# lisvulaczo/lodestar

Measured on AMD Instinct MI355X. Metric: BLS signature sets verified/sec (whole node) at 1/2/4/8 MI355X; p50 batch latency, higher is better.
Workload: dtype u32

## Files before the change

include/lodestar_bls.h:

```cpp
#ifndef LODESTAR_BLS_H
#define LODESTAR_BLS_H

#include <stddef.h>
#include <stdint.h>

#ifdef __cplusplus
extern "C" {
#endif

#define LSG_OK 0
#define LSG_ERR_INVALID_ARG 1
#define LSG_ERR_NO_DEVICE 2
#define LSG_ERR_DEVICE 3
#define LSG_ERR_NOMEM 4
#define LSG_ERR_CLOSED 5
#define LSG_ERR_BUSY 6
#define LSG_ERR_ENTROPY 7

#define LSG_BLST_SUCCESS 0
#define LSG_BLST_BAD_ENCODING 1
#define LSG_BLST_POINT_NOT_ON_CURVE 2
#define LSG_BLST_POINT_NOT_IN_GROUP 3
#define LSG_BLST_AGGR_TYPE_MISMATCH 4
#define LSG_BLST_VERIFY_FAIL 5
#define LSG_BLST_PK_IS_INFINITY 6
#define LSG_BLST_BAD_SCALAR 7
#define LSG_BLST_INVALID_SIZE 10
#define LSG_ERR_EMPTY_SET 100
#define LSG_ERR_EMPTY_AGGREGATE 101
#define LSG_ERR_BAD_INDEX 102
#define LSG_ERR_BAD_COMMITTEE 103

#define LSG_PK_INDEX 4u
#define LSG_PK_BITS 8u

#define LSG_MSG_OBJECT 0x80000000u

#define LSG_INVALID 0
#define LSG_VALID 1
#define LSG_ERROR 2

#define LSG_JOB_BATCHABLE 1u
#define LSG_JOB_PRIORITY 2u
#define LSG_JOB_VALIDATE_KEYS 4u

typedef struct lsg_ctx lsg_ctx;
typedef uint64_t lsg_ticket;

typedef struct {
  const uint8_t* pks;
  uint32_t pk_len;
  uint32_t n_pks;
  const uint8_t* msg;
  uint32_t msg_len;
  const uint8_t* sig;
  uint32_t sig_len;
} lsg_set;

typedef struct {
  const lsg_set* sets;
  uint32_t n_sets;
  uint32_t flags;
} lsg_job;

typedef struct {
  int32_t status;
  int32_t err_code;
} lsg_job_result;

typedef struct {
  uint32_t batch_retries;
  uint32_t batch_sigs_success;
  uint64_t start_ns;
  uint64_t end_ns;
  uint32_t n_final_exps;
  uint32_t submit_us;
  int32_t key_error;
  uint32_t key_error_job;
} lsg_stats;

int lsg_init(int device_ordinal, lsg_ctx** out);
int lsg_init_devices(const int* device_ids, int n_devices, lsg_ctx** out);
int lsg_destroy(lsg_ctx* ctx);
int lsg_device_count(lsg_ctx* ctx, int32_t* n);
const char* lsg_last_error(lsg_ctx* ctx);
int lsg_device_name(lsg_ctx* ctx, char* buf, size_t len);
int lsg_reserve(lsg_ctx* ctx, size_t max_sets, size_t max_pks, size_t max_msg_bytes, int32_t n_slots);
int lsg_allocation_count(lsg_ctx* ctx, uint64_t* n);

int lsg_submit_jobs(lsg_ctx* ctx, const lsg_job* jobs, size_t n_jobs, uint64_t seed, lsg_ticket* ticket);
int lsg_wait_jobs(lsg_ctx* ctx, lsg_ticket ticket, lsg_job_result* results , lsg_stats* stats);
int lsg_jobs_partial(lsg_ctx* ctx, lsg_ticket ticket, uint8_t* out576, int32_t* has_batch);
int lsg_jobs_partial_device(lsg_ctx* ctx, lsg_ticket ticket, void* dev_out576, int32_t* has_batch);
int lsg_wait_jobs_node(lsg_ctx* ctx, lsg_ticket ticket, int32_t node_valid, lsg_job_result* results,
                       lsg_stats* stats);
int lsg_set_coalesce(lsg_ctx* ctx, uint32_t max_sets, int32_t max_inflight);
int lsg_assign_jobs(const uint32_t* job_sets, size_t n_jobs, int32_t n_devices, int32_t* owner);
int lsg_pipeline_slots(lsg_ctx* ctx, int32_t* n);
int lsg_poll(lsg_ctx* ctx, lsg_ticket ticket, int32_t* done);
int lsg_verify_jobs(lsg_ctx* ctx, const lsg_job* jobs, size_t n_jobs, uint64_t seed, lsg_job_result* results,
                    lsg_stats* stats);

int lsg_verify_sets(lsg_ctx* ctx, const lsg_set* sets, size_t n_sets, uint64_t seed, lsg_job_result* result);

int lsg_aggregate_pubkeys(lsg_ctx* ctx, const uint8_t* pks, uint32_t pk_len, size_t n, uint8_t* out96,
                          int32_t* err_code);
int lsg_aggregate_pubkeys_multi(lsg_ctx* ctx, const lsg_set* sets, size_t n_sets, uint8_t* out96, int32_t* err);

int lsg_hash_to_g2(lsg_ctx* ctx, const uint8_t* msgs, uint32_t msg_len, size_t n, const uint8_t* dst,
                   uint32_t dst_len, uint8_t* out192);

int lsg_sig_decode(lsg_ctx* ctx, const uint8_t* sigs, uint32_t sig_len, size_t n, uint8_t* out192, int32_t* err);

int lsg_batch_partial(lsg_ctx* ctx, const lsg_set* sets, size_t n_sets, uint64_t seed, uint8_t* out576,
                      int32_t* set_err, int32_t* any_error);
int lsg_final_verify(lsg_ctx* ctx, const uint8_t* partials576, size_t n_partials, int32_t* valid);
int lsg_final_submit(lsg_ctx* ctx, const uint8_t* partials576, size_t n_partials, lsg_ticket* ticket);
int lsg_final_submit_device(lsg_ctx* ctx, const void* dev_partials576, size_t n_partials, lsg_ticket* ticket);
int lsg_final_wait(lsg_ctx* ctx, lsg_ticket ticket, int32_t* valid);
int lsg_final_submit_groups(lsg_ctx* ctx, const uint8_t* partials576, size_t n_groups, size_t per_group,
                            lsg_ticket* ticket);
int lsg_final_wait_groups(lsg_ctx* ctx, lsg_ticket ticket, int32_t* valid );

int lsg_pubkey_table_set(lsg_ctx* ctx, size_t first_index, const uint8_t* pks, uint32_t pk_len, size_t n,
                         int32_t* err);
int lsg_pubkey_table_size(lsg_ctx* ctx, size_t* n);

int lsg_committees_set(lsg_ctx* ctx, uint32_t first_id, const uint32_t* indices,
                       const uint32_t* offsets , size_t n_committees,
                       int32_t* err );
int lsg_committees_clear(lsg_ctx* ctx, uint32_t first_id, size_t n);
int lsg_committee_count(lsg_ctx* ctx, size_t* n);

int lsg_pubkey_validate(lsg_ctx* ctx, const uint8_t* pks, uint32_t pk_len, size_t n, uint8_t* out96, int32_t* err);

int lsg_aggregate_signatures(lsg_ctx* ctx, const uint8_t* sigs, uint32_t sig_len, const uint32_t* offsets,
                             size_t n_groups, uint8_t* out96, int32_t* err);

int lsg_signing_roots(lsg_ctx* ctx, const uint8_t* roots32, size_t n, const uint8_t* domain32, uint32_t domain_stride,
                      uint8_t* out32);
int lsg_attestation_signing_roots(lsg_ctx* ctx, const uint8_t* data128, size_t n, const uint8_t* domain32,
                                  uint32_t domain_stride, uint8_t* out32);
int lsg_deposit_signing_roots(lsg_ctx* ctx, const uint8_t* msgs88, size_t n, const uint8_t* domain32,
                              uint32_t domain_stride, uint8_t* out32);
int lsg_object_signing_roots(lsg_ctx* ctx, const uint8_t* objs, uint32_t obj_len, size_t n, const uint8_t* domain32,
                             uint32_t domain_stride, uint8_t* out32);

int lsg_verify_deposits(lsg_ctx* ctx, const uint8_t* data184, size_t n, const uint8_t* domain32, uint64_t seed,
                        uint8_t* valid, int32_t* err);

int lsg_sign(lsg_ctx* ctx, const uint8_t* sks32, const uint8_t* msgs, uint32_t msg_len, size_t n, uint8_t* out96);
int lsg_sk_to_pk(lsg_ctx* ctx, const uint8_t* sks32, size_t n, uint8_t* out96);

int lsg_check_fp2_mul(lsg_ctx* ctx, const uint32_t* in, size_t n, uint32_t* out);
int lsg_check_fp_sqr(lsg_ctx* ctx, const uint32_t* in, size_t n, uint32_t* out);
int lsg_check_fp2_sqr(lsg_ctx* ctx, const uint32_t* in, size_t n, uint32_t* out);
int lsg_check_sums(lsg_ctx* ctx, const uint32_t* in, size_t n, uint32_t* out);
int lsg_probe_fp_mul_rate(lsg_ctx* ctx, double* fp_mul_per_s, double* mad_per_s);

int lsg_probe_mad_peak(lsg_ctx* ctx, double* mad_per_s);

int lsg_last_kernel_times(lsg_ctx* ctx, const char** names, double* ms, int max);

#ifdef __cplusplus
}
#endif
#endif
```

lodestar_amd/_native.py:

```python
import ctypes
import os
import struct
import threading

HERE = os.path.dirname(os.path.abspath(__file__))
LIB_PATH = os.environ.get("LSG_LIB", os.path.join(HERE, "liblodestar_bls.so"))
AB_LIB_PATH = os.path.join(HERE, "liblodestar_bls_ab.so")

LSG_OK = 0
LSG_ERR_INVALID_ARG = 1
LSG_ERR_NO_DEVICE = 2
LSG_ERR_BUSY = 6
LSG_ERR_ENTROPY = 7

LSG_INVALID = 0
LSG_VALID = 1
LSG_ERROR = 2

LSG_JOB_BATCHABLE = 1
LSG_JOB_PRIORITY = 2
LSG_JOB_VALIDATE_KEYS = 4

BLST_NAMES = {
    0: "BLST_SUCCESS", 1: "BLST_BAD_ENCODING", 2: "BLST_POINT_NOT_ON_CURVE", 3: "BLST_POINT_NOT_IN_GROUP",
    4: "BLST_AGGR_TYPE_MISMATCH", 5: "BLST_VERIFY_FAIL", 6: "BLST_PK_IS_INFINITY", 7: "BLST_BAD_SCALAR",
    10: "BLST_INVALID_SIZE",
}
LSG_ERR_EMPTY_SET = 100
LSG_ERR_EMPTY_AGGREGATE = 101
LSG_ERR_BAD_INDEX = 102
LSG_ERR_BAD_COMMITTEE = 103
LSG_PK_INDEX = 4
LSG_PK_BITS = 8
LSG_MSG_OBJECT = 0x80000000


def error_message(code):
    if code == LSG_ERR_EMPTY_SET:
        return "Empty signature set"
    if code == LSG_ERR_EMPTY_AGGREGATE:
        return "EMPTY_AGGREGATE_ARRAY"
    if code == LSG_ERR_BAD_INDEX:
        return "Unknown pubkey index"
    if code == LSG_ERR_BAD_COMMITTEE:
        return "Unknown committee or bit length mismatch"
    return "BLST_ERROR: " + BLST_NAMES.get(code, f"BLST_UNKNOWN_{code}")


class NativeUnavailable(RuntimeError):
    pass


class PkIndices(list):

    def tobytes(self):
        import array
        a = array.array("I", self)
        assert a.itemsize == 4
        return a.tobytes()


class PkBits:

    def __init__(self, committee, bits, n_bits):
        self.committee = int(committee)
        self.n_bits = int(n_bits)
        nb = (self.n_bits + 7) // 8
        self.bits = bytes(bits)[:nb].ljust(nb, b"\0")

    def __len__(self):
        return self.n_bits

    def tobytes(self):
        return struct.pack("=I", self.committee) + self.bits


def _key_form(pks):
    if isinstance(pks, PkBits):
        return LSG_PK_BITS, pks.n_bits, pks.tobytes()
    if isinstance(pks, PkIndices):
        return LSG_PK_INDEX, len(pks), pks.tobytes()
    pk_len = len(pks[0]) if pks else 96
    if any(len(p) != pk_len for p in pks):
        raise ValueError("all pubkeys of one set must share one encoding length")
    if pk_len == LSG_PK_BITS:
        pk_len = 0
    return pk_len, len(pks), b"".join(pks)


class MsgObject:

    def __init__(self, obj, domain):
        self.obj = bytes(obj)
        self.domain = bytes(domain)

    def __len__(self):
        return len(self.obj) + len(self.domain)

    def tobytes(self):
        return self.obj + self.domain


def _msg_form(msg):
    if isinstance(msg, MsgObject):
        b = msg.tobytes()
        return b, len(b) | LSG_MSG_OBJECT
    return msg, len(msg)


class LsgSet(ctypes.Structure):
    _fields_ = [
        ("pks", ctypes.c_void_p), ("pk_len", ctypes.c_uint32), ("n_pks", ctypes.c_uint32),
        ("msg", ctypes.c_void_p), ("msg_len", ctypes.c_uint32),
        ("sig", ctypes.c_void_p), ("sig_len", ctypes.c_uint32),
    ]


class LsgJob(ctypes.Structure):
    _fields_ = [("sets", ctypes.POINTER(LsgSet)), ("n_sets", ctypes.c_uint32), ("flags", ctypes.c_uint32)]


class LsgJobResult(ctypes.Structure):
    _fields_ = [("status", ctypes.c_int32), ("err_code", ctypes.c_int32)]


class LsgStats(ctypes.Structure):
    _fields_ = [
        ("batch_retries", ctypes.c_uint32), ("batch_sigs_success", ctypes.c_uint32),
        ("start_ns", ctypes.c_uint64), ("end_ns", ctypes.c_uint64),
        ("n_final_exps", ctypes.c_uint32), ("submit_us", ctypes.c_uint32),
        ("key_error", ctypes.c_int32), ("key_error_job", ctypes.c_uint32),
    ]


_lib = None
_lib_lock = threading.Lock()

EXPORTS = [
    "lsg_init", "lsg_init_devices", "lsg_destroy", "lsg_device_count", "lsg_last_error", "lsg_device_name",
    "lsg_reserve", "lsg_allocation_count", "lsg_verify_jobs", "lsg_verify_sets",
    "lsg_aggregate_pubkeys", "lsg_hash_to_g2", "lsg_sig_decode", "lsg_batch_partial", "lsg_final_verify",
    "lsg_probe_fp_mul_rate", "lsg_last_kernel_times", "lsg_sign", "lsg_sk_to_pk",
    "lsg_submit_jobs", "lsg_wait_jobs", "lsg_wait_jobs_node", "lsg_jobs_partial", "lsg_assign_jobs", "lsg_poll",
    "lsg_final_submit", "lsg_final_wait", "lsg_pipeline_slots", "lsg_probe_mad_peak",
    "lsg_pubkey_table_set", "lsg_pubkey_table_size", "lsg_pubkey_validate",
    "lsg_final_submit_groups", "lsg_final_wait_groups", "lsg_aggregate_signatures",
    "lsg_signing_roots", "lsg_attestation_signing_roots", "lsg_jobs_partial_device", "lsg_final_submit_device",
    "lsg_set_coalesce", "lsg_aggregate_pubkeys_multi", "lsg_check_fp2_mul",
    "lsg_check_fp_sqr", "lsg_check_fp2_sqr", "lsg_check_sums",
    "lsg_deposit_signing_roots", "lsg_verify_deposits",
    "lsg_committees_set", "lsg_committees_clear", "lsg_committee_count",
    "lsg_object_signing_roots",
]


def load_library(path=LIB_PATH):
    global _lib
    with _lib_lock:
        if _lib is not None and path == LIB_PATH:
            return _lib
        if not os.path.exists(path):
            raise NativeUnavailable(f"{path} not built (run python -c 'import __graft_entry__; __graft_entry__.build()')")
        lib = ctypes.CDLL(path)
        vp, u32, u64, i32, sz = ctypes.c_void_p, ctypes.c_uint32, ctypes.c_uint64, ctypes.c_int32, ctypes.c_size_t
        pi32 = ctypes.POINTER(ctypes.c_int32)
        lib.lsg_init.argtypes = [ctypes.c_int, ctypes.POINTER(vp)]
        lib.lsg_init_devices.argtypes = [ctypes.POINTER(ctypes.c_int), ctypes.c_int, ctypes.POINTER(vp)]
        lib.lsg_device_count.argtypes = [vp, pi32]
        lib.lsg_reserve.argtypes = [vp, sz, sz, sz, i32]
        lib.lsg_allocation_count.argtypes = [vp, ctypes.POINTER(u64)]
        lib.lsg_wait_jobs_node.argtypes = [vp, u64, i32, ctypes.POINTER(LsgJobResult), ctypes.POINTER(LsgStats)]
        lib.lsg_jobs_partial.argtypes = [vp, u64, ctypes.c_char_p, pi32]
        lib.lsg_jobs_partial_device.argtypes = [vp, u64, vp, pi32]
        lib.lsg_final_submit_device.argtypes = [vp, vp, sz, ctypes.POINTER(u64)]
        lib.lsg_assign_jobs.argtypes = [ctypes.POINTER(u32), sz, i32, pi32]
        lib.lsg_destroy.argtypes = [vp]
        lib.lsg_last_error.argtypes = [vp]
        lib.lsg_last_error.restype = ctypes.c_char_p
        lib.lsg_device_name.argtypes = [vp, ctypes.c_char_p, sz]
        lib.lsg_verify_jobs.argtypes = [vp, ctypes.POINTER(LsgJob), sz, u64, ctypes.POINTER(LsgJobResult),
                                        ctypes.POINTER(LsgStats)]
        lib.lsg_verify_sets.argtypes = [vp, ctypes.POINTER(LsgSet), sz, u64, ctypes.POINTER(LsgJobResult)]
        lib.lsg_aggregate_pubkeys.argtypes = [vp, ctypes.c_char_p, u32, sz, ctypes.c_char_p, pi32]
        lib.lsg_aggregate_pubkeys_multi.argtypes = [vp, ctypes.POINTER(LsgSet), sz, ctypes.c_char_p, pi32]
        lib.lsg_hash_to_g2.argtypes = [vp, ctypes.c_char_p, u32, sz, ctypes.c_char_p, u32, ctypes.c_char_p]
        lib.lsg_sig_decode.argtypes = [vp, ctypes.c_char_p, u32, sz, ctypes.c_char_p, pi32]
        lib.lsg_batch_partial.argtypes = [vp, ctypes.POINTER(LsgSet), sz, u64, ctypes.c_char_p, pi32, pi32]
        lib.lsg_final_verify.argtypes = [vp, ctypes.c_char_p, sz, pi32]
        lib.lsg_probe_fp_mul_rate.argtypes = [vp, ctypes.POINTER(ctypes.c_double), ctypes.POINTER(ctypes.c_double)]
        lib.lsg_last_kernel_times.argtypes = [vp, ctypes.POINTER(ctypes.c_char_p), ctypes.POINTER(ctypes.c_double),
                                              ctypes.c_int]
        lib.lsg_sign.argtypes = [vp, ctypes.c_char_p, ctypes.c_char_p, u32, sz, ctypes.c_char_p]
        lib.lsg_sk_to_pk.argtypes = [vp, ctypes.c_char_p, sz, ctypes.c_char_p]
        pu64 = ctypes.POINTER(u64)
        lib.lsg_submit_jobs.argtypes = [vp, ctypes.POINTER(LsgJob), sz, u64, pu64]
        lib.lsg_wait_jobs.argtypes = [vp, u64, ctypes.POINTER(LsgJobResult), ctypes.POINTER(LsgStats)]
        lib.lsg_poll.argtypes = [vp, u64, pi32]
        lib.lsg_pubkey_table_set.argtypes = [vp, sz, ctypes.c_char_p, u32, sz, pi32]
        lib.lsg_pubkey_table_size.argtypes = [vp, ctypes.POINTER(sz)]
        lib.lsg_committees_set.argtypes = [vp, u32, ctypes.POINTER(u32), ctypes.POINTER(u32), sz, pi32]
        lib.lsg_committees_clear.argtypes = [vp, u32, sz]
        lib.lsg_committee_count.argtypes = [vp, ctypes.POINTER(sz)]
        lib.lsg_final_submit_groups.argtypes = [vp, ctypes.c_char_p, sz, sz, pu64]
        lib.lsg_final_wait_groups.argtypes = [vp, u64, pi32]
        lib.lsg_pubkey_validate.argtypes = [vp, ctypes.c_char_p, u32, sz, ctypes.c_char_p, pi32]
        lib.lsg_signing_roots.argtypes = [vp, ctypes.c_char_p, sz, ctypes.c_char_p, u32, ctypes.c_char_p]
        lib.lsg_attestation_signing_roots.argtypes = [vp, ctypes.c_char_p, sz, ctypes.c_char_p, u32, ctypes.c_char_p]
        lib.lsg_deposit_signing_roots.argtypes = [vp, ctypes.c_char_p, sz, ctypes.c_char_p, u32, ctypes.c_char_p]
        lib.lsg_object_signing_roots.argtypes = [vp, ctypes.c_char_p, u32, sz, ctypes.c_char_p, u32, ctypes.c_char_p]
        lib.lsg_verify_deposits.argtypes = [vp, ctypes.c_char_p, sz, ctypes.c_char_p, u64, ctypes.c_char_p, pi32]
        lib.lsg_aggregate_signatures.argtypes = [vp, ctypes.c_char_p, u32, ctypes.POINTER(u32), sz,
                                                 ctypes.c_char_p, pi32]
        lib.lsg_final_submit.argtypes = [vp, ctypes.c_char_p, sz, pu64]
        lib.lsg_final_wait.argtypes = [vp, u64, pi32]
        lib.lsg_pipeline_slots.argtypes = [vp, pi32]
        lib.lsg_set_coalesce.argtypes = [vp, u32, i32]
        lib.lsg_check_fp2_mul.argtypes = [vp, ctypes.c_char_p, sz, ctypes.c_char_p]
        lib.lsg_check_fp_sqr.argtypes = [vp, ctypes.c_char_p, sz, ctypes.c_char_p]
        lib.lsg_check_fp2_sqr.argtypes = [vp, ctypes.c_char_p, sz, ctypes.c_char_p]
        lib.lsg_check_sums.argtypes = [vp, ctypes.c_char_p, sz, ctypes.c_char_p]
        lib.lsg_probe_mad_peak.argtypes = [vp, ctypes.POINTER(ctypes.c_double)]
        for name in EXPORTS:
            if name != "lsg_last_error":
                getattr(lib, name).restype = ctypes.c_int
        if path == LIB_PATH:
            _lib = lib
        return lib


class SetBuffer:

    def __init__(self, sets):
        self._keep = []
        sets = list(sets)
        self.arr = (LsgSet * max(len(sets), 1))()
        for i, (pks, msg, sig) in enumerate(sets):
            pk_len, n_pks, pkb = _key_form(pks)
            msg, msg_len = _msg_form(msg)
            for b in (pkb, msg, sig):
                self._keep.append(b)
            s = self.arr[i]
            s.pks = ctypes.cast(ctypes.c_char_p(pkb), ctypes.c_void_p) if pkb else None
            s.pk_len = pk_len
            s.n_pks = n_pks
            s.msg = ctypes.cast(ctypes.c_char_p(msg), ctypes.c_void_p) if msg else None
            s.msg_len = msg_len
            s.sig = ctypes.cast(ctypes.c_char_p(sig), ctypes.c_void_p) if sig else None
            s.sig_len = len(sig)
        self.n = len(sets)


def assign_jobs(job_sizes, n_devices):
    lib = load_library()
    n = len(job_sizes)
    sizes = (ctypes.c_uint32 * max(n, 1))(*job_sizes)
    owner = (ctypes.c_int32 * max(n, 1))()
    rc = lib.lsg_assign_jobs(sizes, n, int(n_devices), owner)
    if rc != LSG_OK:
        raise ValueError(f"lsg_assign_jobs failed ({rc})")
    return list(owner[:n])


class PreparedJobs:

    def __init__(self, jobs):
        import numpy as np
        flat = [st for sets, _ in jobs for st in sets]
        n = len(flat)
        pk_parts, pk_len, n_pks = [], np.zeros(max(n, 1), np.uint32), np.zeros(max(n, 1), np.uint32)
        for i, (pks, _m, _s) in enumerate(flat):
            pk_len[i], n_pks[i], b = _key_form(pks)
            pk_parts.append(b)

        def pack(parts):
            lens = np.array([len(p) for p in parts] or [0], np.uint64)
            offs = np.zeros_like(lens)
            if len(parts) > 1:
                offs[1:] = np.cumsum(lens)[:-1]
            buf = np.frombuffer(b"".join(parts) + b"\0", dtype=np.uint8).copy()
            return buf, offs, lens

        self._pk, pk_off, _ = pack(pk_parts)
        forms = [_msg_form(m) for _, m, _ in flat]
        self._msg, msg_off, msg_len = pack([b for b, _ in forms])
        msg_word = np.array([w for _, w in forms] or [0], np.uint32)
        self._sig, sig_off, sig_len = pack([s for _, _, s in flat])
        self.sets = (LsgSet * max(n, 1))()
        dt = np.dtype({"names": ["pks", "pk_len", "n_pks", "msg", "msg_len", "sig", "sig_len"],
                       "formats": [np.uint64, np.uint32, np.uint32, np.uint64, np.uint32, np.uint64, np.uint32],
                       "offsets": [LsgSet.pks.offset, LsgSet.pk_len.offset, LsgSet.n_pks.offset, LsgSet.msg.offset,
                                   LsgSet.msg_len.offset, LsgSet.sig.offset, LsgSet.sig_len.offset],
                       "itemsize": ctypes.sizeof(LsgSet)})
        v = np.frombuffer(self.sets, dtype=dt)
        if n:
            v["pks"][:n] = np.where(n_pks[:n] > 0, self._pk.ctypes.data + pk_off[:n], 0)
            v["pk_len"][:n] = pk_len[:n]
            v["n_pks"][:n] = n_pks[:n]
            v["msg"][:n] = np.where(msg_len[:n] > 0, self._msg.ctypes.data + msg_off[:n], 0)
            v["msg_len"][:n] = msg_word[:n]
            v["sig"][:n] = np.where(sig_len[:n] > 0, self._sig.ctypes.data + sig_off[:n], 0)
            v["sig_len"][:n] = sig_len[:n]
        self.n_jobs = len(jobs)
        self.n_sets = n
        self.jobs = (LsgJob * max(len(jobs), 1))()
        jd = np.dtype({"names": ["sets", "n_sets", "flags"], "formats": [np.uint64, np.uint32, np.uint32],
                       "offsets": [LsgJob.sets.offset, LsgJob.n_sets.offset, LsgJob.flags.offset],
                       "itemsize": ctypes.sizeof(LsgJob)})
        jv = np.frombuffer(self.jobs, dtype=jd)
        counts = np.array([len(sets) for sets, _ in jobs] or [0], np.uint64)
        firsts = np.zeros_like(counts)
        if len(jobs) > 1:
            firsts[1:] = np.cumsum(counts)[:-1]
        if jobs:
            jv["sets"][:len(jobs)] = ctypes.addressof(self.sets) + firsts * ctypes.sizeof(LsgSet)
            jv["n_sets"][:len(jobs)] = counts
            jv["flags"][:len(jobs)] = [f for _, f in jobs]


class Context:

    def __init__(self, device=0, devices=None, lib=None):
        self.lib = load_library(lib or LIB_PATH)
        h = ctypes.c_void_p()
        if devices is None:
            rc = self.lib.lsg_init(int(device), ctypes.byref(h))
        else:
            ids = (ctypes.c_int * len(devices))(*devices)
            rc = self.lib.lsg_init_devices(ids, len(devices), ctypes.byref(h))
        if rc != LSG_OK:
            raise NativeUnavailable(f"lsg_init({devices if devices is not None else device}) failed with status {rc} "
                                    f"(no gfx950 device?)")
        self.h = h
        self.device = device if devices is None else devices[0]
        self.devices = [self.device] if devices is None else list(devices)

    def reserve(self, max_sets, max_pks=None, max_msg_bytes=None, n_slots=0):
        max_pks = max_sets if max_pks is None else max_pks
        max_msg_bytes = 32 * max_sets if max_msg_bytes is None else max_msg_bytes
        self._check(self.lib.lsg_reserve(self.h, max_sets, max_pks, max_msg_bytes, n_slots), "lsg_reserve")

    def set_coalesce(self, max_sets, max_inflight=2):
        self._check(self.lib.lsg_set_coalesce(self.h, int(max_sets), int(max_inflight)), "lsg_set_coalesce")

    def allocation_count(self):
        v = ctypes.c_uint64()
        self._check(self.lib.lsg_allocation_count(self.h, ctypes.byref(v)), "lsg_allocation_count")
        return v.value

    def device_count(self):
        v = ctypes.c_int32()
        self._check(self.lib.lsg_device_count(self.h, ctypes.byref(v)), "lsg_device_count")
        return v.value

    def close(self):
        if getattr(self, "h", None):
            self.lib.lsg_destroy(self.h)
            self.h = None

    def __del__(self):
        try:
            self.close()
        except Exception:
            pass

    def _check(self, rc, what):
        if rc != LSG_OK:
            raise RuntimeError(f"{what} failed ({rc}): {self.lib.lsg_last_error(self.h).decode(errors='replace')}")

    def device_name(self):
        b = ctypes.create_string_buffer(256)
        self._check(self.lib.lsg_device_name(self.h, b, 256), "lsg_device_name")
        return b.value.decode()

# ... 177 lines not shown
    def attestation_signing_roots(self, data128s, domains):
        return self._signing_roots("lsg_attestation_signing_roots", data128s, 128, domains)

    def deposit_signing_roots(self, msgs88, domains):
        return self._signing_roots("lsg_deposit_signing_roots", msgs88, 88, domains)

    def object_signing_roots(self, objs, domains):
        n = len(objs)
        if n == 0:
            return []
        size = len(objs[0])
        assert all(len(o) == size for o in objs)
        if isinstance(domains, (bytes, bytearray)):
            dom, stride = bytes(domains), 0
        else:
            assert len(domains) == n
            dom, stride = b"".join(domains), 32
        assert len(dom) == (32 if stride == 0 else 32 * n)
        out = ctypes.create_string_buffer(32 * n)
        self._check(self.lib.lsg_object_signing_roots(self.h, b"".join(objs), size, n, dom, stride, out),
                    "lsg_object_signing_roots")
        raw = out.raw
        return [raw[32 * i:32 * i + 32] for i in range(n)]

    def verify_deposits(self, data184s, domain, seed=0):
        n = len(data184s)
        if n == 0:
            return []
        assert all(len(d) == 184 for d in data184s) and len(domain) == 32
        valid = ctypes.create_string_buffer(n)
        err = (ctypes.c_int32 * n)()
        self._check(self.lib.lsg_verify_deposits(self.h, b"".join(data184s), n, bytes(domain), seed, valid, err),
                    "lsg_verify_deposits")
        raw = valid.raw
        return [(raw[i], err[i]) for i in range(n)]

    def hash_to_g2(self, msgs, dst=b"BLS_SIG_BLS12381G2_XMD:SHA-256_SSWU_RO_POP_"):
        if not msgs:
            return []
        ml = len(msgs[0])
        assert all(len(m) == ml for m in msgs)
        out = ctypes.create_string_buffer(192 * len(msgs))
        self._check(self.lib.lsg_hash_to_g2(self.h, b"".join(msgs), ml, len(msgs), dst, len(dst), out), "lsg_hash_to_g2")
        raw = out.raw
        return [raw[192 * i:192 * i + 192] for i in range(len(msgs))]

    def sig_decode(self, sigs):
        if not sigs:
            return []
        sl = len(sigs[0])
        assert all(len(s) == sl for s in sigs)
        out = ctypes.create_string_buffer(192 * len(sigs))
        err = (ctypes.c_int32 * len(sigs))()
        self._check(self.lib.lsg_sig_decode(self.h, b"".join(sigs), sl, len(sigs), out, err), "lsg_sig_decode")
        raw = out.raw
        return [(raw[192 * i:192 * i + 192], err[i]) for i in range(len(sigs))]

    def batch_partial(self, sets, seed=0):
        b = SetBuffer(sets)
        out = ctypes.create_string_buffer(576)
        errs = (ctypes.c_int32 * max(b.n, 1))()
        anyerr = ctypes.c_int32()
        self._check(self.lib.lsg_batch_partial(self.h, b.arr, b.n, seed, out, errs, ctypes.byref(anyerr)),
                    "lsg_batch_partial")
        return out.raw, [errs[i] for i in range(b.n)], bool(anyerr.value)

    def final_verify(self, partials):
        v = ctypes.c_int32()
        self._check(self.lib.lsg_final_verify(self.h, b"".join(partials), len(partials), ctypes.byref(v)),
                    "lsg_final_verify")
        return bool(v.value)

    def final_submit(self, partials):
        t = ctypes.c_uint64()
        rc = self.lib.lsg_final_submit(self.h, b"".join(partials), len(partials), ctypes.byref(t))
        if rc == LSG_ERR_BUSY:
            return None
        self._check(rc, "lsg_final_submit")
        return t.value

    def final_wait(self, ticket):
        v = ctypes.c_int32()
        self._check(self.lib.lsg_final_wait(self.h, ticket, ctypes.byref(v)), "lsg_final_wait")
        return bool(v.value)

    def final_submit_groups(self, groups):
        ng = len(groups)
        pg = len(groups[0]) if groups else 0
        if any(len(g) != pg for g in groups):
            raise ValueError("every group needs the same number of partials")
        t = ctypes.c_uint64()
        rc = self.lib.lsg_final_submit_groups(self.h, b"".join(b"".join(g) for g in groups), ng, pg, ctypes.byref(t))
        if rc == LSG_ERR_BUSY:
            return None
        self._check(rc, "lsg_final_submit_groups")
        t_ng = ng
        return (t.value, t_ng)

    def final_wait_groups(self, ticket):
        t, ng = ticket
        v = (ctypes.c_int32 * max(ng, 1))()
        self._check(self.lib.lsg_final_wait_groups(self.h, t, v), "lsg_final_wait_groups")
        return [bool(x) for x in v[:ng]]

    def sign(self, sks, msgs):
        if not sks:
            return []
        ml = len(msgs[0])
        out = ctypes.create_string_buffer(96 * len(sks))
        skb = b"".join(int(k).to_bytes(32, "big") for k in sks)
        self._check(self.lib.lsg_sign(self.h, skb, b"".join(msgs), ml, len(sks), out), "lsg_sign")
        raw = out.raw
        return [raw[96 * i:96 * i + 96] for i in range(len(sks))]

    def sk_to_pk(self, sks):
        if not sks:
            return []
        out = ctypes.create_string_buffer(96 * len(sks))
        skb = b"".join(int(k).to_bytes(32, "big") for k in sks)
        self._check(self.lib.lsg_sk_to_pk(self.h, skb, len(sks), out), "lsg_sk_to_pk")
        raw = out.raw
        return [raw[96 * i:96 * i + 96] for i in range(len(sks))]

    def check_fp2_mul(self, words):
        n = len(words) // 56
        assert len(words) == 56 * n
        out = ctypes.create_string_buffer(4 * 28 * n)
        src = struct.pack(f"<{len(words)}I", *words)
        self._check(self.lib.lsg_check_fp2_mul(self.h, src, n, out), "lsg_check_fp2_mul")
        return list(struct.unpack(f"<{28 * n}I", out.raw))

    def _check_sqr(self, fn, words, per_item):
        n = len(words) // per_item
        assert len(words) == per_item * n
        out = ctypes.create_string_buffer(4 * per_item * n)
        src = struct.pack(f"<{len(words)}I", *words)
        self._check(getattr(self.lib, fn)(self.h, src, n, out), fn)
        return list(struct.unpack(f"<{per_item * n}I", out.raw))

    def check_fp_sqr(self, words):
        return self._check_sqr("lsg_check_fp_sqr", words, 14)

    def check_fp2_sqr(self, words):
        return self._check_sqr("lsg_check_fp2_sqr", words, 28)

    def check_sums(self, words):
        n = len(words) // (12 * 14)
        assert len(words) == 12 * 14 * n
        out = ctypes.create_string_buffer(4 * 42 * 14 * n)
        src = struct.pack(f"<{len(words)}I", *words)
        self._check(self.lib.lsg_check_sums(self.h, src, n, out), "lsg_check_sums")
        return list(struct.unpack(f"<{42 * 14 * n}I", out.raw))

    def probe_fp_mul_rate(self):
        a, b = ctypes.c_double(), ctypes.c_double()
        self._check(self.lib.lsg_probe_fp_mul_rate(self.h, ctypes.byref(a), ctypes.byref(b)), "lsg_probe_fp_mul_rate")
        return a.value, b.value

    def last_kernel_times(self, max_entries=1024):
        names = (ctypes.c_char_p * max_entries)()
        ms = (ctypes.c_double * max_entries)()
        n = self.lib.lsg_last_kernel_times(self.h, names, ms, max_entries)
        return [(names[i].decode(), ms[i]) for i in range(n)]
```

lodestar_amd/build.py:

```python
import os
import shutil
import subprocess
import sys

HERE = os.path.dirname(os.path.abspath(__file__))
ROOT = os.path.dirname(HERE)
CSRC = os.path.join(HERE, "csrc")
OUT = os.path.join(HERE, "liblodestar_bls.so")
SOURCES = ["lsg_k_hash.hip", "lsg_k_sig.hip", "lsg_k_pk.hip", "lsg_k_miller.hip", "lsg_k_reduce.hip", "lsg_slp.hip",
           "lsg_host.hip"]
HEADERS = ["lsg_types.hpp", "lsg_fp_lane.hpp", "lsg_fp_elem.hpp", "lsg_tower.hpp", "lsg_curve.hpp", "lsg_h2c.hpp",
           "lsg_pairing.hpp", "lsg_constants.hpp", "lsg_fp_pair.hpp", "lsg_constants_r29.hpp", "lsg_io.hpp",
           "lsg_serial.h", "lsg_kcommon.hpp", "lsg_launch.h", "lsg_layout.h", "lsg_slp_progs.h", "lsg_slp_exec.hpp", "lsg_inv.hpp",
           "lsg_ab.h", "lsg_plan.hpp", "lsg_bits.h", "lsg_ssz.hpp"]
OBJ = os.path.join(HERE, "_obj")
AB_OUT = os.path.join(HERE, "liblodestar_bls_ab.so")
AB_SOURCES = ["lsg_host.hip", "lsg_serial.hip", "lsg_serial_wide.hip"]
AB_FLAGS = ["-DLSG_AB=1"]


def hipcc():
    for c in (shutil.which("hipcc"), "/opt/rocm/bin/hipcc"):
        if c and os.path.exists(c):
            return c
    raise RuntimeError("hipcc not found")


def _deps():
    return [os.path.join(CSRC, f) for f in HEADERS] + [os.path.join(ROOT, "include", "lodestar_bls.h"),
                                                       os.path.abspath(__file__)]


def needs_rebuild(out=OUT, sources=SOURCES):
    if not os.path.exists(out):
        return True
    deps = [os.path.join(CSRC, f) for f in sources] + _deps()
    return max(os.path.getmtime(d) for d in deps if os.path.exists(d)) > os.path.getmtime(out)


CFLAGS = ["--offload-arch=gfx950", "-O3", "-std=c++17", "-fPIC", "-DLSG_BIGFN=__host__ __device__ __forceinline__"]


def _obj_dir(extra):
    if not extra:
        return OBJ
    import hashlib
    return OBJ + "_" + hashlib.sha1(" ".join(extra).encode()).hexdigest()[:10]


def _compile(src, verbose, extra):
    obj = os.path.join(_obj_dir(extra), os.path.splitext(src)[0] + ".o")
    srcp = os.path.join(CSRC, src)
    dep_t = max(os.path.getmtime(d) for d in [srcp] + _deps() if os.path.exists(d))
    if os.path.exists(obj) and os.path.getmtime(obj) >= dep_t:
        return obj
    cmd = [hipcc()] + CFLAGS + extra + ["-I", CSRC, "-I", os.path.join(ROOT, "include"), "-c", srcp, "-o", obj + ".tmp"]
    if verbose:
        print("[lodestar_amd.build]", " ".join(cmd), flush=True)
    subprocess.check_call(cmd)
    os.replace(obj + ".tmp", obj)
    return obj


def build(force=False, verbose=True, extra=None, out=None):
    from concurrent.futures import ThreadPoolExecutor
    gen = os.path.join(ROOT, "tools", "gen_constants.py")
    const = os.path.join(CSRC, "lsg_constants.hpp")
    if not os.path.exists(const) or os.path.getmtime(gen) > os.path.getmtime(const):
        subprocess.check_call([sys.executable, gen, const])
    gen_slp = os.path.join(ROOT, "tools", "gen_slp.py")
    progs = os.path.join(CSRC, "lsg_slp_progs.h")
    if not os.path.exists(progs) or os.path.getmtime(gen_slp) > os.path.getmtime(progs):
        subprocess.check_call([sys.executable, gen_slp, progs])
    extra = list(extra or [])
    out = out or OUT
    if not force and not extra and out == OUT and not needs_rebuild():
        if read_manifest(OUT) is None:
            write_manifest(OUT, SOURCES, [])
        return OUT
    odir = _obj_dir(extra)
    os.makedirs(odir, exist_ok=True)
    if force:
        for f in os.listdir(odir):
            os.remove(os.path.join(odir, f))
    jobs = int(os.environ.get("LSG_BUILD_JOBS", str(min(8, os.cpu_count() or 4))))
    with ThreadPoolExecutor(max_workers=jobs) as ex:
        objs = list(ex.map(lambda s: _compile(s, verbose, extra), SOURCES))
    _link(objs, out, verbose)
    write_manifest(out, SOURCES, extra)
    return out


def source_hash(sources=SOURCES):
    import hashlib
    h = hashlib.sha256()
    files = sorted(set([os.path.join(CSRC, f) for f in list(sources) + HEADERS] +
                       [os.path.join(ROOT, "include", "lodestar_bls.h")]))
    for f in files:
        if os.path.exists(f):
            h.update(os.path.basename(f).encode() + b"\0")
            with open(f, "rb") as fh:
                h.update(fh.read())
    return h.hexdigest()


def _compiler_version():
    try:
        out = subprocess.run([hipcc(), "--version"], capture_output=True, text=True, timeout=60).stdout
        return next((ln.strip() for ln in out.splitlines() if "clang version" in ln), out.splitlines()[0].strip())
    except Exception as e:
        return "unknown (%s)" % e


def write_manifest(out, sources, extra):
    import hashlib
    import json
    import time
    with open(out, "rb") as fh:
        so_sha = hashlib.sha256(fh.read()).hexdigest()
    rec = {"lib": os.path.basename(out), "so_sha256_16": so_sha[:16], "src_sha256": source_hash(sources),
           "compiler": _compiler_version(), "flags": CFLAGS + list(extra),
           "built_utc": time.strftime("%Y-%m-%dT%H:%M:%SZ", time.gmtime())}
    with open(out + ".manifest.json", "w") as fh:
        fh.write(json.dumps(rec, sort_keys=True) + "\n")
    return rec


def read_manifest(out=None):
    import json
    try:
        with open((out or OUT) + ".manifest.json") as fh:
            return json.loads(fh.read())
    except (OSError, ValueError):
        return None


def _link(objs, out, verbose):
    cmd = [hipcc(), "--offload-arch=gfx950", "-fPIC", "-shared"] + objs + ["-L/opt/rocm/lib", "-lrccl",
                                                                           "-Wl,-rpath,/opt/rocm/lib", "-o", out + ".tmp"]
    if verbose:
        print("[lodestar_amd.build]", " ".join(cmd), flush=True)
    subprocess.check_call(cmd)
    os.replace(out + ".tmp", out)


def build_ab(verbose=True):
    from concurrent.futures import ThreadPoolExecutor
    build(verbose=verbose)
    if not needs_rebuild(AB_OUT, SOURCES + AB_SOURCES):
        return AB_OUT
    os.makedirs(_obj_dir(AB_FLAGS), exist_ok=True)
    with ThreadPoolExecutor(max_workers=len(AB_SOURCES)) as ex:
        ab = dict(zip(AB_SOURCES, ex.map(lambda s: _compile(s, verbose, AB_FLAGS), AB_SOURCES)))
    objs = [ab.get(s) or os.path.join(OBJ, os.path.splitext(s)[0] + ".o") for s in SOURCES]
    objs += [ab[s] for s in AB_SOURCES if s not in SOURCES]
    _link(objs, AB_OUT, verbose)
    write_manifest(AB_OUT, SOURCES + AB_SOURCES, AB_FLAGS)
    return AB_OUT


NAPI_SRC = os.path.join(HERE, "napi", "lsg_napi.c")
NAPI_OUT = os.path.join(HERE, "napi", "lsg_napi.node")
NODE_INCLUDE = "/usr/include/node"


def build_napi(verbose=True):
    if not os.path.exists(os.path.join(NODE_INCLUDE, "node_api.h")):
# ... 19 lines not shown
```

lodestar_amd/csrc/lsg_host.hip:

```cpp
#include <hip/hip_runtime.h>
#include <rccl/rccl.h>
#include <stdio.h>
#include <stdlib.h>
#include <errno.h>
#include <string.h>
#include <sys/random.h>
#include <time.h>

#include <algorithm>
#include <atomic>
#include <condition_variable>
#include <chrono>
#include <mutex>
#include <shared_mutex>
#include <thread>
#include <unordered_map>
#include <string>
#include <vector>

#include "../../include/lodestar_bls.h"
#include "lsg_launch.h"
#include "lsg_layout.h"
#include "lsg_serial.h"
#include "lsg_ab.h"
// ... 335 lines not shown
  do {                                                    \
    timer_begin((s), name);                               \
    hipError_t _le = (call);                              \
    timer_end((s));                                       \
    if (_le != hipSuccess) return fail((s), name, _le);   \
  } while (0)

inline const int32_t* PL(Slot* s, size_t off) { return P_<int32_t>(s->d_plan) + off; }

void keep_times(Slot* s) {
  auto& v = s->d->last_times;
  v.clear();
  for (size_t i = 0; i < s->ntimers; i++) {
    float t = 0;
    if (hipEventElapsedTime(&t, s->timers[i].a, s->timers[i].b) != hipSuccess) t = -1;
    v.push_back({s->timers[i].name, t});
  }
}

int prio_stream(lsg_ctx* c, Dev* d, hipStream_t* st) {
  if (!*st) {
    int least = 0, greatest = 0;
    LSG_HIPC(c, hipSetDevice(d->device));
    LSG_HIPC(c, hipDeviceGetStreamPriorityRange(&least, &greatest));
    LSG_HIPC(c, hipStreamCreateWithPriority(st, hipStreamNonBlocking, greatest));
  }
  return LSG_OK;
}

hipError_t event_wait(hipEvent_t e) {
  const auto t0 = std::chrono::steady_clock::now();
  for (;;) {
    const hipError_t r = hipEventQuery(e);
    if (r != hipErrorNotReady) return r;
    if (std::chrono::steady_clock::now() - t0 > std::chrono::microseconds(20))
      std::this_thread::sleep_for(std::chrono::microseconds(30));
  }
}

bool blocking_waits() {
  const char* e = getenv("LSG_BLOCKING_WAITS");
  return e && atoi(e) != 0;
}

int slot_create(Dev* d, Slot* s, int index, hipStream_t shared) {
  s->d = d;
  s->index = index;
  if (shared) {
    s->st[0] = s->st[1] = shared;
    s->own_streams = false;
  } else {
    for (int k = 0; k < 2; k++) LSG_HIP(s, hipStreamCreateWithFlags(&s->st_norm[k], hipStreamNonBlocking));
    s->st[0] = s->st_norm[0];
    s->st[1] = s->st_norm[1];
  }
  hipEvent_t* evs[] = {&s->ev_in, &s->ev_sig, &s->ev_grp, &s->ev_part, &s->ev_done, &s->ev_node, &s->ev_xp};
  for (hipEvent_t* e : evs) LSG_HIP(s, hipEventCreateWithFlags(e, hipEventDisableTiming));
  if (blocking_waits()) {
    for (hipEvent_t* e : {&s->ev_part, &s->ev_done}) {
      LSG_HIP(s, hipEventDestroy(*e));
      LSG_HIP(s, hipEventCreateWithFlags(e, hipEventDisableTiming | hipEventBlockingSync));
    }
  }
  LSG_RC(ensure(s, s->d_dst, 256));
  LSG_HIP(s, hipMemcpy(s->d_dst.p, DST_POP, DST_POP_LEN, hipMemcpyHostToDevice));
  return LSG_OK;
}

void slot_destroy(Slot* s) {
  if (!s->d) return;
  for (int k = 0; k < 2; k++)
    if (s->st[k]) (void)hipStreamSynchronize(s->st[k]);
  DevBuf* bufs[] = {&s->d_sig,  &s->d_siglen, &s->d_msg,  &s->d_msgoff, &s->d_msglen, &s->d_pk,    &s->d_pklen,
                    &s->d_rnd,  &s->d_mode,   &s->d_dst,  &s->d_ub,     &s->d_sigaff, &s->d_siginf, &s->d_seterr,
                    &s->d_pkp,  &s->d_pkerr,  &s->d_agg,  &s->d_P,      &s->d_pinf,   &s->d_H,     &s->d_hinf,
                    &s->d_rs,   &s->d_rs2,    &s->d_fall, &s->d_fall2,  &s->d_Pp,     &s->d_zP,    &s->d_zPi,
                    &s->d_U,    &s->d_nrm,    &s->d_nrmi, &s->d_Hp,     &s->d_zN,     &s->d_zNi,   &s->binv_lv[0],
                    &s->binv_lv[1], &s->binv_iv[0], &s->binv_iv[1], &s->d_lines, &s->d_S, &s->d_F, &s->d_verdict,
                    &s->d_Sb,   &s->d_fgb,    &s->d_Fb,   &s->d_bkt,    &s->d_bits,   &s->d_aux,   &s->d_gath,
                    &s->d_nodeF, &s->d_nodeV, &s->d_plan, &s->d_mid, &s->d_Hm, &s->d_hinfm,
                    &s->d_mmask, &s->d_PmP, &s->d_Pm, &s->d_pinfm, &s->d_errm, &s->d_xport,
                    &s->d_agga, &s->d_aggi, &s->d_aggpre, &s->d_aggtot, &s->d_aggflag, &s->d_cbits};
  for (DevBuf* b : bufs) free_dev(*b);
  for (auto& u : s->seg_tmp)
    for (DevBuf& b : u) free_dev(b);
  HostBuf* hb[] = {&s->h_arena, &s->h_err, &s->h_pinf, &s->h_pkerr, &s->h_verdict, &s->h_blob, &s->h_plan, &s->h_nodeV,
                   &s->h_xport, &s->h_cbits};
  for (HostBuf* b : hb) free_host(*b);
  for (Timer& t : s->timers) {
    (void)hipEventDestroy(t.a);
    (void)hipEventDestroy(t.b);
  }
  s->timers.clear();
  hipEvent_t evs[] = {s->ev_in, s->ev_sig, s->ev_grp, s->ev_part, s->ev_done, s->ev_node, s->ev_xp};
  for (hipEvent_t e : evs)
    if (e) (void)hipEventDestroy(e);
  if (s->own_streams) {
    for (int k = 0; k < 2; k++) {
      if (s->st_prio[k]) (void)hipStreamSynchronize(s->st_prio[k]);
      if (s->st_norm[k]) (void)hipStreamSynchronize(s->st_norm[k]);
    }
    for (int k = 0; k < 2; k++) {
      if (s->st_norm[k]) (void)hipStreamDestroy(s->st_norm[k]);
      s->st_norm[k] = s->st_prio[k] = s->st[k] = nullptr;
    }
  }
  s->d = nullptr;
}

int slot_streams(Slot* s, bool prio) {
  if (!s->own_streams) return LSG_OK;
  if (prio && !s->st_prio[0]) {
    Dev* d = s->d;
    for (int k = 0; k < 2; k++) LSG_RC(prio_stream(d->c, d, &d->s_pp[k]));
    s->st_prio[0] = d->s_pp[0];
    s->st_prio[1] = d->s_pp[1];
  }
  hipStream_t* p = prio ? s->st_prio : s->st_norm;
  s->st[0] = p[0];
  s->st[1] = p[1];
  return LSG_OK;
}

int slot_ready(Dev* d, Slot* s, int index) {
  if (s->d) return LSG_OK;
  const int rc = slot_create(d, s, index, nullptr);
  if (rc) slot_destroy(s);
  return rc;
}

bool miller_fused() { return lsg_ab_long("LSG_MILLER_FUSED", 1) != 0; }

size_t slp_items_max();
int miller_k_for(size_t n_sets) {
  if (miller_fused()) return n_sets <= slp_items_max() ? 1 : 4;
  const long v = lsg_ab_long("LSG_MILLER_K", 0);
  if (v == 1 || v == 2 || v == 4) return (int)v;
  return n_sets >= 8192 ? 4 : (n_sets >= 1024 ? 2 : 1);
}

bool agg_tree_on() { return lsg_ab_long("LSG_AGG_TREE", 0) != 0; }

Switches read_switches() {
  Switches w;
  w.package_group = lsg_ab_long("LSG_PACKAGE_GROUP", 1) != 0;
  w.sub_groups = lsg_ab_long("LSG_SUB_GROUPS", 1) != 0;
  w.nb_merge = lsg_ab_long("LSG_NB_MERGE", 1) != 0;
  w.msg_agg = lsg_ab_long("LSG_MSG_AGG", 1) != 0;
  w.msm_min_group = (size_t)std::max(1L, lsg_ab_long("LSG_MSM_MIN_GROUP", 256));
  w.b0_min = (size_t)std::max(0L, lsg_ab_long("LSG_B0_MIN", 64));
  w.b0_run = (size_t)std::max(2L, lsg_ab_long("LSG_B0_RUN", 4));
  w.seg_fold_wide = (int)lsg_ab_long("LSG_SEG_FOLD_WIDE", SEG_FOLD_WIDE);
  w.slp_items = slp_items_max();
  return w;
}
SegPlan slot_seg(Slot* s, int op, const std::vector<int32_t>& seg_off, const std::vector<int32_t>& seg_len, bool has_idx,
                 size_t idx_off, int32_t dst_base) {
  return plan_seg(s->plan, op, seg_off, seg_len, has_idx, idx_off, dst_base,
                  (int)lsg_ab_long("LSG_SEG_FOLD_WIDE", SEG_FOLD_WIDE));
}

void binv_sizes(size_t n, size_t* lv, size_t* iv);
size_t binv_lv_words(size_t n) {
  size_t a, b;
  binv_sizes(n, &a, &b);
  return a;
}
size_t binv_iv_words(size_t n) {
  size_t a, b;
  binv_sizes(n, &a, &b);
  return b;
}

int size_inputs(Slot* s, size_t n, size_t np, size_t mb) {
  const size_t nn = std::max(n, (size_t)1), pp = std::max(np, (size_t)1);
  auto al = [](size_t x) { return (x + 7) & ~(size_t)7; };
  const size_t arena = al(192 * nn) + al(4 * nn) * 4 + al(4 * pp) + al(8 * nn) + al(96 * pp) + al(std::max(mb, (size_t)1)) + nn;
  LSG_RC(ensure_host(s, s->h_arena, arena));
  LSG_RC(ensure(s, s->d_sig, 192 * nn));
  LSG_RC(ensure(s, s->d_siglen, 4 * nn));
  LSG_RC(ensure(s, s->d_msg, std::max(mb, (size_t)1)));
  LSG_RC(ensure(s, s->d_msgoff, 4 * nn));
  LSG_RC(ensure(s, s->d_msglen, 4 * nn));
  LSG_RC(ensure(s, s->d_pk, 96 * pp));
  LSG_RC(ensure(s, s->d_pklen, 4 * pp));
  LSG_RC(ensure(s, s->d_rnd, 8 * nn));
  LSG_RC(ensure(s, s->d_mode, nn));
  LSG_RC(ensure(s, s->d_mid, 4 * nn));
  return LSG_OK;
}

int size_state(Slot* s, size_t n, size_t np, size_t ng, size_t n_msm, int pkg = 0) {
  const size_t nn = std::max(n, (size_t)1), pp = std::max(np, (size_t)1), gg = std::max(ng, (size_t)1);
  const size_t g_msm = std::max(n_msm, (size_t)1);
  struct {
    DevBuf* b;
    size_t bytes;
  } dev[] = {{&s->d_ub, 256 * nn},
             {&s->d_sigaff, 4 * W_G2A * nn},
             {&s->d_siginf, nn},
             {&s->d_seterr, 4 * nn},
             {&s->d_pkp, 4 * W_G1P * pp},
             {&s->d_pkerr, 4 * pp},
             {&s->d_agg, 4 * W_G1P * nn},
             {&s->d_P, 4 * W_G1A * nn},
             {&s->d_pinf, nn},
             {&s->d_H, 4 * W_G2A * nn},
             {&s->d_hinf, nn},
             {&s->d_rs, 4 * W_G2P * nn},
             {&s->d_Pp, 4 * W_G1P * nn},
             {&s->d_zP, 4 * W_FP * nn},
             {&s->d_zPi, 4 * W_FP * nn},
             {&s->d_U, 4 * W_H2CU * nn},
             {&s->d_nrm, 4 * W_FP * 2 * nn},
             {&s->d_nrmi, 4 * W_FP * 2 * nn},
             {&s->d_Hp, 4 * W_G2P * nn},
             {&s->d_zN, 4 * W_FP * nn},
             {&s->d_zNi, 4 * W_FP * nn},
             {&s->binv_lv[0], 4 * W_FP * binv_lv_words(2 * nn)},
             {&s->binv_iv[0], 4 * W_FP * binv_iv_words(2 * nn)},
             {&s->binv_lv[1], 4 * W_FP * binv_lv_words(nn)},
             {&s->binv_iv[1], 4 * W_FP * binv_iv_words(nn)},
             {&s->d_S, 4 * W_G2P * gg},
             {&s->d_F, 4 * W_F12 * gg},
             {&s->d_verdict, 4 * gg},
             {&s->d_Sb, (size_t)288 * (MSM_BITS * g_msm + gg)},
             {&s->d_fgb, 576 * gg},
             {&s->d_Fb, 576 * gg},
             {&s->d_bkt, 4 * W_G2P * (size_t)MSM_WINDOWS * MSM_DIGITS * g_msm},
             {&s->d_bits, 4 * W_G2P * (size_t)MSM_BITS * g_msm},
             {&s->d_gath, 576 * (LSG_MAX_DEVICES + 2)},
             {&s->d_nodeF, 4 * W_F12 * (LSG_MAX_DEVICES + 1)},
             {&s->d_nodeV, 64}};
  for (auto& x : dev) LSG_RC(ensure(s, *x.b, x.bytes));
  if (pkg == 1) {
    if (!miller_fused()) LSG_RC(ensure(s, s->d_lines, 4 * (size_t)ML_STEPS * W_LINE * nn));
    LSG_RC(ensure(s, s->d_fall, 4 * W_F12 * (2 * nn + gg + 2)));
  }
  if (pkg) {
    LSG_RC(ensure(s, s->d_fall2, 4 * W_F12 * (nn + std::max(gg, nn))));
    LSG_RC(ensure(s, s->d_rs2, 4 * W_G2P * nn));
  }
  LSG_RC(ensure_host(s, s->h_err, 4 * nn));
  LSG_RC(ensure_host(s, s->h_pinf, nn));
  LSG_RC(ensure_host(s, s->h_pkerr, 4 * pp));
  LSG_RC(ensure_host(s, s->h_verdict, 4 * gg));
  LSG_RC(ensure_host(s, s->h_blob, 576 * gg));
  LSG_RC(ensure_host(s, s->h_nodeV, 64));
  return LSG_OK;
}

int size_seg(Slot* s, int use, const SegPlan& P) {
  if (P.tmp_items == 0) return LSG_OK;
  const size_t W = P.op == 0 ? W_G1P : (P.op == 1 ? W_G2P : W_F12);
  LSG_RC(ensure(s, s->seg_tmp[use][0], 4 * W * P.tmp_items));
  return ensure(s, s->seg_tmp[use][1], 4 * W * P.tmp_items);
}

int upload_plan(Slot* s) {
  const size_t bytes = 4 * std::max(s->plan.size(), (size_t)1);
  LSG_RC(ensure_host(s, s->h_plan, bytes));
  LSG_RC(ensure(s, s->d_plan, bytes));
  if (!s->plan.empty()) {
    memcpy(s->h_plan.p, s->plan.data(), 4 * s->plan.size());
    LSG_HIP(s, hipMemcpyAsync(s->d_plan.p, s->h_plan.p, 4 * s->plan.size(), hipMemcpyHostToDevice, s->st[0]));
  }
  return LSG_OK;
}

int run_seg(Slot* s, int use, const char* name, const SegPlan& P, const uint32_t* src, uint32_t* dst) {
  LSG_RC(size_seg(s, use, P));
  uint32_t* tmp[3] = {nullptr, P_<uint32_t>(s->seg_tmp[use][0]), P_<uint32_t>(s->seg_tmp[use][1])};
  const int32_t* idx = P.has_idx ? PL(s, P.idx_off) : nullptr;
  for (size_t k = 0; k < P.passes.size(); k++) {
    const SegPass& q = P.passes[k];
    const uint32_t* in = q.src == 0 ? src : tmp[q.src];
    KL(s, name, lsgk::seg_reduce(S_(s), P.op, q.n_chunks, q.ips_log2, PL(s, q.chunk_off), k == 0 ? idx : nullptr, in, dst,
                                 tmp[q.tmp_out]));
  }
  return LSG_OK;
}

int run_pk_seg(Slot* s, const SegPlan& P, uint32_t* dst) {
  LSG_RC(size_seg(s, 0, P));
  Dev* d = s->d;
  uint32_t* tmp[3] = {nullptr, P_<uint32_t>(s->seg_tmp[0][0]), P_<uint32_t>(s->seg_tmp[0][1])};
  for (size_t k = 0; k < P.passes.size(); k++) {
    const SegPass& q = P.passes[k];
    if (k == 0)
      KL(s, "g1_aggregate", lsgk::pk_agg_seg(S_(s), q.n_chunks, q.ips_log2, PL(s, q.chunk_off), P_<uint8_t>(s->d_pk),
                                             s->pk_stride, P_<uint32_t>(s->d_pklen), P_<int32_t>(s->d_pkerr),
                                             P_<uint32_t>(d->d_pktab), P_<uint8_t>(d->d_pktab_ok), (uint32_t)d->pktab_n,
                                             dst, tmp[q.tmp_out]));
    else
      KL(s, "g1_aggregate", lsgk::seg_reduce(S_(s), 0, q.n_chunks, q.ips_log2, PL(s, q.chunk_off), nullptr,
                                             tmp[q.src], dst, tmp[q.tmp_out]));
  }
  return LSG_OK;
}

static bool binv_block_on() { return lsg_ab_long("LSG_BINV_BLOCK", 1) != 0; }

void binv_sizes(size_t n, size_t* lv, size_t* iv) {
  size_t a = 0, b = 0;
  for (size_t m = n; m > 1;) {
    const size_t up = (m + LSG_BINV_T - 1) / LSG_BINV_T;
    a += m + up;
    b += up;
    m = up;
  }
  *lv = std::max(a, (size_t)1);
  *iv = std::max(b, (size_t)1);
}

int batch_inv(Slot* s, int ws, const char* name, const uint32_t* v, size_t n, uint32_t* out) {
  if (n == 0) return LSG_OK;
  size_t lvw, ivw;
  binv_sizes(n, &lvw, &ivw);
  LSG_RC(ensure(s, s->binv_lv[ws], 4 * W_FP * lvw));
  LSG_RC(ensure(s, s->binv_iv[ws], 4 * W_FP * ivw));
  uint32_t* lv = P_<uint32_t>(s->binv_lv[ws]);
  uint32_t* iv = P_<uint32_t>(s->binv_iv[ws]);
  if (binv_block_on()) {
    const int T = (int)std::min<size_t>(64, std::max<size_t>(1, (n + 128 * 64 - 1) / (128 * 64)));
    KL(s, name, lsgk::binv_block(S_(s), (int)n, T, 1, v, lv, out));
    return LSG_OK;
  }
  std::vector<size_t> cnt{n};
  std::vector<uint32_t*> val{(uint32_t*)v}, pre, inv{out};
  size_t lo = 0, io = 0;
  while (cnt.back() > 1) {
    const size_t m = cnt.back(), up = (m + LSG_BINV_T - 1) / LSG_BINV_T;
    pre.push_back(lv + W_FP * lo);
    lo += m;
    val.push_back(lv + W_FP * lo);
    lo += up;
    inv.push_back(iv + W_FP * io);
    io += up;
    cnt.push_back(up);
  }
  const size_t L = cnt.size() - 1;
  if (L == 0) {
    KL(s, name, lsgk::binv_root(S_(s), v, out));
    return LSG_OK;
  }
  for (size_t l = 0; l < L; l++)
    KL(s, name, lsgk::binv_fold(S_(s), (int)cnt[l], l == 0 ? 1 : 0, val[l], pre[l], val[l + 1]));
  KL(s, name, lsgk::binv_root(S_(s), val[L], inv[L]));
  for (size_t l = L; l-- > 0;)
    KL(s, name, lsgk::binv_unfold(S_(s), (int)cnt[l], l == 0 ? 1 : 0, val[l], pre[l], inv[l + 1], inv[l]));
  return LSG_OK;
}


size_t slp_items_max() {
  const long v = lsg_ab_long("LSG_SLP_ITEMS", 2048);
  return lsg_serial_mode() == LSG_SERIAL_SLP && v > 0 ? (size_t)v : 0;
}

int launch_hash(Slot* s, int n, uint32_t* H, uint8_t* hinf) {
  KL(s, "k_h2c_prep", lsgk::h2c_prep(S_(s), n, P_<uint8_t>(s->d_ub), P_<uint32_t>(s->d_U), P_<uint32_t>(s->d_nrm)));
  LSG_RC(batch_inv(s, 0, "binv_sswu", P_<uint32_t>(s->d_nrm), 2 * (size_t)n, P_<uint32_t>(s->d_nrmi)));
  KL(s, "k_h2c_map", lsgk::h2c_map(S_(s), n, P_<uint32_t>(s->d_U), P_<uint32_t>(s->d_nrmi), P_<uint32_t>(s->d_Hp)));
  if ((size_t)n <= slp_items_max()) {
    KL(s, "k_slp_h2c", lsg_slp_h2c_clear(S_(s), n, P_<uint32_t>(s->d_Hp), H, hinf));
    return LSG_OK;
  }
  KL(s, "k_h2c_clear", lsgk::h2c_clear(S_(s), n, P_<uint32_t>(s->d_Hp), P_<uint32_t>(s->d_zN), hinf));
  LSG_RC(batch_inv(s, 0, "binv_hash", P_<uint32_t>(s->d_zN), (size_t)n, P_<uint32_t>(s->d_zNi)));
  KL(s, "k_h2c_affine", lsgk::h2c_affine(S_(s), n, P_<uint32_t>(s->d_Hp), P_<uint32_t>(s->d_zNi), hinf, H));
  return LSG_OK;
}

static uint64_t msg_key(const uint8_t* m, uint32_t msg_len) {
  uint64_t h = 0x9e3779b97f4a7c15ull ^ msg_len;
  const uint32_t len = msg_bytes(msg_len);
  uint32_t k = 0;
  for (; k + 8 <= len; k += 8) {
    uint64_t w;
    memcpy(&w, m + k, 8);
    h = (h ^ w) * 0xff51afd7ed558ccdull;
    h ^= h >> 32;
  }
  for (; k < len; k++) h = (h ^ m[k]) * 0x100000001b3ull;
  return h ^ (h >> 29);
}

int stage_sets(Slot* s, const lsg_set* const* sets, size_t n, uint64_t seed, bool scale,
               const std::vector<uint8_t>* noscale = nullptr, bool dedup = false, bool bits_ok = false) {
  size_t npk = 0, msg_total = 0, n_bits_sets = 0, bit_words = 0;
  bool any_obj = false;
  bool all_index = true;
  auto is_bits = [&](const lsg_set* q) { return bits_ok && q->pk_len == LSG_PK_BITS; };
  for (size_t i = 0; i < n; i++) {
    msg_total += msg_bytes(sets[i]->msg_len);
    any_obj = any_obj || msg_marked(sets[i]->msg_len);
    if (is_bits(sets[i])) {
      n_bits_sets++;
      bit_words += bits_words(sets[i]->n_pks);
      continue;
    }
    npk += sets[i]->n_pks;
    if (sets[i]->n_pks && sets[i]->pk_len != LSG_PK_INDEX) all_index = false;
  }
  s->bits_sets.clear();
  s->shape.bits_p.clear();
  s->shape.bits_kerr.clear();
  s->pk_all_bits = n > 0 && n_bits_sets == n;
  uint32_t* cbits = nullptr;
  if (n_bits_sets) {
    s->shape.bits_p.assign(n, -1);
    s->shape.bits_kerr.assign(n, 0);
    s->bits_sets.reserve(n_bits_sets);
    LSG_RC(ensure_host(s, s->h_cbits, 4 * bit_words));
    LSG_RC(ensure(s, s->d_cbits, 4 * bit_words));
    cbits = H_<uint32_t>(s->h_cbits);
  }
  size_t bw = 0;
  const size_t ks = all_index ? 4 : 96;
  s->pk_stride = (uint32_t)ks;
  s->n_sets = n;
  s->n_pks = npk;
  LSG_RC(size_inputs(s, n, npk, msg_total));
  const size_t nn = std::max(n, (size_t)1), np = std::max(npk, (size_t)1);
  auto al = [](size_t x) { return (x + 7) & ~(size_t)7; };
  const size_t o_sig = 0, o_siglen = al(o_sig + 192 * nn), o_msgoff = al(o_siglen + 4 * nn),
               o_msglen = al(o_msgoff + 4 * nn), o_mid = al(o_msglen + 4 * nn), o_pklen = al(o_mid + 4 * nn),
               o_rnd = al(o_pklen + 4 * np), o_pk = al(o_rnd + 8 * nn), o_msg = al(o_pk + ks * np);
  uint8_t* A = H_<uint8_t>(s->h_arena);
  uint32_t* siglen = (uint32_t*)(A + o_siglen);
  uint32_t* msgoff = (uint32_t*)(A + o_msgoff);
  uint32_t* msglen = (uint32_t*)(A + o_msglen);
  uint32_t* mid = (uint32_t*)(A + o_mid);
  uint32_t* pklen = (uint32_t*)(A + o_pklen);
  uint64_t* rnd = (uint64_t*)(A + o_rnd);
// ... 53 lines not shown
        if (s->mkey[h] != key) continue;
        const lsg_set* r = sets[s->mfirst[e]];
        if (r->msg_len == q->msg_len && (q->msg_len == 0 || memcmp(r->msg, q->msg, msg_bytes(q->msg_len)) == 0)) {
          id = e;
          break;
        }
      }
    }
    mid[i] = id;
    if (id == nm) {
      msgoff[nm] = (uint32_t)mo;
      msglen[nm] = q->msg_len;
      const uint32_t mb = msg_bytes(q->msg_len);
      if (mb) memcpy(A + o_msg + mo, q->msg, mb);
      mo += mb;
      nm++;
    }
    if (is_bits(q)) {
      const lsg_ctx* c = s->d->c;
      s->shape.pk_cnt[i] = 0;
      s->shape.pk_first[i] = (uint32_t)po;
      BitsSet b;
      b.out = (int32_t)i;
      uint32_t id = 0;
      if (q->pks) memcpy(&id, q->pks, 4);
      if (!q->pks || id >= c->cm_ok.size() || !c->cm_ok[id] || c->cm_len[id] != q->n_pks)
        s->shape.bits_kerr[i] = LSG_ERR_BAD_COMMITTEE;
      else
        b = bits_stage_set(id, q->pks + 4, q->n_pks, (int32_t)i, cbits, &bw);
      s->shape.bits_p[i] = (int32_t)b.p;
      s->bits_sets.push_back(b);
      continue;
    }
    s->shape.pk_cnt[i] = q->n_pks;
    s->shape.pk_first[i] = (uint32_t)po;
    if (q->n_pks != 1) single = false;
    if (all_index) {
      std::fill(pklen + po, pklen + po + q->n_pks, (uint32_t)LSG_PK_INDEX);
      if (q->pks)
        memcpy(A + o_pk + 4 * po, q->pks, 4 * (size_t)q->n_pks);
      else
        memset(A + o_pk + 4 * po, 0, 4 * (size_t)q->n_pks);
      po += q->n_pks;
      continue;
    }
    for (uint32_t k = 0; k < q->n_pks; k++) {
      pklen[po] = q->pk_len;
      uint8_t* pd = A + o_pk + 96 * po;
      if ((q->pk_len == 48 || q->pk_len == 96 || q->pk_len == LSG_PK_INDEX) && q->pks)
        memcpy(pd, q->pks + (size_t)q->pk_len * k, q->pk_len);
      else
        memset(pd, 0, 4);
      po++;
    }
  }
  s->single_keys = single && n > 0;
  s->n_msgs = nm;
  s->msg_objs = any_obj;
  s->msg_dedup = nm < n;
  if (s->msg_dedup) s->msg_id.assign(mid, mid + n);
  if (scale && n) {
    if (seed == 0) {
      if (!os_random(rnd, 8 * n)) {
        set_err(s->d->c, "no entropy for the RLC randomizers (getrandom failed)");
        return LSG_ERR_ENTROPY;
      }
      for (size_t i = 0; i < n; i++)
        while (rnd[i] == 0)
          if (!os_random(&rnd[i], 8)) {
            set_err(s->d->c, "no entropy for the RLC randomizers (getrandom failed)");
            return LSG_ERR_ENTROPY;
          }
    } else {
      uint64_t sd = seed;
      for (size_t i = 0; i < n; i++) {
        uint64_t r;
        do r = splitmix64(sd);
        while (r == 0);
        rnd[i] = r;
      }
    }
  } else if (n) {
    memset(rnd, 0, 8 * n);
  }
  if (scale && noscale)
    for (size_t i = 0; i < n; i++)
      if ((*noscale)[i]) rnd[i] = 0;
  memcpy(s->rnd.data(), rnd, 8 * n);
  hipStream_t S = s->st[0];
  struct {
    DevBuf* d;
    size_t off, len;
  } cp[] = {{&s->d_sig, o_sig, 192 * nn},      {&s->d_siglen, o_siglen, 4 * nn}, {&s->d_msg, o_msg, std::max(msg_total, (size_t)1)},
            {&s->d_msgoff, o_msgoff, 4 * nn}, {&s->d_msglen, o_msglen, 4 * nn}, {&s->d_pk, o_pk, ks * np},
            {&s->d_pklen, o_pklen, 4 * np},   {&s->d_rnd, o_rnd, 8 * nn}};
  for (auto& x : cp) LSG_HIP(s, hipMemcpyAsync(x.d->p, A + x.off, x.len, hipMemcpyHostToDevice, S));
  if (s->msg_dedup) LSG_HIP(s, hipMemcpyAsync(s->d_mid.p, A + o_mid, 4 * n, hipMemcpyHostToDevice, S));
  if (bw) LSG_HIP(s, hipMemcpyAsync(s->d_cbits.p, cbits, 4 * bw, hipMemcpyHostToDevice, S));
  return LSG_OK;
}

int run_pk_bits(Slot* s, uint32_t* dst) {
  if (s->bits_sets.empty()) return LSG_OK;
  Dev* d = s->d;
  KL(s, "k_pk_agg_bits", lsgk::pk_agg_bits(S_(s), (int)s->bplan.n_pairs, PL(s, s->bplan.pair_off), PL(s, s->bplan.plan_off),
                                           P_<uint32_t>(s->d_cbits), P_<uint32_t>(d->d_cm_idx), P_<uint32_t>(d->d_cm_off),
                                           P_<uint32_t>(d->d_cm_sum), P_<uint32_t>(d->d_pktab), P_<uint8_t>(d->d_pktab_ok),
                                           (uint32_t)d->pktab_n, dst));
  return LSG_OK;
}


int launch_accum(Slot* s, size_t n_items, size_t item_off, uint32_t* fall, bool single = false) {
  const int ni = (int)n_items;
  const int32_t* items = PL(s, item_off);
  if (ni > 0 && (single || s->K == 1) && miller_fused() && (size_t)ni <= std::max(slp_items_max(), (size_t)8192) &&
      slp_items_max() > 0) {
    KL(s, "k_slp_items1", lsg_slp_miller_items1(S_(s), ni, items, P_<uint32_t>(s->d_P), P_<uint8_t>(s->d_pinf),
                                                P_<uint8_t>(s->d_hinf), P_<int32_t>(s->d_seterr), P_<uint32_t>(s->d_H),
                                                fall));
    return LSG_OK;
  }
  if (single && ni > 0) {
    LSG_RC(ensure(s, s->d_lines, 4 * (size_t)ML_STEPS * W_LINE * n_items));
    KL(s, "k_miller_lines_list", lsgk::miller_lines_list(S_(s), ni, items, P_<uint32_t>(s->d_H), P_<uint32_t>(s->d_lines)));
    KL(s, "k_miller_accum_list",
       lsgk::miller_accum_list(S_(s), ni, items, P_<uint32_t>(s->d_P), P_<uint8_t>(s->d_pinf), P_<uint8_t>(s->d_hinf),
                               P_<int32_t>(s->d_seterr), P_<uint32_t>(s->d_lines), fall));
    return LSG_OK;
  }
  if (miller_fused()) {
    KL(s, "k_miller_fused", lsgk::miller_fused(S_(s), ni, items, items + ni, P_<uint32_t>(s->d_P), P_<uint8_t>(s->d_pinf),
                                              P_<uint8_t>(s->d_hinf), P_<int32_t>(s->d_seterr), P_<uint32_t>(s->d_H),
                                              fall));
    return LSG_OK;
  }
  KL(s, "k_miller_accum",
     lsgk::miller_accum(S_(s), s->K, ni, items, items + ni, P_<uint32_t>(s->d_P), P_<uint8_t>(s->d_pinf),
                        P_<uint8_t>(s->d_hinf), P_<int32_t>(s->d_seterr), (int)s->n_sets, P_<uint32_t>(s->d_lines),
                        fall));
  return LSG_OK;
}

#define SERIAL_LABEL(name) (lsg_serial_mode() == LSG_SERIAL_SLP ? "slp_" #name : "k_row_" #name)

int launch_phase(Slot* s, const PhasePlan& Ph, const uint32_t* rs, uint32_t* fall, bool export_blobs,
                 const uint32_t* rs_msm = nullptr) {
  if (!rs_msm) rs_msm = rs;
  const size_t ng = Ph.groups.size();
  if (ng == 0) return LSG_OK;
  LSG_RC(size_state(s, s->n_sets, s->n_pks, ng, Ph.n_msm, 2));
  s->cur = 1;
  if (Ph.n_msm) {
    LSG_RC(run_seg(s, 1, "msm_buckets", Ph.buckets, rs_msm, P_<uint32_t>(s->d_bkt)));
    LSG_RC(run_seg(s, 1, "msm_bits", Ph.bits, P_<uint32_t>(s->d_bkt), P_<uint32_t>(s->d_bits)));
    KL(s, "k_g2p_to_canon", lsgk::g2p_to_canon(S_(s), (int)(MSM_BITS * Ph.n_msm), P_<uint32_t>(s->d_bits),
                                               P_<uint8_t>(s->d_Sb)));
    KL(s, SERIAL_LABEL(horner_miller),
       lsg_row_horner_miller(S_(s), (int)Ph.n_msm, P_<uint8_t>(s->d_Sb), P_<uint8_t>(s->d_fgb)));
  }
  if (Ph.n_msm < ng) {
    const int nsm = (int)(ng - Ph.n_msm);
    LSG_RC(run_seg(s, 1, "sig_sums", Ph.sums, rs, P_<uint32_t>(s->d_S)));
    uint8_t* sb = P_<uint8_t>(s->d_Sb) + (size_t)288 * MSM_BITS * Ph.n_msm;
    KL(s, "k_g2p_to_canon", lsgk::g2p_to_canon(S_(s), nsm, P_<uint32_t>(s->d_S) + W_G2P * Ph.n_msm, sb));
    KL(s, SERIAL_LABEL(miller_neg_g1),
       lsg_row_miller_neg_g1(S_(s), nsm, sb, P_<uint8_t>(s->d_fgb) + 576 * Ph.n_msm));
  }
  KL(s, "k_blobs_to_fp12", lsgk::blobs_to_fp12(S_(s), (int)ng, P_<uint8_t>(s->d_fgb), fall + W_F12 * Ph.term_base));
  LSG_HIP(s, hipEventRecord(s->ev_grp, s->st[1]));
  s->cur = 0;
  LSG_HIP(s, hipStreamWaitEvent(s->st[0], s->ev_grp, 0));
  LSG_RC(run_seg(s, 2, "fp12_product", Ph.prod, fall, P_<uint32_t>(s->d_F)));
  KL(s, "k_fp12_to_canon", lsgk::fp12_to_canon(S_(s), (int)ng, P_<uint32_t>(s->d_F), P_<uint8_t>(s->d_Fb)));
  if (export_blobs) LSG_HIP(s, hipMemcpyAsync(s->h_blob.p, s->d_Fb.p, 576 * ng, hipMemcpyDeviceToHost, s->st[0]));
  LSG_HIP(s, hipEventRecord(s->ev_part, s->st[0]));
  return LSG_OK;
}

int launch_fe_range(Slot* s, size_t g0, size_t g1) {
  if (g1 <= g0) return LSG_OK;
  s->cur = 0;
  const size_t ng = g1 - g0;
  KL(s, SERIAL_LABEL(final_exp),
     lsg_row_final_exp(S_(s), (int)ng, P_<uint8_t>(s->d_Fb) + 576 * g0, P_<int32_t>(s->d_verdict) + g0));
  LSG_HIP(s, hipMemcpyAsync(H_<int32_t>(s->h_verdict) + g0, P_<int32_t>(s->d_verdict) + g0, 4 * ng,
                            hipMemcpyDeviceToHost, s->st[0]));
  return LSG_OK;
}
int launch_fe(Slot* s, size_t ng) { return launch_fe_range(s, 0, ng); }

int launch_agg_tree(Slot* s, const AggPlan& P, uint32_t* agg);

int launch_set_stages(Slot* s, const SegPlan* pkagg, const PhasePlan& Ph, uint32_t* fall) {
  const size_t n_items = Ph.agg_g >= 0 ? Ph.n_set_items : Ph.n_items, item_off = Ph.item_off;
  const int n = (int)s->n_sets, np = (int)s->n_pks;
  if (n == 0) return LSG_OK;
  Dev* d = s->d;
  LSG_HIP(s, hipEventRecord(s->ev_in, s->st[0]));
  s->cur = 1;
  LSG_HIP(s, hipStreamWaitEvent(s->st[1], s->ev_in, 0));
  if (!s->single_keys && s->agg.tree) {
    LSG_RC(launch_agg_tree(s, s->agg, P_<uint32_t>(s->d_agg)));
  } else if (s->single_keys) {
    if (np > 0)
      KL(s, "k_pk_decode", lsgk::pk_decode(S_(s), np, P_<uint8_t>(s->d_pk), s->pk_stride, P_<uint32_t>(s->d_pklen),
                                           P_<uint32_t>(s->d_agg), P_<int32_t>(s->d_pkerr), P_<uint32_t>(d->d_pktab),
                                           P_<uint8_t>(d->d_pktab_ok), (uint32_t)d->pktab_n));
  } else if (!s->pk_all_bits) {
    LSG_RC(run_pk_seg(s, *pkagg, P_<uint32_t>(s->d_agg)));
  }
  LSG_RC(run_pk_bits(s, P_<uint32_t>(s->d_agg)));
  if (s->n_kv)
    KL(s, "k_pk_keyvalidate", lsgk::pk_keyvalidate(S_(s), (int)s->n_kv, PL(s, s->kv_off), P_<uint8_t>(s->d_pk),
                                                   P_<uint32_t>(s->d_pklen), P_<int32_t>(s->d_pkp)));
  KL(s, "k_pk_scale", lsgk::pk_scale(S_(s), n, P_<uint32_t>(s->d_agg), P_<uint64_t>(s->d_rnd), P_<uint32_t>(s->d_Pp),
                                     P_<uint32_t>(s->d_zP), P_<uint8_t>(s->d_pinf)));
  LSG_RC(batch_inv(s, 1, "binv_pk", P_<uint32_t>(s->d_zP), (size_t)n, P_<uint32_t>(s->d_zPi)));
  KL(s, "k_pk_affine", lsgk::pk_affine(S_(s), n, P_<uint32_t>(s->d_Pp), P_<uint32_t>(s->d_zPi), P_<uint32_t>(s->d_P)));
  KL(s, "k_sig_decode", lsgk::sig_decode(S_(s), n, P_<uint8_t>(s->d_sig), P_<uint32_t>(s->d_siglen),
                                         P_<uint32_t>(s->d_sigaff), P_<uint8_t>(s->d_siginf), P_<int32_t>(s->d_seterr)));
  if ((size_t)n <= slp_items_max())
    KL(s, "k_slp_subgroup", lsg_slp_g2_subgroup(S_(s), n, P_<uint32_t>(s->d_sigaff), P_<uint8_t>(s->d_siginf),
                                                P_<int32_t>(s->d_seterr)));
  else
    KL(s, "k_sig_subgroup", lsgk::sig_subgroup(S_(s), n, P_<uint32_t>(s->d_sigaff), P_<uint8_t>(s->d_siginf),
                                               P_<int32_t>(s->d_seterr)));
  if (s->n_kv)
    KL(s, "k_pk_keyvalidate_apply", lsgk::pk_keyvalidate_apply(S_(s), (int)s->n_kv, PL(s, s->kv_off + s->n_kv),
                                                               P_<int32_t>(s->d_pkp), P_<int32_t>(s->d_seterr)));
  if (Ph.agg_g >= 0) {
    const Grp& g = Ph.groups[(size_t)Ph.agg_g];
    const size_t nm = Ph.n_magg;
    LSG_RC(ensure(s, s->d_mmask, 4 * W_G1P * std::max(g.first + g.len, (size_t)1)));
    LSG_RC(ensure(s, s->d_PmP, 4 * W_G1P * nm));
    LSG_RC(ensure(s, s->d_Pm, 4 * W_G1A * nm));
    LSG_RC(ensure(s, s->d_pinfm, nm));
    LSG_RC(ensure(s, s->d_errm, 4 * nm));
    KL(s, "k_pk_mask", lsgk::pk_mask(S_(s), (int)(g.first + g.len), P_<uint32_t>(s->d_Pp), P_<int32_t>(s->d_seterr),
                                     P_<uint8_t>(s->d_pinf), P_<uint32_t>(s->d_mmask)));
    LSG_RC(run_seg(s, 0, "msg_pk_sums", s->msum, P_<uint32_t>(s->d_mmask), P_<uint32_t>(s->d_PmP)));
    KL(s, "k_g1p_affine_inv", lsgk::g1p_affine_inv(S_(s), (int)nm, P_<uint32_t>(s->d_PmP), P_<uint32_t>(s->d_Pm),
                                                   P_<uint8_t>(s->d_pinfm)));
    LSG_HIP(s, hipMemsetAsync(s->d_errm.p, 0, 4 * nm, s->st[1]));
  }
  LSG_HIP(s, hipEventRecord(s->ev_sig, s->st[1]));
  s->cur = 0;
  const int nm = (int)s->n_msgs;
  if (s->msg_objs)
    KL(s, "k_msg_roots", lsgk::msg_roots(S_(s), nm, P_<uint8_t>(s->d_msg), P_<uint32_t>(s->d_msgoff),
                                         P_<uint32_t>(s->d_msglen)));
  KL(s, "k_expand_msg", lsgk::expand_msg(S_(s), nm, P_<uint8_t>(s->d_msg), P_<uint32_t>(s->d_msgoff),
                                         P_<uint32_t>(s->d_msglen), P_<uint8_t>(s->d_dst), DST_POP_LEN,
                                         P_<uint8_t>(s->d_ub)));
  if (s->msg_dedup) {
    LSG_RC(ensure(s, s->d_Hm, 4 * W_G2A * (size_t)nm));
    LSG_RC(ensure(s, s->d_hinfm, (size_t)nm));
    LSG_RC(launch_hash(s, nm, P_<uint32_t>(s->d_Hm), P_<uint8_t>(s->d_hinfm)));
    KL(s, "k_h2c_gather", lsgk::h2c_gather(S_(s), n, P_<uint32_t>(s->d_mid), P_<uint32_t>(s->d_Hm),
                                           P_<uint8_t>(s->d_hinfm), P_<uint32_t>(s->d_H), P_<uint8_t>(s->d_hinf)));
  } else {
    LSG_RC(launch_hash(s, n, P_<uint32_t>(s->d_H), P_<uint8_t>(s->d_hinf)));
  }
  if (!miller_fused())
    KL(s, "k_miller_lines", lsgk::miller_lines(S_(s), n, P_<uint32_t>(s->d_H), P_<uint32_t>(s->d_lines)));
  LSG_HIP(s, hipStreamWaitEvent(s->st[0], s->ev_sig, 0));
  if (n_items) LSG_RC(launch_accum(s, n_items, item_off, fall));
  if (Ph.agg_g >= 0)
    KL(s, "k_slp_items_msg",
       lsg_slp_miller_items1(S_(s), (int)Ph.n_magg, PL(s, Ph.magg_off), P_<uint32_t>(s->d_Pm), P_<uint8_t>(s->d_pinfm),
                             P_<uint8_t>(s->d_hinfm), P_<int32_t>(s->d_errm), P_<uint32_t>(s->d_Hm),
                             fall + (size_t)lsgl::W_F12 * Ph.n_set_items));
  return LSG_OK;
}

SegPlan plan_pk_agg(Slot* s) {
  std::vector<int32_t> off(s->n_sets), len(s->n_sets);
  for (size_t i = 0; i < s->n_sets; i++) {
    off[i] = (int32_t)s->shape.pk_first[i];
    len[i] = (int32_t)s->shape.pk_cnt[i];
  }
  return slot_seg(s, 0, off, len, false, 0, 0);
}

AggPlan plan_agg_tree(Slot* s) {
  AggPlan P;
  P.tree = true;
  const size_t n = s->n_sets;
  auto tree_cost = [](int64_t len, int L) {
    const int64_t A = (int64_t)1 << L;
    return ((len + A - 1) / A) * A * 7 + ((len + A - 1) / A) * 11;
  };
  int64_t best = -1;
  for (int L = 0; L <= 9; L++) {
    int64_t cost = 0;
    for (size_t i = 0; i < n; i++) {
      const int64_t len = (int64_t)s->shape.pk_cnt[i];
      cost += L > 0 ? std::min(tree_cost(len, L), len * 11) : len * 11;
    }
    if (best < 0 || cost < best) {
      best = cost;
      P.L = L;
    }
  }
  const int64_t A = (int64_t)1 << P.L;
  P.T = (int)std::max<long>(1, std::min<long>(64, lsg_ab_long("LSG_AGG_T", 8)));
  std::vector<int32_t> o0(n, 0), src(3 * n);
  int64_t N0 = 0;
  for (size_t i = 0; i < n; i++) {
    const int64_t len = (int64_t)s->shape.pk_cnt[i];
    if (P.L > 0 && tree_cost(len, P.L) < len * 11) {
      o0[i] = (int32_t)N0;
      src[3 * i] = 0;
      src[3 * i + 1] = (int32_t)(N0 >> P.L);
      src[3 * i + 2] = (int32_t)((len + A - 1) / A);
      N0 += (len + A - 1) / A * A;
    } else {
      src[3 * i] = 1;
      src[3 * i + 1] = (int32_t)s->shape.pk_first[i];
      src[3 * i + 2] = (int32_t)len;
    }
  }
  P.N0 = N0;
  if (N0 == 0) P.L = 0;
  if (P.L > 0) {
    const int64_t unit = (int64_t)LSG_ITEMS_PER_BLOCK_HOST << (P.L - 1);
    const int64_t need = (N0 / 2 + P.T - 1) / P.T;
    P.n_c0 = (need + unit - 1) / unit * unit;
    P.blk_off = s->plan.size();
    s->plan.resize(P.blk_off + (size_t)(N0 >> P.L));
    int32_t* blk = s->plan.data() + P.blk_off;
    for (size_t i = 0; i < n; i++)
      if (src[3 * i] == 0)
        for (int32_t b = src[3 * i + 1], e = b + src[3 * i + 2]; b < e; b++) blk[b] = (int32_t)i;
  }
  P.o0_off = s->plan.size();
  s->plan.insert(s->plan.end(), o0.begin(), o0.end());
  P.len_off = s->plan.size();
  for (size_t i = 0; i < n; i++) s->plan.push_back((int32_t)s->shape.pk_cnt[i]);
  P.pk0_off = s->plan.size();
  for (size_t i = 0; i < n; i++) s->plan.push_back((int32_t)s->shape.pk_first[i]);
  P.src_off = s->plan.size();
  s->plan.insert(s->plan.end(), src.begin(), src.end());
  return P;
}

int launch_agg_tree(Slot* s, const AggPlan& P, uint32_t* agg) {
  Dev* d = s->d;
  lsgk::AggTreeArgs a;
  a.L = P.L;
  a.T = P.T;
  a.n_c0 = P.n_c0;
  a.N0 = P.N0;
  a.blk_set = PL(s, P.blk_off);
  a.set_o0 = PL(s, P.o0_off);
  a.set_len = PL(s, P.len_off);
  a.set_pk0 = PL(s, P.pk0_off);
  a.pk = P_<uint8_t>(s->d_pk);
  a.stride = s->pk_stride;
  a.pk_len = P_<uint32_t>(s->d_pklen);
  a.pk_err = P_<int32_t>(s->d_pkerr);
  a.tab = P_<uint32_t>(d->d_pktab);
  a.tab_ok = P_<uint8_t>(d->d_pktab_ok);
  a.tab_n = (uint32_t)d->pktab_n;
  if (P.L > 0) {
    const size_t npts = (size_t)(2 * P.N0), pre_w = W_FP * (size_t)(P.T * P.n_c0), cinv_w = W_FP * (size_t)P.n_c0;
    LSG_RC(ensure(s, s->d_agga, 4 * W_G1A * npts));
    LSG_RC(ensure(s, s->d_aggi, npts));
    LSG_RC(ensure(s, s->d_aggpre, 4 * 2 * pre_w));
    LSG_RC(ensure(s, s->d_aggtot, 4 * 2 * cinv_w));
    LSG_RC(ensure(s, s->d_aggflag, 2 * (size_t)P.n_c0));
    a.pts = P_<uint32_t>(s->d_agga);
    a.inf = P_<uint8_t>(s->d_aggi);
    a.pre[0] = P_<uint32_t>(s->d_aggpre);
    a.pre[1] = a.pre[0] + pre_w;
    a.cinv[0] = P_<uint32_t>(s->d_aggtot);
    a.cinv[1] = a.cinv[0] + cinv_w;
    a.flag[0] = P_<uint8_t>(s->d_aggflag);
    a.flag[1] = a.flag[0] + P.n_c0;
    KL(s, "g1_aggregate", lsgk::agg_leaf(S_(s), a));
    for (int t = 0; t < P.L; t++) KL(s, "g1_aggregate", lsgk::agg_step(S_(s), a, t));
  }
  KL(s, "g1_aggregate", lsgk::agg_final(S_(s), a, (int)s->n_sets, PL(s, P.src_off), agg));
  return LSG_OK;
}

int launch_readback(Slot* s, bool status) {
  hipStream_t S = s->st[0];
  const size_t n = s->n_sets, np = s->n_pks;
  if (s->own_streams) {
    LSG_HIP(s, hipEventRecord(s->ev_grp, s->st[1]));
    LSG_HIP(s, hipStreamWaitEvent(S, s->ev_grp, 0));
  }
  if (status) {
    if (n) {
      LSG_HIP(s, hipMemcpyAsync(s->h_err.p, s->d_seterr.p, 4 * n, hipMemcpyDeviceToHost, S));
      LSG_HIP(s, hipMemcpyAsync(s->h_pinf.p, s->d_pinf.p, n, hipMemcpyDeviceToHost, S));
    }
    if (np) LSG_HIP(s, hipMemcpyAsync(s->h_pkerr.p, s->d_pkerr.p, 4 * np, hipMemcpyDeviceToHost, S));
  }
  LSG_HIP(s, hipEventRecord(s->ev_done, S));
  return LSG_OK;
}

SetStatus read_status(Slot* s) {
  SetStatus ss;
  const size_t n = s->n_sets;
  ss.err = H_<int32_t>(s->h_err);
  ss.pkerr = H_<int32_t>(s->h_pkerr);
  ss.pinf.assign(H_<uint8_t>(s->h_pinf), H_<uint8_t>(s->h_pinf) + n);
  for (size_t i = 0; i < n; i++)
    if (s->shape.pk_cnt[i] == 0 && !(i < s->shape.bits_p.size() && s->shape.bits_p[i] > 0))
      ss.pinf[i] = 2;
  return ss;
}

}

namespace {

const uint8_t* fp12_one_blob() {
  static uint8_t b[576] = {0};
  b[47] = 1;
  return b;
}

int launch_sig_prep(Slot* s, bool scale, const std::vector<uint8_t>* mode, uint32_t* out) {
  const int n = (int)s->n_sets;
  if (n == 0) return LSG_OK;
  s->cur = 1;
  const uint8_t* dm = nullptr;
  if (scale && mode) {
    LSG_RC(ensure_host(s, s->h_mode, (size_t)n));
    LSG_RC(ensure(s, s->d_mode, (size_t)n));
    memcpy(s->h_mode.p, mode->data(), (size_t)n);
    LSG_HIP(s, hipMemcpyAsync(s->d_mode.p, s->h_mode.p, (size_t)n, hipMemcpyHostToDevice, s->st[1]));
    dm = P_<uint8_t>(s->d_mode);
  }
  if (scale && (size_t)n <= slp_items_max()) {
    KL(s, "k_sig_prep", lsgk::sig_prep(S_(s), n, P_<uint32_t>(s->d_sigaff), P_<uint8_t>(s->d_siginf),
                                       P_<int32_t>(s->d_seterr), P_<uint8_t>(s->d_pinf), nullptr, nullptr, out));
    KL(s, "k_slp_g2_scale", lsg_slp_g2_scale(S_(s), n, P_<uint32_t>(s->d_sigaff), P_<uint8_t>(s->d_siginf),
                                             P_<int32_t>(s->d_seterr), P_<uint8_t>(s->d_pinf), P_<uint64_t>(s->d_rnd),
                                             dm, out));
    return LSG_OK;
  }
  KL(s, "k_sig_prep", lsgk::sig_prep(S_(s), n, P_<uint32_t>(s->d_sigaff), P_<uint8_t>(s->d_siginf),
                                     P_<int32_t>(s->d_seterr), P_<uint8_t>(s->d_pinf),
                                     scale ? P_<uint64_t>(s->d_rnd) : nullptr, dm, out));
  return LSG_OK;
}

int pkg_part1(Slot* s, const lsg_job* jobs, const std::vector<size_t>& ids, uint64_t seed, int n_node,
              const std::vector<size_t>* subs = nullptr, bool lone_ok = true, const uint8_t* dev_msgs = nullptr) {
  timer_reset(s);
  s->plan.clear();
  memset(&s->stats, 0, sizeof(s->stats));
  s->stats.start_ns = now_ns();
  const size_t nj = ids.size();
  s->results.assign(nj, lsg_job_result{LSG_INVALID, 0});
  s->rs2_ready = false;
  s->rs2_scaled.clear();
  s->has_node = n_node > 0;
  s->big_fe_pending = false;
  s->seed = seed;
  s->resolved = s->resolving = false;
  s->resolve_rc = LSG_OK;
  std::vector<const lsg_set*> flat(shape_jobs(s->shape, jobs, ids, subs));
  for (size_t k = 0; k < nj; k++)
    for (uint32_t q = 0; q < jobs[ids[k]].n_sets; q++) flat[s->shape.jobs[k].first + q] = &jobs[ids[k]].sets[q];
  if (subs) {
    lsg_stats z;
    memset(&z, 0, sizeof(z));
    s->sub_stats.assign(s->shape.n_sub, z);
    s->sub_pkfail.assign(s->shape.n_sub, 0);
    s->sub_done.assign(s->shape.n_sub, 0);
  }
  s->K = miller_k_for(flat.size());
  s->sw = read_switches();
  s->gp = plan_groups(s->shape, s->sw, lone_ok);
  const uint64_t th0 = trace_host() ? now_ns() : 0;
  LSG_RC(stage_sets(s, flat.data(), flat.size(), seed, true, &s->gp.noscale, dev_msgs == nullptr, true));
  if (dev_msgs && !flat.empty())
    LSG_HIP(s, hipMemcpyAsync(s->d_msg.p, dev_msgs, 32 * flat.size(), hipMemcpyDeviceToDevice, s->st[0]));
  s->n_kv = 0;
  s->shape.kv_set.clear();
  bool any_kv = false;
  for (size_t k = 0; k < nj && !any_kv; k++) any_kv = (s->shape.jobs[k].flags & LSG_JOB_VALIDATE_KEYS) != 0;
  if (any_kv) {
    s->shape.kv_set.assign(flat.size(), 0);
    for (size_t k = 0; k < nj; k++) {
      if (!(s->shape.jobs[k].flags & LSG_JOB_VALIDATE_KEYS)) continue;
      for (size_t i = s->shape.jobs[k].first; i < s->shape.jobs[k].first + s->shape.jobs[k].count; i++)
        if (flat[i]->pk_len != LSG_PK_INDEX && flat[i]->pk_len != LSG_PK_BITS && s->shape.pk_cnt[i]) {
          s->shape.kv_set[i] = 1;
          s->n_kv += s->shape.pk_cnt[i];
        }
    }
    s->kv_off = s->plan.size();
    s->plan.resize(s->kv_off + 2 * s->n_kv);
    size_t q = 0;
    for (size_t i = 0; i < flat.size(); i++)
      for (uint32_t k = 0; s->shape.kv_set[i] && k < s->shape.pk_cnt[i]; k++, q++) {
        s->plan[s->kv_off + q] = (int32_t)(s->shape.pk_first[i] + k);
        s->plan[s->kv_off + s->n_kv + q] = (int32_t)i;
      }
    if (!s->n_kv) s->shape.kv_set.clear();
  }
  const uint64_t th1 = trace_host() ? now_ns() : 0;
  PhasePlan& A = s->phA;
  A = PhasePlan();
  A.groups = s->gp.groups;
  A.sub = s->gp.sub;
  size_t n_msm = 0;
  while (n_msm < A.groups.size() && A.groups[n_msm].msm) n_msm++;
  LSG_RC(size_state(s, s->n_sets, s->n_pks, A.groups.size(), n_msm, 1));
  s->agg = AggPlan();
  if (!s->single_keys && !s->pk_all_bits) {
    if (s->n_pks >= AGG_TREE_MIN_KEYS && agg_tree_on() && s->bits_sets.empty())
      s->agg = plan_agg_tree(s);
    else
      s->pkagg = plan_pk_agg(s);
  }
  s->bplan = plan_bits(s->plan, s->bits_sets);
  A.agg_g = -1;
  if (s->msg_dedup && !s->gp.chunk_mode && s->gp.big_g >= 0 && s->sw.msg_agg && s->n_msgs <= (size_t)8192 &&
      s->sw.slp_items > 0) {
    const Grp& g = A.groups[(size_t)s->gp.big_g];
    std::vector<int32_t> cnt(s->n_msgs, 0), off(s->n_msgs), fill;
    for (size_t i = g.first; i < g.first + g.len; i++) cnt[s->msg_id[i]]++;
    int32_t tot = 0;
    for (size_t j = 0; j < s->n_msgs; j++) {
      off[j] = tot;
      tot += cnt[j];
    }
    fill = off;
    const size_t idx_off = s->plan.size();
    s->plan.resize(idx_off + (size_t)tot);
    for (size_t i = g.first; i < g.first + g.len; i++) s->plan[idx_off + (size_t)fill[s->msg_id[i]]++] = (int32_t)i;
    s->msum = slot_seg(s, 0, off, cnt, true, idx_off, 0);
    A.agg_g = s->gp.big_g;
    A.n_magg = s->n_msgs;
  }
  plan_phase(s->plan, s->rnd, s->K, s->sw, A);
  group_items(s->gp, s->shape, A);
  SegPlan node;
  if (n_node > 0) {
    std::vector<int32_t> off{0}, len{(int32_t)n_node};
    node = slot_seg(s, 2, off, len, false, 0, 0);
  }
  LSG_RC(upload_plan(s));
  const uint64_t th2 = trace_host() ? now_ns() : 0;
  LSG_RC(launch_set_stages(s, &s->pkagg, A, P_<uint32_t>(s->d_fall)));
  const uint64_t th3 = trace_host() ? now_ns() : 0;
  s->rs_raw.assign(s->n_sets, 0);
  for (size_t g = 0; g < A.n_msm; g++) memset(s->rs_raw.data() + A.groups[g].first, 1, A.groups[g].len);
  if (!A.groups.empty()) {
    const bool any_small = A.n_msm < A.groups.size();
    std::vector<uint8_t> mode;
    if (any_small && A.n_msm) {
      mode.assign(s->n_sets, 0);
      for (size_t g = A.n_msm; g < A.groups.size(); g++)
        memset(mode.data() + A.groups[g].first, 1, A.groups[g].len);
    }
    LSG_RC(launch_sig_prep(s, any_small, mode.empty() ? nullptr : &mode, P_<uint32_t>(s->d_rs)));
  }
  LSG_RC(launch_phase(s, A, P_<uint32_t>(s->d_rs), P_<uint32_t>(s->d_fall), true));
  if (A.groups.empty() || s->gp.big_g < 0) {
    s->cur = 0;
    LSG_HIP(s, hipMemcpyAsync(P_<uint8_t>(s->d_gath) + 576 * LSG_MAX_DEVICES, fp12_one_blob(), 576,
                              hipMemcpyHostToDevice, s->st[0]));
    LSG_HIP(s, hipEventRecord(s->ev_part, s->st[0]));
  }
  s->phA_node = node;
  if (trace_host()) {
    const uint64_t th4 = now_ns();
    fprintf(stderr, "lsg host: sets %zu jobs %zu subs %d groups %zu | stage %.3f plan %.3f set-launch %.3f group-launch %.3f ms\n",
            (size_t)s->n_sets, nj, s->shape.n_sub, A.groups.size(), (th1 - th0) * 1e-6, (th2 - th1) * 1e-6, (th3 - th2) * 1e-6,
            (th4 - th3) * 1e-6);
  }
  return LSG_OK;
}

const uint8_t* pkg_partial_dev(Slot* s) {
  if (s->phA.groups.empty() || s->gp.big_g < 0) return P_<uint8_t>(s->d_gath) + 576 * LSG_MAX_DEVICES;
  return P_<uint8_t>(s->d_Fb) + 576 * (size_t)s->gp.big_g;
}

int export_partial_dev(Slot* s, const uint8_t** src, hipStream_t xs = nullptr) {
  *src = pkg_partial_dev(s);
  if (!s->gp.lone_unscaled) return LSG_OK;
  uint64_t r = 0;
  if (s->seed) {
    uint64_t sd = s->seed ^ 0x5851f42d4c957f2dull;
    do r = splitmix64(sd);
    while (r == 0);
  } else {
    do {
      if (!os_random(&r, 8)) {
        set_err(s->d->c, "no entropy for the exported partial's randomizer (getrandom failed)");
        return LSG_ERR_ENTROPY;
      }
    } while (r == 0);
  }
  LSG_RC(ensure(s, s->d_xport, 576));
  s->cur = 0;
  if (xs) {
    const hipError_t e = lsgk::fp12_pow_u64(xs, *src, r, P_<uint8_t>(s->d_xport));
    if (e != hipSuccess) return fail(s, "k_fp12_pow", e);
  } else {
    KL(s, "k_fp12_pow", lsgk::fp12_pow_u64(S_(s), *src, r, P_<uint8_t>(s->d_xport)));
  }
  *src = P_<uint8_t>(s->d_xport);
  return LSG_OK;
}

int pkg_node_check(Slot* s, int n) {
  s->cur = 0;
  const uint32_t* nf = P_<uint32_t>(s->d_nodeF);
  KL(s, "k_blobs_to_fp12", lsgk::blobs_to_fp12(S_(s), n, P_<uint8_t>(s->d_gath), P_<uint32_t>(s->d_nodeF)));
  LSG_RC(run_seg(s, 2, "fp12_product", s->phA_node, nf, P_<uint32_t>(s->d_nodeF) + W_F12 * (size_t)n));
  uint8_t* blob = P_<uint8_t>(s->d_gath) + 576 * (size_t)(LSG_MAX_DEVICES + 1);
  KL(s, "k_fp12_to_canon", lsgk::fp12_to_canon(S_(s), 1, P_<uint32_t>(s->d_nodeF) + W_F12 * (size_t)n, blob));
  KL(s, SERIAL_LABEL(final_exp), lsg_row_final_exp(S_(s), 1, blob, P_<int32_t>(s->d_nodeV)));
  LSG_HIP(s, hipMemcpyAsync(s->h_nodeV.p, s->d_nodeV.p, 4, hipMemcpyDeviceToHost, s->st[0]));
  LSG_HIP(s, hipEventRecord(s->ev_node, s->st[0]));
  return LSG_OK;
}

int pkg_part2(Slot* s, bool skip_big = false) {
  const size_t ng = s->phA.groups.size();
  s->big_fe_pending = skip_big && !s->gp.chunk_mode && s->gp.big_g >= 0;
  if (s->big_fe_pending) {
    LSG_RC(launch_fe_range(s, 0, (size_t)s->gp.big_g));
    LSG_RC(launch_fe_range(s, (size_t)s->gp.big_g + 1, ng));
  } else {
    LSG_RC(launch_fe(s, ng));
  }
  return launch_readback(s, true);
}

typedef std::unique_lock<std::mutex> CtxLock;

int run_fallback_phase(Slot* s, CtxLock* lk, const std::vector<Grp>& groups,
                       const std::vector<std::pair<int32_t, int32_t>>* given, std::vector<int32_t>& v) {
  v.assign(groups.size(), 0);
  if (groups.empty()) return LSG_OK;
  const uint64_t tf0 = trace_host() ? now_ns() : 0;
  std::vector<size_t> order;
  std::vector<uint8_t> gm(groups.size(), 0);
  for (size_t g = 0; g < groups.size(); g++) {
    bool ok = groups[g].len >= std::max(s->sw.msm_min_group, (size_t)2) && s->rs_raw.size() == s->n_sets;
    for (size_t i = groups[g].first; ok && i < groups[g].first + groups[g].len; i++) ok = s->rs_raw[i] != 0;
    gm[g] = ok;
    if (ok) order.push_back(g);
  }
  const size_t n_msm = order.size();
  for (size_t g = 0; g < groups.size(); g++)
    if (!gm[g]) order.push_back(g);
  LSG_RC(size_state(s, s->n_sets, s->n_pks, groups.size(), n_msm, 2));
  s->cur = 0;
  s->plan.clear();
  PhasePlan Ph;
  for (size_t k = 0; k < order.size(); k++) {
    Ph.groups.push_back(groups[order[k]]);
    Ph.groups.back().msm = gm[order[k]] != 0;
  }
  size_t singles = 0;
  for (auto& g : groups) singles += g.len == 1 ? 1 : 0;
  const int K = !given && 2 * singles >= groups.size() ? 1 : s->K;
  if (given) {
    Ph.reuse_items = true;
    for (size_t k = 0; k < order.size(); k++) Ph.given.push_back((*given)[order[k]]);
    Ph.n_items = s->phA.n_items;
    Ph.term_base = s->phA.n_items + s->phA.groups.size();
  }
  plan_phase(s->plan, s->rnd, K, s->sw, Ph);
  LSG_RC(upload_plan(s));
  if (s->rs2_scaled.size() != s->n_sets) s->rs2_scaled.assign(s->n_sets, 0);
  std::vector<uint8_t> mode(s->n_sets, 0);
  bool any = false;
  for (size_t g = 0; g < groups.size(); g++) {
    if (gm[g]) continue;
    for (size_t i = groups[g].first; i < groups[g].first + groups[g].len; i++)
      if (!s->rs2_scaled[i]) {
        mode[i] = s->rs2_scaled[i] = 1;
        any = true;
      }
  }
  LSG_HIP(s, hipEventRecord(s->ev_in, s->st[0]));
  LSG_HIP(s, hipStreamWaitEvent(s->st[1], s->ev_in, 0));
  if (any) {
    s->cur = 1;
    const int n = (int)s->n_sets;
    LSG_RC(ensure_host(s, s->h_mode, (size_t)n));
    memcpy(s->h_mode.p, mode.data(), (size_t)n);
    LSG_HIP(s, hipMemcpyAsync(s->d_mode.p, s->h_mode.p, (size_t)n, hipMemcpyHostToDevice, s->st[1]));
    size_t n_scaled = 0;
    for (uint8_t m : mode) n_scaled += m;
    if (slp_items_max() > 0 && n_scaled <= 8192)
      KL(s, "k_slp_g2_scale", lsg_slp_g2_scale(S_(s), n, P_<uint32_t>(s->d_sigaff), P_<uint8_t>(s->d_siginf),
                                               P_<int32_t>(s->d_seterr), P_<uint8_t>(s->d_pinf), P_<uint64_t>(s->d_rnd),
                                               P_<uint8_t>(s->d_mode), P_<uint32_t>(s->d_rs2)));
    else
      KL(s, "k_sig_scale", lsgk::sig_scale_only(S_(s), n, P_<uint32_t>(s->d_sigaff), P_<uint8_t>(s->d_siginf),
                                                P_<int32_t>(s->d_seterr), P_<uint8_t>(s->d_pinf), P_<uint64_t>(s->d_rnd),
                                                P_<uint8_t>(s->d_mode), P_<uint32_t>(s->d_rs2)));
  }
  s->cur = 0;
  uint32_t* fall = given ? P_<uint32_t>(s->d_fall) : P_<uint32_t>(s->d_fall2);
  if (!given) LSG_RC(launch_accum(s, Ph.n_items, Ph.item_off, fall, Ph.single_items));
  LSG_RC(launch_phase(s, Ph, P_<uint32_t>(s->d_rs2), fall, false, P_<uint32_t>(s->d_rs)));
  LSG_RC(launch_fe(s, groups.size()));
  LSG_RC(launch_readback(s, false));
  const uint64_t tf1 = trace_host() ? now_ns() : 0;
  const int dev = s->d->device;
  if (lk) lk->unlock();
  hipError_t e = event_wait(s->ev_done);
// ... 1608 lines not shown
  }
  static const uint8_t zero32[32] = {0};
  std::vector<lsg_set> sets(n);
  std::vector<lsg_job> jobs(n);
  for (size_t i = 0; i < n; i++) {
    const uint8_t* dd = data184 + 184 * i;
    sets[i].pks = dd;
    sets[i].pk_len = 48;
    sets[i].n_pks = 1;
    sets[i].msg = resident ? zero32 : host_roots.data() + 32 * i;
    sets[i].msg_len = 32;
    sets[i].sig = dd + 88;
    sets[i].sig_len = 96;
    jobs[i].sets = &sets[i];
    jobs[i].n_sets = 1;
    jobs[i].flags = LSG_JOB_BATCHABLE | LSG_JOB_VALIDATE_KEYS;
  }
  constexpr size_t DEPOSIT_PKG = 8192, DEPOSIT_INFLIGHT = 4;
  struct Out {
    lsg_ticket t;
    size_t first, count;
  };
  std::vector<Out> out;
  std::vector<lsg_job_result> res(std::min(n, DEPOSIT_PKG));
  int rc = LSG_OK;
  auto wait_oldest = [&]() {
    const Out o = out.front();
    out.erase(out.begin());
    const int w = lsg_wait_jobs(c, o.t, res.data(), nullptr);
    if (w) return w;
    for (size_t k = 0; k < o.count; k++) {
      valid[o.first + k] = res[k].status == LSG_VALID ? 1 : 0;
      err[o.first + k] = res[k].status == LSG_ERROR ? res[k].err_code : 0;
    }
    return (int)LSG_OK;
  };
  size_t pkg = 0;
  for (size_t o = 0; o < n && !rc; pkg++) {
    const size_t cnt = std::min(DEPOSIT_PKG, n - o);
    lsg_ticket t = 0;
    if (out.size() >= DEPOSIT_INFLIGHT) {
      rc = wait_oldest();
      pkg--;
      continue;
    }
    {
      CtxLock lk(c->mu);
      const hipError_t he = hipSetDevice(d->device);
      if (he != hipSuccess)
        rc = fail_c(c, "hipSetDevice", he);
      else
        rc = submit_pkg(c, lk, jobs.data() + o, cnt, seed ? seed + 0x9e3779b97f4a7c15ull * pkg : 0, &t, true,
                        resident ? P_<uint8_t>(d->d_dep_roots) + 32 * o : nullptr);
    }
    if (rc == LSG_ERR_BUSY && !out.empty()) {
      rc = wait_oldest();
      pkg--;
      continue;
    }
    if (rc) break;
    out.push_back({t, o, cnt});
    o += cnt;
  }
  while (!out.empty()) {
    const int w = wait_oldest();
    if (!rc) rc = w;
  }
  return rc;
}

int lsg_sign(lsg_ctx* c, const uint8_t* sks32, const uint8_t* msgs, uint32_t msg_len, size_t n, uint8_t* out96) {
  if (!c || !out96 || (n && (!sks32 || !msgs)) || msg_marked(msg_len)) return LSG_ERR_INVALID_ARG;
  LSG_ENTER(c);
  Slot* s = &c->dev[0]->util;
  timer_reset(s);
  if (n == 0) return LSG_OK;
  LSG_RC(util_hash(s, msgs, msg_len, n, DST_POP, DST_POP_LEN));
  LSG_RC(ensure(s, s->d_aux, 96 * n));
  LSG_RC(ensure(s, s->d_Fb, 32 * n));
  LSG_HIP(s, hipMemcpyAsync(s->d_Fb.p, sks32, 32 * n, hipMemcpyHostToDevice, s->st[0]));
  KL(s, "k_sign", lsgk::sign(S_(s), (int)n, P_<uint8_t>(s->d_Fb), P_<uint32_t>(s->d_H), P_<uint8_t>(s->d_aux)));
  LSG_HIP(s, hipMemcpyAsync(out96, s->d_aux.p, 96 * n, hipMemcpyDeviceToHost, s->st[0]));
  LSG_HIP(s, hipStreamSynchronize(s->st[0]));
  return LSG_OK;
}

int lsg_sk_to_pk(lsg_ctx* c, const uint8_t* sks32, size_t n, uint8_t* out96) {
  if (!c || !out96 || (n && !sks32)) return LSG_ERR_INVALID_ARG;
  LSG_ENTER(c);
  Slot* s = &c->dev[0]->util;
  timer_reset(s);
  if (n == 0) return LSG_OK;
  LSG_RC(ensure(s, s->d_aux, 96 * n));
  LSG_RC(ensure(s, s->d_Fb, 32 * n));
  LSG_HIP(s, hipMemcpyAsync(s->d_Fb.p, sks32, 32 * n, hipMemcpyHostToDevice, s->st[0]));
  KL(s, "k_sk_to_pk", lsgk::sk_to_pk(S_(s), (int)n, P_<uint8_t>(s->d_Fb), P_<uint8_t>(s->d_aux)));
  LSG_HIP(s, hipMemcpyAsync(out96, s->d_aux.p, 96 * n, hipMemcpyDeviceToHost, s->st[0]));
  LSG_HIP(s, hipStreamSynchronize(s->st[0]));
  return LSG_OK;
}

int lsg_check_fp2_mul(lsg_ctx* c, const uint32_t* in, size_t n, uint32_t* out) {
  if (!c || (n && (!in || !out)) || n > 0x7fffffffull / (4 * W_FP)) return LSG_ERR_INVALID_ARG;
  LSG_ENTER(c);
  if (n == 0) return LSG_OK;
  Slot* s = &c->dev[0]->util;
  timer_reset(s);
  LSG_RC(ensure(s, s->d_aux, 4 * 4 * W_FP * n));
  LSG_RC(ensure(s, s->d_Fb, 4 * 2 * W_FP * n));
  LSG_HIP(s, hipMemcpyAsync(s->d_aux.p, in, 4 * 4 * W_FP * n, hipMemcpyHostToDevice, s->st[0]));
  KL(s, "k_check_fp2_mul", lsgk::check_fp2_mul(S_(s), (int)n, P_<uint32_t>(s->d_aux), P_<uint32_t>(s->d_Fb)));
  LSG_HIP(s, hipMemcpyAsync(out, s->d_Fb.p, 4 * 2 * W_FP * n, hipMemcpyDeviceToHost, s->st[0]));
  LSG_HIP(s, hipStreamSynchronize(s->st[0]));
  return LSG_OK;
}

static int check_sqr(lsg_ctx* c, const uint32_t* in, size_t n, uint32_t* out, int E) {
  if (!c || (n && (!in || !out)) || n > 0x7fffffffull / (4 * W_FP)) return LSG_ERR_INVALID_ARG;
  LSG_ENTER(c);
  if (n == 0) return LSG_OK;
  Slot* s = &c->dev[0]->util;
  timer_reset(s);
  const size_t bytes = 4 * (size_t)E * W_FP * n;
  LSG_RC(ensure(s, s->d_aux, bytes));
  LSG_RC(ensure(s, s->d_Fb, bytes));
  LSG_HIP(s, hipMemcpyAsync(s->d_aux.p, in, bytes, hipMemcpyHostToDevice, s->st[0]));
  if (E == 1)
    KL(s, "k_check_fp_sqr", lsgk::check_fp_sqr(S_(s), (int)n, P_<uint32_t>(s->d_aux), P_<uint32_t>(s->d_Fb)));
  else
    KL(s, "k_check_fp2_sqr", lsgk::check_fp2_sqr(S_(s), (int)n, P_<uint32_t>(s->d_aux), P_<uint32_t>(s->d_Fb)));
  LSG_HIP(s, hipMemcpyAsync(out, s->d_Fb.p, bytes, hipMemcpyDeviceToHost, s->st[0]));
  LSG_HIP(s, hipStreamSynchronize(s->st[0]));
  return LSG_OK;
}
int lsg_check_fp_sqr(lsg_ctx* c, const uint32_t* in, size_t n, uint32_t* out) { return check_sqr(c, in, n, out, 1); }
int lsg_check_fp2_sqr(lsg_ctx* c, const uint32_t* in, size_t n, uint32_t* out) { return check_sqr(c, in, n, out, 2); }

int lsg_check_sums(lsg_ctx* c, const uint32_t* in, size_t n, uint32_t* out) {
  constexpr size_t EIN = 12, EOUT = 42;
  if (!c || (n && (!in || !out)) || n > 0x7fffffffull / (4 * W_FP * EOUT)) return LSG_ERR_INVALID_ARG;
  LSG_ENTER(c);
  if (n == 0) return LSG_OK;
  Slot* s = &c->dev[0]->util;
  timer_reset(s);
  LSG_RC(ensure(s, s->d_aux, 4 * EIN * W_FP * n));
  LSG_RC(ensure(s, s->d_Fb, 4 * EOUT * W_FP * n));
  LSG_HIP(s, hipMemcpyAsync(s->d_aux.p, in, 4 * EIN * W_FP * n, hipMemcpyHostToDevice, s->st[0]));
  KL(s, "k_check_sums", lsgk::check_sums(S_(s), (int)n, P_<uint32_t>(s->d_aux), P_<uint32_t>(s->d_Fb)));
  LSG_HIP(s, hipMemcpyAsync(out, s->d_Fb.p, 4 * EOUT * W_FP * n, hipMemcpyDeviceToHost, s->st[0]));
  LSG_HIP(s, hipStreamSynchronize(s->st[0]));
  return LSG_OK;
}

int lsg_probe_fp_mul_rate(lsg_ctx* c, double* fp_mul_per_s, double* mad_per_s) {
  if (!c || !fp_mul_per_s || !mad_per_s) return LSG_ERR_INVALID_ARG;
  LSG_ENTER(c);
  Slot* s = &c->dev[0]->util;
  hipDeviceProp_t prop;
  LSG_HIP(s, hipGetDeviceProperties(&prop, c->dev[0]->device));
  const int items = prop.multiProcessorCount * 32 * 32;
  LSG_RC(ensure(s, s->d_aux, 4 * W_FP * (size_t)items));
  std::vector<uint32_t> init(W_FP * (size_t)items, 0);
  for (size_t i = 0; i < init.size(); i += 4) init[i] = (uint32_t)(i * 2654435761u) & 0x1fffffffu;
  LSG_HIP(s, hipMemcpy(s->d_aux.p, init.data(), 4 * init.size(), hipMemcpyHostToDevice));
  const int iters = 64;
  hipStream_t S = s->st[0];
  LSG_HIP(s, lsgk::probe_fp_mul(S, items, 2, P_<uint32_t>(s->d_aux)));
  hipEvent_t a, b;
  LSG_HIP(s, hipEventCreate(&a));
  LSG_HIP(s, hipEventCreate(&b));
  LSG_HIP(s, hipEventRecord(a, S));
  LSG_HIP(s, lsgk::probe_fp_mul(S, items, iters, P_<uint32_t>(s->d_aux)));
  LSG_HIP(s, hipEventRecord(b, S));
  LSG_HIP(s, hipEventSynchronize(b));
  float ms = 0;
  LSG_HIP(s, hipEventElapsedTime(&ms, a, b));
  (void)hipEventDestroy(a);
  (void)hipEventDestroy(b);
  *fp_mul_per_s = (double)items * iters * 4.0 / (ms * 1e-3);
  *mad_per_s = *fp_mul_per_s * 300.0;
  return LSG_OK;
}

int lsg_probe_mad_peak(lsg_ctx* c, double* mad_per_s) {
  if (!c || !mad_per_s) return LSG_ERR_INVALID_ARG;
  LSG_ENTER(c);
  Slot* s = &c->dev[0]->util;
  hipDeviceProp_t prop;
  LSG_HIP(s, hipGetDeviceProperties(&prop, c->dev[0]->device));
  const int blocks = prop.multiProcessorCount * 32;
  const size_t threads = (size_t)blocks * 256;
  LSG_RC(ensure(s, s->d_aux, 8 * threads));
  hipStream_t S = s->st[0];
  const int iters = 4096;
  LSG_HIP(s, lsgk::probe_mad(S, blocks, 16, 3u, P_<uint64_t>(s->d_aux)));
  hipEvent_t a, b;
  LSG_HIP(s, hipEventCreate(&a));
  LSG_HIP(s, hipEventCreate(&b));
  LSG_HIP(s, hipEventRecord(a, S));
  LSG_HIP(s, lsgk::probe_mad(S, blocks, iters, 5u, P_<uint64_t>(s->d_aux)));
  LSG_HIP(s, hipEventRecord(b, S));
  LSG_HIP(s, hipEventSynchronize(b));
  float ms = 0;
  LSG_HIP(s, hipEventElapsedTime(&ms, a, b));
  (void)hipEventDestroy(a);
  (void)hipEventDestroy(b);
  *mad_per_s = (double)threads * iters * 16.0 / (ms * 1e-3);
  return LSG_OK;
}

int lsg_last_kernel_times(lsg_ctx* c, const char** names, double* ms, int max) {
  if (!c) return 0;
  std::lock_guard<std::mutex> lk(c->mu);
  const auto& v = c->dev[0]->last_times;
  int n = 0;
  for (size_t i = 0; i < v.size() && n < max; i++, n++) {
    if (names) names[n] = v[i].first;
    if (ms) ms[n] = v[i].second;
  }
  return n;
}

int lsg_assign_jobs(const uint32_t* job_sets, size_t n_jobs, int32_t n_devices, int32_t* owner) {
  if ((n_jobs && (!job_sets || !owner)) || n_devices < 1) return LSG_ERR_INVALID_ARG;
  assign_jobs(job_sets, n_jobs, n_devices, owner);
  return LSG_OK;
}

}
```

lodestar_amd/csrc/lsg_k_reduce.hip:

```cpp
#include "lsg_kcommon.hpp"
namespace {
#include "lsg_inv.hpp"
}

template <int OP>
struct seg_op;
template <>
struct seg_op<0> {
  typedef g1p_t T;
  static LSG_DEVI T ident() { return proj_inf<fp_t>(); }
  static LSG_DEVI T op(const T& a, const T& b) { return g1_add(a, b); }
};
template <>
struct seg_op<1> {
  typedef g2p_t T;
  static LSG_DEVI T ident() { return proj_inf<fp2_t>(); }
  static LSG_DEVI T op(const T& a, const T& b) { return g2_add(a, b); }
};
template <>
struct seg_op<2> {
  typedef fp12_t T;
  static LSG_DEVI T ident() { return fp12_one(); }
  static LSG_DEVI T op(const T& a, const T& b) { return fp12_mul(a, b); }
};

template <int OP>
__global__ void LSG_KERNEL_ATTR_W(OP == 2 ? 1 : LSG_WAVES_PER_EU)
    k_seg_reduce(int n_chunks, int ips_log2, const int32_t* __restrict__ chunks, const int32_t* __restrict__ idx,
                 const uint32_t* __restrict__ src, uint32_t* __restrict__ dst, uint32_t* __restrict__ tmp) {
  typedef seg_op<OP> O;
  typedef typename O::T T;
  lsg_lane_setup();
#if LSG_RED_PRIO
  __builtin_amdgcn_s_setprio(LSG_RED_PRIO);
#endif
  const size_t item = gtid() / LSG_GROUP;
  const size_t c = item >> ips_log2;
  const int ips = 1 << ips_log2, j = (int)(item & (size_t)(ips - 1));
  const bool active = c < (size_t)n_chunks;
  T acc = O::ident();
  int out = 0;
  if (active) {
    const int off = chunks[3 * c], len = chunks[3 * c + 1];
    out = chunks[3 * c + 2];
    if (j < len) {
      acc = lane_load<T>(src, idx ? (size_t)idx[off + j] : (size_t)(off + j));
#pragma unroll 1
      for (int k = j + ips; k < len; k += ips) acc = O::op(acc, lane_load<T>(src, idx ? (size_t)idx[off + k] : (size_t)(off + k)));
    }
  }
#pragma unroll 1
  for (int o = ips >> 1; o >= 1; o >>= 1) acc = O::op(acc, shfl_xor_t(acc, LSG_GROUP * o));
  if (active && j == 0) {
    if (out >= 0)
      lane_store(dst, (size_t)out, acc);
    else
      lane_store(tmp, (size_t)(-out - 1), acc);
  }
}

__global__ void LSG_KERNEL_ATTR k_binv_fold(int n, int zero_to_one, const uint32_t* __restrict__ in,
                                            uint32_t* __restrict__ pre, uint32_t* __restrict__ tot) {
  const int n_chunks = (n + LSG_BINV_T - 1) / LSG_BINV_T;
  LANE_ITEM(n_chunks);
  (void)lead;
  const fp_t one = fp_one();
  const int first = (int)item * LSG_BINV_T, last = min(n, first + LSG_BINV_T);
  fp_t acc = one;
#pragma unroll 1
  for (int k = first; k < last; k++) {
    fp_t x = lane_load<fp_t>(in, k);
    if (zero_to_one) x = fp_select(fp_is_zero(x), one, x);
    acc = k == first ? x : fp_mul(acc, x);
    lane_store(pre, k, acc);
  }
  lane_store(tot, item, acc);
}
__global__ void LSG_KERNEL_ATTR k_binv_root(const uint32_t* __restrict__ top, uint32_t* __restrict__ inv) {
  LANE_ITEM(1);
  (void)lead;
  const fp_t d = pair_inv_gcd(pair_canon(lane_load<fp_t>(top, 0)));
  lane_store(inv, 0, pair_mont_mul(d, fp_t(FP_RCUBE)));
}
__global__ void LSG_KERNEL_ATTR k_binv_unfold(int n, int zero_to_one, const uint32_t* __restrict__ in,
                                              const uint32_t* __restrict__ pre, const uint32_t* __restrict__ tinv,
                                              uint32_t* __restrict__ out) {
  const int n_chunks = (n + LSG_BINV_T - 1) / LSG_BINV_T;
  LANE_ITEM(n_chunks);
  (void)lead;
  const fp_t one = fp_one();
  const int first = (int)item * LSG_BINV_T, last = min(n, first + LSG_BINV_T);
  fp_t acc = lane_load<fp_t>(tinv, item);
#pragma unroll 1
  for (int k = last - 1; k >= first; k--) {
    fp_t x = lane_load<fp_t>(in, k);
    const bool z = zero_to_one && fp_is_zero(x);
    fp_t r = k > first ? fp_mul(acc, lane_load<fp_t>(pre, k - 1)) : acc;
    lane_store(out, k, z ? fp_zero() : r);
    if (k > first && !z) acc = fp_mul(acc, x);
  }
}

__global__ void LSG_KERNEL_ATTR k_binv_block(int n, int T, int zero_to_one, const uint32_t* __restrict__ in,
                                             uint32_t* __restrict__ pre, uint32_t* __restrict__ out) {
  __shared__ uint32_t H[2 * LSG_ITEMS_PER_BLOCK * lsgl::W_FP], I[2 * LSG_ITEMS_PER_BLOCK * lsgl::W_FP];
  lsg_lane_setup();
#if LSG_RED_PRIO
  __builtin_amdgcn_s_setprio(LSG_RED_PRIO);
#endif
  const int l = (int)(threadIdx.x / LSG_GROUP);
  const int64_t first = ((int64_t)blockIdx.x * LSG_ITEMS_PER_BLOCK + l) * T;
  const int64_t last = first + T < (int64_t)n ? first + T : (int64_t)n;
  const fp_t one = fp_one();
  fp_t acc = one;
#pragma unroll 1
  for (int64_t k = first; k < last; k++) {
    fp_t x = lane_load<fp_t>(in, (size_t)k);
    if (zero_to_one) x = fp_select(fp_is_zero(x), one, x);
    acc = k == first ? x : fp_mul(acc, x);
    if (T > 1) lane_store(pre, (size_t)k, acc);
  }
  fp_t inv = block_inv<LSG_ITEMS_PER_BLOCK>(H, I, l, acc);
#pragma unroll 1
  for (int64_t k = last - 1; k >= first; k--) {
    const fp_t x = lane_load<fp_t>(in, (size_t)k);
    const bool z = zero_to_one && fp_is_zero(x);
    const fp_t r = k > first ? fp_mul(inv, lane_load<fp_t>(pre, (size_t)k - 1)) : inv;
    lane_store(out, (size_t)k, z ? fp_zero() : r);
    if (k > first && !z) inv = fp_mul(inv, x);
  }
}

__global__ void LSG_KERNEL_ATTR k_blobs_to_fp12(int n, const uint8_t* __restrict__ blobs, uint32_t* __restrict__ out) {
  LANE_ITEM(n);
  (void)lead;
  lane_store(out, item, fp12_from_canon_bytes(blobs + 576 * item));
}
__global__ void LSG_KERNEL_ATTR k_fp12_to_canon(int n, const uint32_t* __restrict__ in, uint8_t* __restrict__ out) {
  LANE_ITEM(n);
  (void)lead;
  fp12_to_canon_bytes(out + 576 * item, lane_load<fp12_t>(in, item));
}

__global__ void LSG_KERNEL_ATTR_W(1) k_fp12_pow_u64(const uint8_t* __restrict__ in576, uint64_t r,
                                                    uint8_t* __restrict__ out576) {
  LANE_ITEM(1);
  (void)lead;
  const fp12_t f = fp12_from_canon_bytes(in576);
  fp12_t acc = f;
  int top = 63;
  while (top > 0 && !((r >> top) & 1u)) top--;
#pragma unroll 1
  for (int b = top - 1; b >= 0; b--) {
    acc = fp12_sqr<false>(acc);
    if ((r >> b) & 1u) acc = fp12_mul<false>(acc, f);
  }
  fp12_to_canon_bytes(out576, acc);
}

__global__ void LSG_KERNEL_ATTR k_check_fp2_mul(int n, const uint32_t* __restrict__ in, uint32_t* __restrict__ out) {
  LANE_ITEM(n);
  (void)lead;
  const fp2_t a(lane_load<fp_t>(in, 4 * item), lane_load<fp_t>(in, 4 * item + 1));
  const fp2_t b(lane_load<fp_t>(in, 4 * item + 2), lane_load<fp_t>(in, 4 * item + 3));
  const fp2_t c = fp2_mul(a, b);
  lane_store(out, 2 * item, c.c0);
  lane_store(out, 2 * item + 1, c.c1);
}
__global__ void LSG_KERNEL_ATTR k_check_fp_sqr(int n, const uint32_t* __restrict__ in, uint32_t* __restrict__ out) {
  LANE_ITEM(n);
  (void)lead;
  lane_store(out, item, fp_sqr(lane_load<fp_t>(in, item)));
}
__global__ void LSG_KERNEL_ATTR k_check_fp2_sqr(int n, const uint32_t* __restrict__ in, uint32_t* __restrict__ out) {
  LANE_ITEM(n);
  (void)lead;
  const fp2_t c = fp2_sqr(fp2_t(lane_load<fp_t>(in, 2 * item), lane_load<fp_t>(in, 2 * item + 1)));
  lane_store(out, 2 * item, c.c0);
  lane_store(out, 2 * item + 1, c.c1);
}
template <class F>
LSG_DEVI jac_t<F> check_jac_dbl_nested(const jac_t<F>& p) {
  F A = fsqr(p.X), B = fsqr(p.Y), C = fsqr(B);
  F D = fsub(fsqr(fadd(p.X, B)), fadd(A, C));
  D = fadd(D, D);
  F E = fadd(fadd(A, A), A);
  F Fq = fsqr(E);
  jac_t<F> r;
  r.X = fsub(Fq, fadd(D, D));
  F C8 = fadd(C, C);
  C8 = fadd(C8, C8);
  C8 = fadd(C8, C8);
  r.Y = fsub(fmul(E, fsub(D, r.X)), C8);
  F yz = fmul(p.Y, p.Z);
  r.Z = fadd(yz, yz);
  return r;
}
LSG_DEVI fp2_t check_b3_nested(const fp2_t& a) {
  auto m12 = [](const fp_t& x) {
    const fp_t x4 = fp_dbl(fp_dbl(x));
    return fp_add(fp_dbl(x4), x4);
  };
  return fp2_t(m12(fp_sub(a.c0, a.c1)), m12(fp_add(a.c0, a.c1)));
}
LSG_DEVI g2p_t check_proj_add_nested(const g2p_t& p, const g2p_t& q) {
  typedef fp2_t F;
  F t0 = fmul(p.X, q.X), t1 = fmul(p.Y, q.Y), t2 = fmul(p.Z, q.Z);
  F t3 = fmul(fadd(p.X, p.Y), fadd(q.X, q.Y));
  F t4 = fadd(t0, t1);
  t3 = fsub(t3, t4);
  t4 = fmul(fadd(p.Y, p.Z), fadd(q.Y, q.Z));
  F X3 = fadd(t1, t2);
  t4 = fsub(t4, X3);
  X3 = fmul(fadd(p.X, p.Z), fadd(q.X, q.Z));
  F Y3 = fadd(t0, t2);
  Y3 = fsub(X3, Y3);
  X3 = fadd(t0, t0);
  t0 = fadd(X3, t0);
  t2 = check_b3_nested(t2);
  F Z3 = fadd(t1, t2);
  t1 = fsub(t1, t2);
  Y3 = check_b3_nested(Y3);
  X3 = fmul(t4, Y3);
  t2 = fmul(t3, t1);
  X3 = fsub(t2, X3);
  Y3 = fmul(Y3, t0);
  t1 = fmul(t1, Z3);
  Y3 = fadd(t1, Y3);
  t0 = fmul(t0, t3);
  Z3 = fmul(Z3, t4);
  Z3 = fadd(Z3, t0);
  return g2p_t{X3, Y3, Z3};
}
constexpr int LSG_CHECK_SUMS_IN = 12, LSG_CHECK_SUMS_OUT = 42;
__global__ void LSG_KERNEL_ATTR k_check_sums(int n, const uint32_t* __restrict__ in, uint32_t* __restrict__ out) {
  LANE_ITEM(n);
  (void)lead;
  const size_t ring = (size_t)LSG_CHECK_SUMS_IN * (size_t)n;
  auto el = [&](int j) { return lane_load<fp_t>(in, ((size_t)LSG_CHECK_SUMS_IN * item + (size_t)j) % ring); };
  auto el2 = [&](int j) { return fp2_t(el(2 * j), el(2 * j + 1)); };
  int o = 0;
  auto put = [&](const fp_t& v) { lane_store(out, (size_t)LSG_CHECK_SUMS_OUT * item + (size_t)(o++), v); };
  auto put2 = [&](const fp2_t& v) {
    put(v.c0);
    put(v.c1);
  };
  const fp_t a = el(0), b = el(1), c = el(2);
  put((fps(a) + b + c - el(3) - el(4) - el(5)).carry());
  put(fp_mulk<2>(a));
  put(fp_mulk<3>(a));
  put(fp_mulk<4>(a));
  put(fp_mulk<8>(a));
  put(fp_mulk<12>(a));
  put2(fp2_mul_b3(fp2_t(a, b)));
  const jac_t<fp_t> j1 = {a, b, c};
  const jac_t<fp_t> r1 = jac_dbl(j1), n1 = check_jac_dbl_nested(j1);
  put(r1.X), put(r1.Y), put(r1.Z);
  put(n1.X), put(n1.Y), put(n1.Z);
  const jac_t<fp2_t> j2 = {el2(0), el2(1), el2(2)};
  const jac_t<fp2_t> r2 = jac_dbl(j2), n2 = check_jac_dbl_nested(j2);
  put2(r2.X), put2(r2.Y), put2(r2.Z);
  put2(n2.X), put2(n2.Y), put2(n2.Z);
  const g2p_t p = {el2(0), el2(1), el2(2)}, q = {el2(3), el2(4), el2(5)};
  const g2p_t r3 = g2_add(p, q), n3 = check_proj_add_nested(p, q);
  put2(r3.X), put2(r3.Y), put2(r3.Z);
  put2(n3.X), put2(n3.Y), put2(n3.Z);
  put2(mfc_mul<3>(el2));
  const fp2_t t2c = fp2_add(el2(11), fp2_mul_xi(fp2_sub(fp2_sub(el2(15), el2(12)), el2(13))));
  const fp2_t t0c = fp2_add(el2(0), fp2_mul_xi(fp2_sub(fp2_sub(el2(4), el2(1)), el2(2))));
  put2(fp2_sub(fp2_sub(t2c, t0c), fp2_mul_xi(fp2_add(el2(7), el2(9)))));
}

__global__ void LSG_KERNEL_ATTR k_probe_fp_mul(int n, int iters, uint32_t* __restrict__ io) {
  LANE_ITEM(n);
  (void)lead;
  fp_t a = lane_load<fp_t>(io, item), b = fp_t(FP_R2), c = fp_t(FP_R3), d = fp_t(FP_HALF);
  for (int k = 0; k < iters; k++) {
    a = fp_mul(a, b);
    b = fp_mul(b, c);
    c = fp_mul(c, d);
    d = fp_mul(d, a);
  }
  lane_store(io, item, fp_add(fp_add(a, b), fp_add(c, d)));
}

__global__ void __launch_bounds__(256) k_probe_mad(int iters, uint32_t seed, uint64_t* __restrict__ io) {
  const uint32_t t = blockIdx.x * blockDim.x + threadIdx.x;
  uint64_t acc[16];
  uint32_t x[16];
#pragma unroll
  for (int k = 0; k < 16; k++) {
    acc[k] = t + k;
    x[k] = (t * 2654435761u) ^ (seed + 977u * k);
  }
  const uint32_t y = seed | 1u;
  for (int i = 0; i < iters; i++) {
#pragma unroll
    for (int k = 0; k < 16; k++) acc[k] = (uint64_t)x[k] * y + acc[k];
  }
  uint64_t r = 0;
#pragma unroll
  for (int k = 0; k < 16; k++) r ^= acc[k];
  io[t] = r;
}

namespace lsgk {
hipError_t seg_reduce(hipStream_t st, int op, int n_chunks, int ips_log2, const int32_t* chunks, const int32_t* idx,
                      const uint32_t* src, uint32_t* dst, uint32_t* tmp) {
  const size_t items = (size_t)n_chunks << ips_log2;
  if (op == 0) LSG_LAUNCH_ITEMS(k_seg_reduce<0>, items, st, n_chunks, ips_log2, chunks, idx, src, dst, tmp);
  if (op == 1) LSG_LAUNCH_ITEMS(k_seg_reduce<1>, items, st, n_chunks, ips_log2, chunks, idx, src, dst, tmp);
  LSG_LAUNCH_ITEMS(k_seg_reduce<2>, items, st, n_chunks, ips_log2, chunks, idx, src, dst, tmp);
}
hipError_t binv_fold(hipStream_t st, int n, int zero_to_one, const uint32_t* in, uint32_t* pre, uint32_t* tot) {
  LSG_LAUNCH_ITEMS(k_binv_fold, (n + LSG_BINV_T - 1) / LSG_BINV_T, st, n, zero_to_one, in, pre, tot);
}
hipError_t binv_block(hipStream_t st, int n, int T, int zero_to_one, const uint32_t* in, uint32_t* pre, uint32_t* out) {
  if (n <= 0) return hipSuccess;
  const size_t chunks = ((size_t)n + T - 1) / T;
  hipLaunchKernelGGL(k_binv_block, dim3(lane_blocks(chunks)), dim3(LSG_TPB), 0, st, n, T, zero_to_one, in, pre, out);
  return hipGetLastError();
}
hipError_t binv_root(hipStream_t st, const uint32_t* top, uint32_t* inv) {
  LSG_LAUNCH_ITEMS(k_binv_root, 1, st, top, inv);
}
hipError_t binv_unfold(hipStream_t st, int n, int zero_to_one, const uint32_t* in, const uint32_t* pre,
                       const uint32_t* tinv, uint32_t* out) {
  LSG_LAUNCH_ITEMS(k_binv_unfold, (n + LSG_BINV_T - 1) / LSG_BINV_T, st, n, zero_to_one, in, pre, tinv, out);
}
hipError_t blobs_to_fp12(hipStream_t st, int n, const uint8_t* blobs, uint32_t* out) {
  LSG_LAUNCH_ITEMS(k_blobs_to_fp12, n, st, n, blobs, out);
}
hipError_t fp12_to_canon(hipStream_t st, int n, const uint32_t* in, uint8_t* out576) {
  LSG_LAUNCH_ITEMS(k_fp12_to_canon, n, st, n, in, out576);
}
hipError_t fp12_pow_u64(hipStream_t st, const uint8_t* in576, uint64_t r, uint8_t* out576) {
  LSG_LAUNCH_ITEMS(k_fp12_pow_u64, 1, st, in576, r, out576);
}
hipError_t check_fp2_mul(hipStream_t st, int n, const uint32_t* in, uint32_t* out) {
  LSG_LAUNCH_ITEMS(k_check_fp2_mul, n, st, n, in, out);
}
hipError_t check_fp_sqr(hipStream_t st, int n, const uint32_t* in, uint32_t* out) {
  LSG_LAUNCH_ITEMS(k_check_fp_sqr, n, st, n, in, out);
}
hipError_t check_fp2_sqr(hipStream_t st, int n, const uint32_t* in, uint32_t* out) {
  LSG_LAUNCH_ITEMS(k_check_fp2_sqr, n, st, n, in, out);
}
hipError_t check_sums(hipStream_t st, int n, const uint32_t* in, uint32_t* out) {
  LSG_LAUNCH_ITEMS(k_check_sums, n, st, n, in, out);
}
hipError_t probe_fp_mul(hipStream_t st, int items, int iters, uint32_t* io) {
  LSG_LAUNCH_ITEMS(k_probe_fp_mul, items, st, items, iters, io);
}
hipError_t probe_mad(hipStream_t st, int blocks, int iters, uint32_t seed, uint64_t* io) {
  if (blocks <= 0) return hipSuccess;
  hipLaunchKernelGGL(k_probe_mad, dim3(blocks), dim3(256), 0, st, iters, seed, io);
  return hipGetLastError();
}
}
```

lodestar_amd/csrc/lsg_k_sig.hip:

```cpp
#include "lsg_kcommon.hpp"

__global__ void LSG_KERNEL_ATTR k_sig_decode(int n, const uint8_t* __restrict__ sig, const uint32_t* __restrict__ sig_len,
                                             uint32_t* __restrict__ sig_aff, uint8_t* __restrict__ inf,
                                             int32_t* __restrict__ err) {
  LANE_ITEM(n);
  uint32_t len = sig_len[item];
  g2a_t p;
  p.x = fp2_zero();
  p.y = fp2_zero();
  bool is_inf = false;
  int e;
  if (len == 96)
    e = g2_uncompress(p, is_inf, sig + 192 * item);
  else if (len == 192)
    e = g2_deserialize_uncompressed(p, is_inf, sig + 192 * item);
  else
    e = LSG_BLST_INVALID_SIZE;
  lane_store(sig_aff, item, p);
  if (lead) {
    inf[item] = is_inf ? 1 : 0;
    err[item] = e;
  }
}

__global__ void LSG_KERNEL_ATTR k_sig_subgroup(int n, const uint32_t* __restrict__ sig_aff,
                                               const uint8_t* __restrict__ inf, int32_t* __restrict__ err) {
  __shared__ uint32_t park[sizeof(g2a_t) / 4 * LSG_TPB];
  LANE_ITEM(n);
  if (err[item] != 0 || inf[item]) return;
  lds_park(park, lane_load<g2a_t>(sig_aff, item));
  bool ok = g2_in_group_get([&]() { return proj_from_aff(lds_unpark<g2a_t>(park)); });
  if (lead && !ok) err[item] = LSG_BLST_POINT_NOT_IN_GROUP;
}

LSG_DEVI bool sig_usable(size_t i, const uint8_t* inf, const int32_t* err, const uint8_t* pinf) {
  return err[i] == 0 && !inf[i] && !(pinf && pinf[i]);
}
__global__ void LSG_KERNEL_ATTR k_sig_proj(int n, const uint32_t* __restrict__ sig_aff, const uint8_t* __restrict__ inf,
                                           const int32_t* __restrict__ err, const uint8_t* __restrict__ pinf,
                                           uint32_t* __restrict__ out) {
  LANE_ITEM(n);
  (void)lead;
  g2p_t r = proj_inf<fp2_t>();
  if (sig_usable(item, inf, err, pinf)) r = proj_from_aff(lane_load<g2a_t>(sig_aff, item));
  lane_store(out, item, r);
}
__global__ void LSG_KERNEL_ATTR_W(1) k_sig_scale3(int n, const uint32_t* __restrict__ sig_aff, const uint8_t* __restrict__ inf,
                                                  const int32_t* __restrict__ err, const uint8_t* __restrict__ pinf,
                                                  const uint64_t* __restrict__ rnd, const uint8_t* __restrict__ mode,
                                                  uint32_t* __restrict__ out) {
  LANE_ITEM(n);
  (void)lead;
  if (mode && !mode[item]) return;
  g2p_t r = proj_inf<fp2_t>();
  if (sig_usable(item, inf, err, pinf)) {
    r = proj_from_aff(lane_load<g2a_t>(sig_aff, item));
    if (rnd[item] != 0) r = proj_mul_u64_s3(r, rnd[item]);
  }
  lane_store(out, item, r);
}

__global__ void LSG_KERNEL_ATTR k_g2a_to_bytes(int n, const uint32_t* __restrict__ pts, const uint8_t* __restrict__ inf,
                                               uint8_t* __restrict__ out) {
  LANE_ITEM(n);
  (void)lead;
  g2_serialize(out + 192 * item, lane_load<g2a_t>(pts, item), inf[item] != 0);
}

__global__ void LSG_KERNEL_ATTR k_g2p_compress(int n, const uint32_t* __restrict__ pts, uint8_t* __restrict__ out96) {
  LANE_ITEM(n);
  (void)lead;
  g2p_t p = lane_load<g2p_t>(pts, item);
  bool is_inf = proj_is_inf(p);
  g2a_t a;
  if (is_inf) {
    a.x = fp2_zero();
    a.y = fp2_zero();
  } else {
    a = proj_to_aff(p);
  }
  g2_compress(out96 + 96 * item, a, is_inf);
}

__global__ void LSG_KERNEL_ATTR k_g2p_to_canon(int n, const uint32_t* __restrict__ in, uint8_t* __restrict__ out) {
  LANE_ITEM(n);
  (void)lead;
  g2p_to_canon_bytes(out + 288 * item, lane_load<g2p_t>(in, item));
}

template <class F>
__device__ proj_t<F> proj_mul_be256(const proj_t<F>& p, const uint8_t* k) {
  proj_t<F> acc = proj_inf<F>();
  for (int byte = 0; byte < 32; byte++) {
    uint32_t v = k[byte];
    for (int b = 7; b >= 0; b--) {
      acc = gdbl(acc);
      proj_t<F> s = gadd(acc, p);
      bool bit = (v >> b) & 1u;
      acc.X = fselect(bit, s.X, acc.X);
      acc.Y = fselect(bit, s.Y, acc.Y);
      acc.Z = fselect(bit, s.Z, acc.Z);
    }
  }
  return acc;
}

__global__ void LSG_KERNEL_ATTR k_sign(int n, const uint8_t* __restrict__ sks, const uint32_t* __restrict__ H,
                                       uint8_t* __restrict__ out96) {
  LANE_ITEM(n);
  (void)lead;
  g2p_t s = proj_mul_be256(proj_from_aff(lane_load<g2a_t>(H, item)), sks + 32 * item);
  bool is_inf = proj_is_inf(s);
  g2a_t a;
  if (is_inf) {
    a.x = fp2_zero();
    a.y = fp2_zero();
  } else {
    a = proj_to_aff(s);
  }
  g2_compress(out96 + 96 * item, a, is_inf);
}

namespace lsgk {
hipError_t sig_decode(hipStream_t st, int n, const uint8_t* sig, const uint32_t* sig_len, uint32_t* sig_aff,
                      uint8_t* inf, int32_t* err) {
  LSG_LAUNCH_ITEMS(k_sig_decode, n, st, n, sig, sig_len, sig_aff, inf, err);
}
hipError_t sig_subgroup(hipStream_t st, int n, const uint32_t* sig_aff, const uint8_t* inf, int32_t* err) {
  LSG_LAUNCH_ITEMS(k_sig_subgroup, n, st, n, sig_aff, inf, err);
}
hipError_t sig_prep(hipStream_t st, int n, const uint32_t* sig_aff, const uint8_t* inf, const int32_t* err,
                    const uint8_t* pinf, const uint64_t* rnd, const uint8_t* mode, uint32_t* out) {
  if (n <= 0) return hipSuccess;
  if (!rnd || mode) {
    hipLaunchKernelGGL(k_sig_proj, dim3(lane_blocks((size_t)n)), dim3(LSG_TPB), 0, st, n, sig_aff, inf, err, pinf, out);
    hipError_t e = hipGetLastError();
    if (e != hipSuccess || !rnd) return e;
  }
  return sig_scale_only(st, n, sig_aff, inf, err, pinf, rnd, mode, out);
}
hipError_t sig_scale_only(hipStream_t st, int n, const uint32_t* sig_aff, const uint8_t* inf, const int32_t* err,
                          const uint8_t* pinf, const uint64_t* rnd, const uint8_t* mode, uint32_t* out) {
  LSG_LAUNCH_ITEMS(k_sig_scale3, n, st, n, sig_aff, inf, err, pinf, rnd, mode, out);
}
hipError_t g2a_to_bytes(hipStream_t st, int n, const uint32_t* pts, const uint8_t* inf, uint8_t* out192) {
  LSG_LAUNCH_ITEMS(k_g2a_to_bytes, n, st, n, pts, inf, out192);
}
hipError_t g2p_compress(hipStream_t st, int n, const uint32_t* pts, uint8_t* out96) {
  LSG_LAUNCH_ITEMS(k_g2p_compress, n, st, n, pts, out96);
}
hipError_t g2p_to_canon(hipStream_t st, int n, const uint32_t* pts, uint8_t* out288) {
  LSG_LAUNCH_ITEMS(k_g2p_to_canon, n, st, n, pts, out288);
}
hipError_t sign(hipStream_t st, int n, const uint8_t* sks, const uint32_t* H, uint8_t* out96) {
  LSG_LAUNCH_ITEMS(k_sign, n, st, n, sks, H, out96);
}
}
```

lodestar_amd/csrc/lsg_kcommon.hpp:

```cpp
#pragma once
#include <hip/hip_runtime.h>
#include <stdint.h>

#include "../../include/lodestar_bls.h"
#include "lsg_launch.h"
#include "lsg_layout.h"

namespace {
#include "lsg_fp_pair.hpp"
#include "lsg_h2c.hpp"
#include "lsg_io.hpp"
#include "lsg_inv.hpp"

static_assert(lane_words<fp_t>() == lsgl::W_FP, "layout: Fp");
static_assert(lane_words<g1a_t>() == lsgl::W_G1A, "layout: G1 affine");
static_assert(lane_words<g1p_t>() == lsgl::W_G1P, "layout: G1 projective");
static_assert(lane_words<g2a_t>() == lsgl::W_G2A, "layout: G2 affine");
static_assert(lane_words<g2p_t>() == lsgl::W_G2P, "layout: G2 projective");
static_assert(lane_words<fp12_t>() == lsgl::W_F12, "layout: Fp12");
static_assert(lane_words<line_t>() == lsgl::W_LINE, "layout: line");
static_assert(ML_STEPS == lsgl::ML_STEPS, "layout: Miller steps");
}

#define LSG_TPB 256
#ifndef LSG_WAVES_PER_EU
#define LSG_WAVES_PER_EU 2
#endif
#define LSG_KERNEL_ATTR __launch_bounds__(LSG_TPB) __attribute__((amdgpu_waves_per_eu(LSG_WAVES_PER_EU)))
#define LSG_KERNEL_ATTR_W(w) __launch_bounds__(LSG_TPB) __attribute__((amdgpu_waves_per_eu(w)))
#define LSG_ITEMS_PER_BLOCK (LSG_TPB / LSG_GROUP)

template <class T>
static __device__ __forceinline__ void lds_park(uint32_t* l, const T& v) {
  constexpr int W = sizeof(T) / 4;
  uint32_t w[W];
  __builtin_memcpy(w, &v, sizeof(T));
#pragma unroll
  for (int k = 0; k < W; k++) l[k * LSG_TPB + threadIdx.x] = w[k];
}
template <class T>
static __device__ __forceinline__ T lds_unpark(const uint32_t* l) {
  constexpr int W = sizeof(T) / 4;
  uint32_t w[W];
#pragma unroll
  for (int k = 0; k < W; k++) w[k] = l[k * LSG_TPB + threadIdx.x];
  T v;
  __builtin_memcpy(&v, w, sizeof(T));
  return v;
}

template <class T>
static __device__ __forceinline__ T shfl_xor_t(const T& v, int lane_mask) {
  constexpr int W = sizeof(T) / 4;
  uint32_t w[W];
  __builtin_memcpy(w, &v, sizeof(T));
#pragma unroll
  for (int k = 0; k < W; k++) w[k] = (uint32_t)__shfl_xor((int)w[k], lane_mask, 64);
  T r;
  __builtin_memcpy(&r, w, sizeof(T));
  return r;
}

static __device__ __forceinline__ size_t gtid() { return (size_t)blockIdx.x * blockDim.x + threadIdx.x; }
#define LANE_ITEM(n)                        \
  lsg_lane_setup();                         \
  const size_t item = gtid() / LSG_GROUP;   \
  if (item >= (size_t)(n)) return;          \
  const bool lead = (threadIdx.x % LSG_GROUP) == 0

template <int G>
static __device__ __forceinline__ void heap_up(uint32_t* Hg, int leaf, const fp_t& v) {
  if (leaf >= 0) lane_store(Hg, G + leaf, v);
#pragma unroll 1
  for (int w = G / 2; w >= 1; w >>= 1) {
    __syncthreads();
    if (leaf >= 0 && leaf < w)
      lane_store(Hg, w + leaf, fp_mul(lane_load<fp_t>(Hg, 2 * (w + leaf)), lane_load<fp_t>(Hg, 2 * (w + leaf) + 1)));
  }
  __syncthreads();
}
template <int G>
static __device__ __forceinline__ void heap_down(const uint32_t* Hg, uint32_t* Ig, int leaf) {
#pragma unroll 1
  for (int w = 2; w <= G; w <<= 1) {
    __syncthreads();
    if (leaf < w) {
      const int i = w + leaf;
      lane_store(Ig, i, fp_mul(lane_load<fp_t>(Ig, i >> 1), lane_load<fp_t>(Hg, i ^ 1)));
    }
  }
  __syncthreads();
}

template <int G>
static __device__ __forceinline__ fp_t block_inv(uint32_t* H, uint32_t* I, int leaf, const fp_t& v) {
  heap_up<G>(H, leaf, v);
  if (leaf == 0) {
    const fp_t d = pair_inv_gcd(pair_canon(lane_load<fp_t>(H, 1)));
    lane_store(I, 1, pair_mont_mul(d, fp_t(FP_RCUBE)));
  }
  heap_down<G>(H, I, leaf < 0 ? G : leaf);
  return leaf >= 0 ? lane_load<fp_t>(I, G + leaf) : v;
}

static inline int lane_blocks(size_t items) { return (int)((items + LSG_ITEMS_PER_BLOCK - 1) / LSG_ITEMS_PER_BLOCK); }

#define LSG_LAUNCH_ITEMS(kern, items, st, ...)                                                      \
  do {                                                                                              \
    if ((items) <= 0) return hipSuccess;                                                            \
    hipLaunchKernelGGL(kern, dim3(lane_blocks((size_t)(items))), dim3(LSG_TPB), 0, st, __VA_ARGS__); \
    return hipGetLastError();                                                                       \
  } while (0)
```

lodestar_amd/csrc/lsg_launch.h:

```cpp
#pragma once
#include <hip/hip_runtime.h>
#include <stddef.h>
#include <stdint.h>

namespace lsgk {
hipError_t expand_msg(hipStream_t st, int n, const uint8_t* msg, const uint32_t* off, const uint32_t* len,
                      const uint8_t* dst, uint32_t dst_len, uint8_t* ub);
hipError_t h2c_prep(hipStream_t st, int n, const uint8_t* ub, uint32_t* U, uint32_t* norms);
hipError_t h2c_map(hipStream_t st, int n, const uint32_t* U, const uint32_t* ninv, uint32_t* Hp);
hipError_t h2c_clear(hipStream_t st, int n, uint32_t* Hp, uint32_t* zN, uint8_t* hinf);
hipError_t h2c_gather(hipStream_t st, int n, const uint32_t* mid, const uint32_t* Hm, const uint8_t* hinfm, uint32_t* H,
                      uint8_t* hinf);
hipError_t h2c_affine(hipStream_t st, int n, const uint32_t* Hp, const uint32_t* ninv, const uint8_t* hinf,
                      uint32_t* H);
hipError_t signing_root(hipStream_t st, int n, const uint8_t* roots, const uint8_t* domains, uint32_t dstride,
                        uint8_t* out32);
hipError_t attestation_signing_root(hipStream_t st, int n, const uint8_t* data, const uint8_t* domains,
                                    uint32_t dstride, uint8_t* out32);
hipError_t deposit_signing_root(hipStream_t st, int n, const uint8_t* data, uint32_t stride, const uint8_t* domains,
                                uint32_t dstride, uint8_t* out32);
hipError_t object_signing_root(hipStream_t st, int n, const uint8_t* objs, uint32_t obj_len, const uint8_t* domains,
                               uint32_t dstride, uint8_t* out32);
hipError_t msg_roots(hipStream_t st, int n, uint8_t* msg, const uint32_t* off, uint32_t* len);

hipError_t sig_decode(hipStream_t st, int n, const uint8_t* sig, const uint32_t* sig_len, uint32_t* sig_aff,
                      uint8_t* inf, int32_t* err);
hipError_t sig_subgroup(hipStream_t st, int n, const uint32_t* sig_aff, const uint8_t* inf, int32_t* err);
hipError_t sig_prep(hipStream_t st, int n, const uint32_t* sig_aff, const uint8_t* inf, const int32_t* err,
                    const uint8_t* pinf, const uint64_t* rnd, const uint8_t* mode, uint32_t* out);
hipError_t sig_scale_only(hipStream_t st, int n, const uint32_t* sig_aff, const uint8_t* inf, const int32_t* err,
                          const uint8_t* pinf, const uint64_t* rnd, const uint8_t* mode, uint32_t* out);
hipError_t g2a_to_bytes(hipStream_t st, int n, const uint32_t* pts, const uint8_t* inf, uint8_t* out192);
hipError_t g2p_compress(hipStream_t st, int n, const uint32_t* pts, uint8_t* out96);
hipError_t g2p_to_canon(hipStream_t st, int n, const uint32_t* pts, uint8_t* out288);
hipError_t sign(hipStream_t st, int n, const uint8_t* sks, const uint32_t* H, uint8_t* out96);

hipError_t pk_decode(hipStream_t st, int n, const uint8_t* pk, uint32_t stride, const uint32_t* pk_len, uint32_t* pts,
                     int32_t* err, const uint32_t* tab, const uint8_t* tab_ok, uint32_t tab_n);
hipError_t pk_validate(hipStream_t st, int n, const uint8_t* pk, uint32_t len, uint32_t* pts, int32_t* err);
hipError_t pk_keyvalidate(hipStream_t st, int n, const int32_t* keys, const uint8_t* pk, const uint32_t* pk_len,
                          int32_t* code);
hipError_t pk_keyvalidate_apply(hipStream_t st, int n, const int32_t* sets, const int32_t* code, int32_t* set_err);
hipError_t pk_gather_aff(hipStream_t st, int n, const uint8_t* pk, uint32_t stride, const uint32_t* pk_len, uint32_t* pts,
                         uint8_t* inf, int32_t* err, const uint32_t* tab, const uint8_t* tab_ok, uint32_t tab_n);
hipError_t pk_agg_seg(hipStream_t st, int n_chunks, int ips_log2, const int32_t* chunks, const uint8_t* pk, uint32_t stride,
                      const uint32_t* pk_len, int32_t* err, const uint32_t* tab, const uint8_t* tab_ok, uint32_t tab_n,
                      uint32_t* dst, uint32_t* tmp);
hipError_t pk_agg_bits(hipStream_t st, int n_pairs, const int32_t* pair_set, const int32_t* plan, const uint32_t* bits,
                       const uint32_t* cm_idx, const uint32_t* cm_off, const uint32_t* cm_sum, const uint32_t* tab,
                       const uint8_t* tab_ok, uint32_t tab_n, uint32_t* dst);
struct AggTreeArgs {
  int L = 0, T = 1;
  int64_t n_c0 = 0, N0 = 0;
  const int32_t* blk_set = nullptr;
  const int32_t* set_o0 = nullptr;
  const int32_t* set_len = nullptr;
  const int32_t* set_pk0 = nullptr;
  const uint8_t* pk = nullptr;
  uint32_t stride = 0;
  const uint32_t* pk_len = nullptr;
  int32_t* pk_err = nullptr;
  const uint32_t* tab = nullptr;
  const uint8_t* tab_ok = nullptr;
  uint32_t tab_n = 0;
  uint32_t* pts = nullptr;
  uint8_t* inf = nullptr;
  uint32_t* pre[2] = {nullptr, nullptr};
  uint32_t* cinv[2] = {nullptr, nullptr};
  uint8_t* flag[2] = {nullptr, nullptr};
};
hipError_t agg_leaf(hipStream_t st, const AggTreeArgs& a);
hipError_t agg_step(hipStream_t st, const AggTreeArgs& a, int t);
hipError_t agg_final(hipStream_t st, const AggTreeArgs& a, int n_sets, const int32_t* src, uint32_t* agg);
hipError_t pk_scale(hipStream_t st, int n, const uint32_t* agg, const uint64_t* rnd, uint32_t* Pp, uint32_t* zP,
                    uint8_t* pinf);
hipError_t pk_affine(hipStream_t st, int n, const uint32_t* Pp, const uint32_t* zinv, uint32_t* P);
hipError_t pk_mask(hipStream_t st, int n, const uint32_t* Pp, const int32_t* err, const uint8_t* pinf, uint32_t* out);
hipError_t g1p_affine_inv(hipStream_t st, int n, const uint32_t* Pp, uint32_t* P, uint8_t* pinf);
hipError_t g1p_to_bytes(hipStream_t st, int n, const uint32_t* pts, uint8_t* out96);
hipError_t sk_to_pk(hipStream_t st, int n, const uint8_t* sks, uint8_t* out96);

hipError_t miller_fused(hipStream_t st, int n_items, const int32_t* item_first, const int32_t* item_cnt,
                        const uint32_t* P, const uint8_t* pinf, const uint8_t* hinf, const int32_t* err,
                        const uint32_t* H, uint32_t* f);
hipError_t miller_lines(hipStream_t st, int n, const uint32_t* H, uint32_t* lines);
hipError_t miller_lines_list(hipStream_t st, int n, const int32_t* list, const uint32_t* H, uint32_t* lines);
hipError_t miller_accum_list(hipStream_t st, int n, const int32_t* list, const uint32_t* P, const uint8_t* pinf,
                             const uint8_t* hinf, const int32_t* err, const uint32_t* lines, uint32_t* f);
hipError_t miller_accum(hipStream_t st, int K, int n_items, const int32_t* item_first, const int32_t* item_cnt,
                        const uint32_t* P, const uint8_t* pinf, const uint8_t* hinf, const int32_t* err, int n_sets,
                        const uint32_t* lines, uint32_t* f);

hipError_t seg_reduce(hipStream_t st, int op, int n_chunks, int ips_log2, const int32_t* chunks, const int32_t* idx,
                      const uint32_t* src, uint32_t* dst, uint32_t* tmp);
hipError_t binv_fold(hipStream_t st, int n, int zero_to_one, const uint32_t* in, uint32_t* pre, uint32_t* tot);
hipError_t binv_root(hipStream_t st, const uint32_t* top, uint32_t* inv);
hipError_t binv_block(hipStream_t st, int n, int T, int zero_to_one, const uint32_t* in, uint32_t* pre, uint32_t* out);
hipError_t binv_unfold(hipStream_t st, int n, int zero_to_one, const uint32_t* in, const uint32_t* pre,
                       const uint32_t* tinv, uint32_t* out);
hipError_t blobs_to_fp12(hipStream_t st, int n, const uint8_t* blobs, uint32_t* out);
hipError_t fp12_to_canon(hipStream_t st, int n, const uint32_t* in, uint8_t* out576);
hipError_t fp12_pow_u64(hipStream_t st, const uint8_t* in576, uint64_t r, uint8_t* out576);
hipError_t probe_fp_mul(hipStream_t st, int items, int iters, uint32_t* io);
hipError_t check_fp2_mul(hipStream_t st, int n, const uint32_t* in, uint32_t* out);
hipError_t check_fp_sqr(hipStream_t st, int n, const uint32_t* in, uint32_t* out);
hipError_t check_fp2_sqr(hipStream_t st, int n, const uint32_t* in, uint32_t* out);
hipError_t check_sums(hipStream_t st, int n, const uint32_t* in, uint32_t* out);
hipError_t probe_mad(hipStream_t st, int blocks, int iters, uint32_t seed, uint64_t* io);
}
```

lodestar_amd/csrc/lsg_plan.hpp:

```cpp
#pragma once
#include <stddef.h>
#include <stdint.h>

#include <string.h>

#include <algorithm>
#include <functional>
#include <utility>
#include <vector>

#include "../../include/lodestar_bls.h"
#include "lsg_bits.h"

namespace lsgp {

typedef std::pair<size_t, size_t> Range;
typedef std::pair<int32_t, int32_t> ItemRange;

inline std::vector<Range> chunkify(size_t len, size_t min_per_chunk) {
  std::vector<Range> out;
  size_t chunk_count = len / min_per_chunk;
  if (chunk_count <= 1) {
    out.push_back({0, len});
    return out;
  }
  size_t per = (len + chunk_count - 1) / chunk_count;
  for (size_t i = 0; i < len; i += per) out.push_back({i, std::min(len, i + per)});
  return out;
}

inline void assign_jobs(const uint32_t* sizes, size_t n_jobs, int n_dev, int32_t* owner) {
  uint64_t total = 0;
  for (size_t j = 0; j < n_jobs; j++) total += sizes[j];
  uint64_t before = 0;
  for (size_t j = 0; j < n_jobs; j++) {
    owner[j] = (total == 0 || n_dev <= 1) ? 0 : (int32_t)std::min<uint64_t>((uint64_t)n_dev - 1, before * (uint64_t)n_dev / total);
    before += sizes[j];
  }
}

inline int msm_window_bits(size_t n) { return n >= 256 ? 8 : (n >= 48 ? 4 : 2); }

struct SegPass {
  int ips_log2 = 0, n_chunks = 0;
  size_t chunk_off = 0;
  int src = 0;
  int tmp_out = 1;
};
struct SegPlan {
  int op = 0;
  bool has_idx = false;
  size_t idx_off = 0;
  std::vector<SegPass> passes;
  size_t tmp_items = 0;
};
constexpr int SEG_FOLD = 16;
constexpr int SEG_FOLD_FP12 = 4;
constexpr int SEG_FOLD_WIDE = 64;
constexpr size_t SEG_WIDE_PAIRS = 131072;

struct Switches {
  bool package_group = true;
  bool sub_groups = true;
  bool nb_merge = true;
  bool msg_agg = true;
  size_t msm_min_group = 256;
  size_t b0_min = 64;
  size_t b0_run = 4;
  int seg_fold_wide = SEG_FOLD_WIDE;
  size_t slp_items = 2048;
};

inline int ips_for(double avg, int32_t max_len, int fold) {
  int l = 0;
  while (l < 5 && ((int32_t)(fold << l) < max_len || (double)(2 << l) * 4.0 <= avg)) l++;
  return l;
}

inline SegPlan plan_seg(std::vector<int32_t>& A, int op, const std::vector<int32_t>& seg_off,
                        const std::vector<int32_t>& seg_len, bool has_idx, size_t idx_off, int32_t dst_base,
                        int fold_wide) {
  SegPlan P;
  P.op = op;
  P.has_idx = has_idx;
  P.idx_off = idx_off;
  const size_t ns = seg_len.size();
  if (ns == 0) return P;
  size_t total = 0;
  for (int32_t l : seg_len) total += (size_t)l;
  struct Pend {
    int32_t seg, off, len;
  };
  std::vector<Pend> cur(ns);
  for (size_t s = 0; s < ns; s++) cur[s] = {(int32_t)s, seg_off[s], seg_len[s]};
  double avg = (double)total / (double)ns;
  int src = 0, tmp_out = 1;
  while (!cur.empty()) {
    SegPass pass;
    int32_t max_len = 0;
    for (const Pend& p : cur) max_len = std::max(max_len, p.len);
    int fold = op == 2 ? SEG_FOLD_FP12 : SEG_FOLD;
    pass.ips_log2 = ips_for(avg, max_len, fold);
    if (op != 2 && (cur.size() << 5) >= SEG_WIDE_PAIRS) {
      int l = 0;
      while (l < pass.ips_log2 && (int32_t)(fold_wide << l) < max_len) l++;
      pass.ips_log2 = l;
      fold = fold_wide;
    }
    pass.src = src;
    pass.tmp_out = tmp_out;
    const int32_t cap = (int32_t)((1 << pass.ips_log2) * fold);
    pass.chunk_off = A.size();
    std::vector<Pend> nxt;
    int32_t t = 0;
    size_t nxt_total = 0;
    for (const Pend& p : cur) {
      if (p.len <= cap) {
        A.push_back(p.off);
        A.push_back(p.len);
        A.push_back(dst_base + p.seg);
        pass.n_chunks++;
      } else {
        const int32_t first = t;
        for (int32_t o = 0; o < p.len; o += cap) {
          A.push_back(p.off + o);
          A.push_back(std::min(cap, p.len - o));
          A.push_back(-(t + 1));
          t++;
          pass.n_chunks++;
        }
        nxt.push_back({p.seg, first, t - first});
        nxt_total += (size_t)(t - first);
      }
    }
    P.tmp_items = std::max(P.tmp_items, (size_t)t);
    P.passes.push_back(pass);
    avg = nxt.empty() ? 1.0 : (double)nxt_total / (double)nxt.size();
    cur.swap(nxt);
    src = tmp_out;
    tmp_out = tmp_out == 1 ? 2 : 1;
  }
  return P;
}

struct Grp {
  size_t first = 0, len = 0;
  bool msm = false;
};

struct PhasePlan {
  std::vector<Grp> groups;
  size_t n_msm = 0;
  SegPlan buckets, bits, sums, prod;
  size_t n_items = 0;
  size_t item_off = 0;
  size_t term_base = 0;
  std::vector<std::vector<Range>> sub;
  std::vector<ItemRange> sub_items;
  bool reuse_items = false;
  std::vector<ItemRange> given;
  std::vector<int32_t> it_first, it_cnt;
  bool single_items = false;
  int agg_g = -1;
  size_t n_magg = 0, magg_off = 0, n_set_items = 0;
};

inline size_t plan_items(std::vector<int32_t>& A, size_t K, const std::vector<Range>& ranges, size_t* off,
                         std::vector<ItemRange>* range_items, std::vector<int32_t>* host_first,
                         std::vector<int32_t>* host_cnt) {
  std::vector<int32_t> first, cnt;
  for (auto& r : ranges) {
    const int32_t i0 = (int32_t)first.size();
    for (size_t i = r.first; i < r.second; i += K) {
      first.push_back((int32_t)i);
      cnt.push_back((int32_t)std::min(K, r.second - i));
    }
    if (range_items) range_items->push_back({i0, (int32_t)first.size()});
  }
  *off = A.size();
  A.insert(A.end(), first.begin(), first.end());
  A.insert(A.end(), cnt.begin(), cnt.end());
  if (host_first) *host_first = first;
  if (host_cnt) *host_cnt = cnt;
  return first.size();
}

inline void plan_phase(std::vector<int32_t>& A, const std::vector<uint64_t>& rnd, int K, const Switches& sw,
                       PhasePlan& Ph) {
  const size_t ng = Ph.groups.size();
  Ph.n_msm = 0;
  while (Ph.n_msm < ng && Ph.groups[Ph.n_msm].msm) Ph.n_msm++;
  if (Ph.n_msm) {
    std::vector<int> cw(Ph.n_msm);
    std::vector<size_t> gbase(Ph.n_msm + 1, 0);
    for (size_t g = 0; g < Ph.n_msm; g++) {
      cw[g] = msm_window_bits(Ph.groups[g].len);
      gbase[g + 1] = gbase[g] + (size_t)(64 / cw[g]) * (size_t)((1u << cw[g]) - 1);
    }
    auto bucket = [&](size_t g, int w, uint32_t d) { return gbase[g] + (size_t)w * ((1u << cw[g]) - 1) + d - 1; };
    std::vector<int32_t> cnt(gbase[Ph.n_msm], 0);
    for (size_t g = 0; g < Ph.n_msm; g++) {
      const int c = cw[g], nw = 64 / c;
      const uint64_t dm = (1ull << c) - 1;
      for (size_t i = Ph.groups[g].first; i < Ph.groups[g].first + Ph.groups[g].len; i++) {
        const uint64_t r = rnd[i];
        for (int w = 0; w < nw; w++) {
          const uint32_t d = (uint32_t)((r >> (c * w)) & dm);
          if (d) cnt[bucket(g, w, d)]++;
        }
      }
    }
    std::vector<int32_t> seg_off(cnt.size()), seg_len(cnt);
    int32_t tot = 0;
    for (size_t b = 0; b < cnt.size(); b++) {
      seg_off[b] = tot;
      tot += cnt[b];
    }
    const size_t idx_off = A.size();
    A.resize(idx_off + (size_t)tot);
    int32_t* idx = A.data() + idx_off;
    std::vector<int32_t> fill(seg_off);
    for (size_t g = 0; g < Ph.n_msm; g++) {
      const int c = cw[g], nw = 64 / c;
      const uint64_t dm = (1ull << c) - 1;
      for (size_t i = Ph.groups[g].first; i < Ph.groups[g].first + Ph.groups[g].len; i++) {
        const uint64_t r = rnd[i];
        for (int w = 0; w < nw; w++) {
          const uint32_t d = (uint32_t)((r >> (c * w)) & dm);
          if (d) idx[fill[bucket(g, w, d)]++] = (int32_t)i;
        }
      }
    }
    Ph.buckets = plan_seg(A, 1, seg_off, seg_len, true, idx_off, 0, sw.seg_fold_wide);
    const size_t bidx = A.size();
    std::vector<int32_t> boff, blen;
    for (size_t g = 0; g < Ph.n_msm; g++) {
      const int c = cw[g], nw = 64 / c;
      for (int w = 0; w < nw; w++)
        for (int j = 0; j < c; j++) {
          boff.push_back((int32_t)(A.size() - bidx));
          for (uint32_t d = 1; d < (1u << c); d++)
            if ((d >> j) & 1u) A.push_back((int32_t)bucket(g, w, d));
          blen.push_back((int32_t)(A.size() - bidx) - boff.back());
        }
    }
    Ph.bits = plan_seg(A, 1, boff, blen, true, bidx, 0, sw.seg_fold_wide);
  }
  if (Ph.n_msm < ng) {
    std::vector<int32_t> off, len;
    for (size_t g = Ph.n_msm; g < ng; g++) {
      off.push_back((int32_t)Ph.groups[g].first);
      len.push_back((int32_t)Ph.groups[g].len);
    }
    Ph.sums = plan_seg(A, 1, off, len, false, 0, (int32_t)Ph.n_msm, sw.seg_fold_wide);
  }
  std::vector<ItemRange> gi;
  if (Ph.reuse_items) {
    gi = Ph.given;
  } else {
    std::vector<Range> ranges;
    std::vector<size_t> nsub(ng, 1);
    for (size_t g = 0; g < ng; g++) {
      if ((int)g == Ph.agg_g) {
        nsub[g] = 0;
      } else if (g < Ph.sub.size() && !Ph.sub[g].empty()) {
        ranges.insert(ranges.end(), Ph.sub[g].begin(), Ph.sub[g].end());
        nsub[g] = Ph.sub[g].size();
      } else {
        ranges.push_back({Ph.groups[g].first, Ph.groups[g].first + Ph.groups[g].len});
      }
    }
    Ph.sub_items.clear();
    Ph.n_items = plan_items(A, (size_t)K, ranges, &Ph.item_off, &Ph.sub_items, &Ph.it_first, &Ph.it_cnt);
    Ph.single_items = true;
    for (int32_t c : Ph.it_cnt) Ph.single_items = Ph.single_items && c == 1;
    Ph.n_set_items = Ph.n_items;
    if (Ph.agg_g >= 0) {
      Ph.magg_off = A.size();
      for (size_t j = 0; j < Ph.n_magg; j++) A.push_back((int32_t)j);
      for (size_t j = 0; j < Ph.n_magg; j++) A.push_back(1);
      Ph.n_items += Ph.n_magg;
    }
    Ph.term_base = Ph.n_items;
    size_t r = 0;
    for (size_t g = 0; g < ng; g++) {
      if ((int)g == Ph.agg_g) {
        gi.push_back({(int32_t)Ph.n_set_items, (int32_t)Ph.n_items});
        continue;
      }
      gi.push_back({Ph.sub_items[r].first, Ph.sub_items[r + nsub[g] - 1].second});
      r += nsub[g];
    }
  }
  const size_t pidx = A.size();
  std::vector<int32_t> poff, plen;
  for (size_t g = 0; g < ng; g++) {
    poff.push_back((int32_t)(A.size() - pidx));
    for (int32_t it = gi[g].first; it < gi[g].second; it++) A.push_back(it);
    A.push_back((int32_t)(Ph.term_base + g));
    plen.push_back((int32_t)(A.size() - pidx) - poff.back());
  }
  Ph.prod = plan_seg(A, 2, poff, plen, true, pidx, 0, sw.seg_fold_wide);
}

inline uint32_t msg_bytes(uint32_t msg_len) { return msg_len & ~LSG_MSG_OBJECT; }
inline bool msg_marked(uint32_t msg_len) { return (msg_len & LSG_MSG_OBJECT) != 0; }
inline uint32_t msg_object_kind(uint32_t msg_len) {
  if (!msg_marked(msg_len)) return 0;
  switch (msg_bytes(msg_len)) {
    case 40: return 8;
    case 48: return 16;
    case 64: return 32;
    case 108: return 76;
    case 120: return 88;
    case 144: return 112;
    case 160: return 128;
    default: return 0;
  }
}
inline bool msg_set_ok(const lsg_set& t) { return !msg_marked(t.msg_len) || (t.msg && msg_object_kind(t.msg_len)); }
inline bool msg_sets_ok(const lsg_set* sets, size_t n) {
  for (size_t i = 0; i < n; i++)
    if (!msg_set_ok(sets[i])) return false;
  return true;
}
inline bool msg_jobs_ok(const lsg_job* jobs, size_t n_jobs) {
  for (size_t j = 0; j < n_jobs; j++)
    if (jobs[j].n_sets && jobs[j].sets && !msg_sets_ok(jobs[j].sets, jobs[j].n_sets)) return false;
  return true;
}

struct JobRec {
  size_t first = 0, count = 0;
  uint32_t flags = 0;
};

struct PkgShape {
  std::vector<JobRec> jobs;
  std::vector<size_t> job_ids;
  std::vector<size_t> batch_order;
  size_t nb_sets = 0;
  int n_sub = 0;
  std::vector<size_t> sub_first, bpos_first;
  std::vector<uint32_t> pk_cnt, pk_first;
  std::vector<uint8_t> kv_set;
  std::vector<int32_t> bits_p, bits_kerr;
};

inline size_t shape_jobs(PkgShape& sh, const lsg_job* jobs, const std::vector<size_t>& ids,
                         const std::vector<size_t>* subs) {
  const size_t nj = ids.size();
  sh.jobs.assign(nj, JobRec());
  sh.job_ids = ids;
  sh.batch_order.clear();
  size_t n = 0;
  for (int pass = 0; pass < 2; pass++)
    for (size_t k = 0; k < nj; k++) {
      const lsg_job& J = jobs[ids[k]];
      const bool b = (J.flags & LSG_JOB_BATCHABLE) != 0;
      if (b != (pass == 0)) continue;
      sh.jobs[k].first = n;
      sh.jobs[k].count = J.n_sets;
      sh.jobs[k].flags = J.flags;
      n += J.n_sets;
      if (b) sh.batch_order.push_back(k);
    }
  sh.nb_sets = 0;
  for (size_t k : sh.batch_order) sh.nb_sets += sh.jobs[k].count;
  sh.n_sub = subs ? (int)subs->size() - 1 : 0;
  sh.sub_first.clear();
  sh.bpos_first.clear();
  if (subs) {
    sh.sub_first = *subs;
    sh.bpos_first.assign(1, 0);
    size_t q = 0;
    for (int k = 0; k < sh.n_sub; k++) {
      while (q < sh.batch_order.size() && sh.batch_order[q] < (*subs)[(size_t)k + 1]) q++;
      sh.bpos_first.push_back(q);
    }
  }
  return n;
}

inline bool batchable(const JobRec& J) { return (J.flags & LSG_JOB_BATCHABLE) != 0; }

inline std::vector<Range> pkg_chunks(const PkgShape& sh) {
// ... 606 lines not shown
```

Baseline: 3.623 million.

## Accumulate MSM buckets directly from affine signatures with mixed addition

Adds a direct MSM bucket kernel that reads affine signature points and accumulates them with mixed addition, splitting each bucket across lanes in slices that are combined by shuffle reduction. Because the kernel checks per-point usability itself, the separate sig_prep pass that built projective copies is skipped when only MSM groups need it. A new planner chooses the slice count from bucket sizes and occupancy targets. It also adds a check_msm test entry point. The aim is less memory traffic and cheaper adds, at the cost of extra shuffle reductions and possible lane imbalance.

```diff
diff --git a/include/lodestar_bls.h b/include/lodestar_bls.h
--- a/include/lodestar_bls.h
+++ b/include/lodestar_bls.h
@@ -156,6 +156,11 @@
 int lsg_check_fp_sqr(lsg_ctx* ctx, const uint32_t* in, size_t n, uint32_t* out);
 int lsg_check_fp2_sqr(lsg_ctx* ctx, const uint32_t* in, size_t n, uint32_t* out);
 int lsg_check_sums(lsg_ctx* ctx, const uint32_t* in, size_t n, uint32_t* out);
+#define LSG_CHECK_MSM_INF 1u
+#define LSG_CHECK_MSM_ERR 2u
+#define LSG_CHECK_MSM_PINF 4u
+int lsg_check_msm(lsg_ctx* ctx, const uint8_t* sig_aff192, const uint8_t* flags, const uint64_t* rnd, size_t n,
+                  uint8_t* out96);
 int lsg_probe_fp_mul_rate(lsg_ctx* ctx, double* fp_mul_per_s, double* mad_per_s);
 
 int lsg_probe_mad_peak(lsg_ctx* ctx, double* mad_per_s);
diff --git a/lodestar_amd/_native.py b/lodestar_amd/_native.py
--- a/lodestar_amd/_native.py
+++ b/lodestar_amd/_native.py
@@ -147,7 +147,7 @@
     "lsg_final_submit_groups", "lsg_final_wait_groups", "lsg_aggregate_signatures",
     "lsg_signing_roots", "lsg_attestation_signing_roots", "lsg_jobs_partial_device", "lsg_final_submit_device",
     "lsg_set_coalesce", "lsg_aggregate_pubkeys_multi", "lsg_check_fp2_mul",
-    "lsg_check_fp_sqr", "lsg_check_fp2_sqr", "lsg_check_sums",
+    "lsg_check_fp_sqr", "lsg_check_fp2_sqr", "lsg_check_sums", "lsg_check_msm",
     "lsg_deposit_signing_roots", "lsg_verify_deposits",
     "lsg_committees_set", "lsg_committees_clear", "lsg_committee_count",
     "lsg_object_signing_roots",
@@ -219,6 +219,7 @@
         lib.lsg_check_fp_sqr.argtypes = [vp, ctypes.c_char_p, sz, ctypes.c_char_p]
         lib.lsg_check_fp2_sqr.argtypes = [vp, ctypes.c_char_p, sz, ctypes.c_char_p]
         lib.lsg_check_sums.argtypes = [vp, ctypes.c_char_p, sz, ctypes.c_char_p]
+        lib.lsg_check_msm.argtypes = [vp, ctypes.c_char_p, ctypes.c_char_p, ctypes.POINTER(u64), sz, ctypes.c_char_p]
         lib.lsg_probe_mad_peak.argtypes = [vp, ctypes.POINTER(ctypes.c_double)]
         for name in EXPORTS:
             if name != "lsg_last_error":
@@ -702,6 +703,14 @@
         self._check(self.lib.lsg_check_sums(self.h, src, n, out), "lsg_check_sums")
         return list(struct.unpack(f"<{42 * 14 * n}I", out.raw))
 
+    def check_msm(self, points192, flags, rnd):
+        n = len(points192)
+        assert len(flags) == n and len(rnd) == n and all(len(p) == 192 for p in points192)
+        out = ctypes.create_string_buffer(96)
+        r = (ctypes.c_uint64 * n)(*rnd)
+        self._check(self.lib.lsg_check_msm(self.h, b"".join(points192), bytes(flags), r, n, out), "lsg_check_msm")
+        return out.raw
+
     def probe_fp_mul_rate(self):
         a, b = ctypes.c_double(), ctypes.c_double()
         self._check(self.lib.lsg_probe_fp_mul_rate(self.h, ctypes.byref(a), ctypes.byref(b)), "lsg_probe_fp_mul_rate")
diff --git a/lodestar_amd/build.py b/lodestar_amd/build.py
--- a/lodestar_amd/build.py
+++ b/lodestar_amd/build.py
@@ -12,7 +12,7 @@
 HEADERS = ["lsg_types.hpp", "lsg_fp_lane.hpp", "lsg_fp_elem.hpp", "lsg_tower.hpp", "lsg_curve.hpp", "lsg_h2c.hpp",
            "lsg_pairing.hpp", "lsg_constants.hpp", "lsg_fp_pair.hpp", "lsg_constants_r29.hpp", "lsg_io.hpp",
            "lsg_serial.h", "lsg_kcommon.hpp", "lsg_launch.h", "lsg_layout.h", "lsg_slp_progs.h", "lsg_slp_exec.hpp", "lsg_inv.hpp",
-           "lsg_ab.h", "lsg_plan.hpp", "lsg_bits.h", "lsg_ssz.hpp"]
+           "lsg_ab.h", "lsg_plan.hpp", "lsg_bits.h", "lsg_ssz.hpp", "lsg_msm.h"]
 OBJ = os.path.join(HERE, "_obj")
 AB_OUT = os.path.join(HERE, "liblodestar_bls_ab.so")
 AB_SOURCES = ["lsg_host.hip", "lsg_serial.hip", "lsg_serial_wide.hip"]
diff --git a/lodestar_amd/csrc/lsg_host.hip b/lodestar_amd/csrc/lsg_host.hip
--- a/lodestar_amd/csrc/lsg_host.hip
+++ b/lodestar_amd/csrc/lsg_host.hip
@@ -511,6 +511,10 @@
   w.b0_run = (size_t)std::max(2L, lsg_ab_long("LSG_B0_RUN", 4));
   w.seg_fold_wide = (int)lsg_ab_long("LSG_SEG_FOLD_WIDE", SEG_FOLD_WIDE);
   w.slp_items = slp_items_max();
+  w.msm_direct = lsg_ab_long("LSG_MSM_DIRECT", 1) != 0;
+  w.msm_slices_log2 = (int)lsg_ab_long("LSG_MSM_SLICES_LOG2", -1);
+  w.msm_fold = (int)std::min(1024L, std::max(1L, lsg_ab_long("LSG_MSM_FOLD", MSM_FOLD)));
+  w.msm_wide_pairs = (size_t)std::max(1L, lsg_ab_long("LSG_MSM_WIDE_PAIRS", (long)SEG_WIDE_PAIRS));
   return w;
 }
 SegPlan slot_seg(Slot* s, int op, const std::vector<int32_t>& seg_off, const std::vector<int32_t>& seg_len, bool has_idx,
@@ -640,6 +644,23 @@
   return LSG_OK;
 }
 
+int run_msm_buckets(Slot* s, int use, const SegPlan& P, uint32_t* dst) {
+  LSG_RC(size_seg(s, use, P));
+  uint32_t* tmp[3] = {nullptr, P_<uint32_t>(s->seg_tmp[use][0]), P_<uint32_t>(s->seg_tmp[use][1])};
+  for (size_t k = 0; k < P.passes.size(); k++) {
+    const SegPass& q = P.passes[k];
+    if (k == 0)
+      KL(s, "msm_buckets",
+         lsgk::msm_buckets(S_(s), q.n_chunks, q.ips_log2, PL(s, q.chunk_off), PL(s, P.idx_off), P_<uint32_t>(s->d_sigaff),
+                           P_<uint8_t>(s->d_siginf), P_<int32_t>(s->d_seterr), P_<uint8_t>(s->d_pinf), dst,
+                           tmp[q.tmp_out]));
+    else
+      KL(s, "msm_buckets", lsgk::seg_reduce(S_(s), 1, q.n_chunks, q.ips_log2, PL(s, q.chunk_off), nullptr, tmp[q.src], dst,
+                                            tmp[q.tmp_out]));
+  }
+  return LSG_OK;
+}
+
 int run_pk_seg(Slot* s, const SegPlan& P, uint32_t* dst) {
   LSG_RC(size_seg(s, 0, P));
   Dev* d = s->d;
@@ -999,7 +1020,10 @@
   LSG_RC(size_state(s, s->n_sets, s->n_pks, ng, Ph.n_msm, 2));
   s->cur = 1;
   if (Ph.n_msm) {
-    LSG_RC(run_seg(s, 1, "msm_buckets", Ph.buckets, rs_msm, P_<uint32_t>(s->d_bkt)));
+    if (Ph.buckets_direct)
+      LSG_RC(run_msm_buckets(s, 1, Ph.buckets, P_<uint32_t>(s->d_bkt)));
+    else
+      LSG_RC(run_seg(s, 1, "msm_buckets", Ph.buckets, rs_msm, P_<uint32_t>(s->d_bkt)));
     LSG_RC(run_seg(s, 1, "msm_bits", Ph.bits, P_<uint32_t>(s->d_bkt), P_<uint32_t>(s->d_bits)));
     KL(s, "k_g2p_to_canon", lsgk::g2p_to_canon(S_(s), (int)(MSM_BITS * Ph.n_msm), P_<uint32_t>(s->d_bits),
                                                P_<uint8_t>(s->d_Sb)));
@@ -1272,9 +1296,9 @@
   return b;
 }
 
-int launch_sig_prep(Slot* s, bool scale, const std::vector<uint8_t>* mode, uint32_t* out) {
+int launch_sig_prep(Slot* s, bool scale, bool raw, const std::vector<uint8_t>* mode, uint32_t* out) {
   const int n = (int)s->n_sets;
-  if (n == 0) return LSG_OK;
+  if (n == 0 || (!scale && !raw)) return LSG_OK;
   s->cur = 1;
   const uint8_t* dm = nullptr;
   if (scale && mode) {
@@ -1285,11 +1309,18 @@
     dm = P_<uint8_t>(s->d_mode);
   }
   if (scale && (size_t)n <= slp_items_max()) {
-    KL(s, "k_sig_prep", lsgk::sig_prep(S_(s), n, P_<uint32_t>(s->d_sigaff), P_<uint8_t>(s->d_siginf),
-                                       P_<int32_t>(s->d_seterr), P_<uint8_t>(s->d_pinf), nullptr, nullptr, out));
+    if (raw || !dm)
+      KL(s, "k_sig_prep", lsgk::sig_prep(S_(s), n, P_<uint32_t>(s->d_sigaff), P_<uint8_t>(s->d_siginf),
+                                         P_<int32_t>(s->d_seterr), P_<uint8_t>(s->d_pinf), nullptr, nullptr, out));
     KL(s, "k_slp_g2_scale", lsg_slp_g2_scale(S_(s), n, P_<uint32_t>(s->d_sigaff), P_<uint8_t>(s->d_siginf),
                                              P_<int32_t>(s->d_seterr), P_<uint8_t>(s->d_pinf), P_<uint64_t>(s->d_rnd),
                                              dm, out));
+    return LSG_OK;
+  }
+  if (scale && dm && !raw) {
+    KL(s, "k_sig_prep", lsgk::sig_scale_only(S_(s), n, P_<uint32_t>(s->d_sigaff), P_<uint8_t>(s->d_siginf),
+                                             P_<int32_t>(s->d_seterr), P_<uint8_t>(s->d_pinf), P_<uint64_t>(s->d_rnd), dm,
+                                             out));
     return LSG_OK;
   }
   KL(s, "k_sig_prep", lsgk::sig_prep(S_(s), n, P_<uint32_t>(s->d_sigaff), P_<uint8_t>(s->d_siginf),
@@ -1410,7 +1441,8 @@
       for (size_t g = A.n_msm; g < A.groups.size(); g++)
         memset(mode.data() + A.groups[g].first, 1, A.groups[g].len);
     }
-    LSG_RC(launch_sig_prep(s, any_small, mode.empty() ? nullptr : &mode, P_<uint32_t>(s->d_rs)));
+    LSG_RC(launch_sig_prep(s, any_small, A.n_msm && !A.buckets_direct, mode.empty() ? nullptr : &mode,
+                           P_<uint32_t>(s->d_rs)));
   }
   LSG_RC(launch_phase(s, A, P_<uint32_t>(s->d_rs), P_<uint32_t>(s->d_fall), true));
   if (A.groups.empty() || s->gp.big_g < 0) {
@@ -3325,6 +3357,55 @@
   return LSG_OK;
 }
 
+int lsg_check_msm(lsg_ctx* c, const uint8_t* sig_aff192, const uint8_t* flags, const uint64_t* rnd, size_t n,
+                  uint8_t* out96) {
+  if (!c || !sig_aff192 || !flags || !rnd || !out96 || n < 2 || n > 0x7fffffffull / 192) return LSG_ERR_INVALID_ARG;
+  LSG_ENTER(c);
+  timer_reset(&c->dev[0]->util);
+  Slot* s;
+  LSG_RC(sig_decode_impl(c, sig_aff192, 192, n, false, &s));
+  std::vector<int32_t> err(n);
+  std::vector<uint8_t> inf(n), pinf(n);
+  LSG_HIP(s, hipMemcpyAsync(err.data(), s->d_seterr.p, 4 * n, hipMemcpyDeviceToHost, s->st[0]));
+  LSG_HIP(s, hipMemcpyAsync(inf.data(), s->d_siginf.p, n, hipMemcpyDeviceToHost, s->st[0]));
+  LSG_HIP(s, hipStreamSynchronize(s->st[0]));
+  for (size_t i = 0; i < n; i++)
+    if (err[i] || inf[i]) return LSG_ERR_INVALID_ARG;
+  for (size_t i = 0; i < n; i++) {
+    inf[i] = (flags[i] & LSG_CHECK_MSM_INF) ? 1 : 0;
+    err[i] = (flags[i] & LSG_CHECK_MSM_ERR) ? LSG_BLST_BAD_ENCODING : 0;
+    pinf[i] = (flags[i] & LSG_CHECK_MSM_PINF) ? 1 : 0;
+  }
+  LSG_HIP(s, hipMemcpyAsync(s->d_seterr.p, err.data(), 4 * n, hipMemcpyHostToDevice, s->st[0]));
+  LSG_HIP(s, hipMemcpyAsync(s->d_siginf.p, inf.data(), n, hipMemcpyHostToDevice, s->st[0]));
+  LSG_HIP(s, hipMemcpyAsync(s->d_pinf.p, pinf.data(), n, hipMemcpyHostToDevice, s->st[0]));
+  PhasePlan Ph;
+  Grp g;
+  g.first = 0;
+  g.len = n;
+  g.msm = true;
+  Ph.groups.push_back(g);
+  s->plan.clear();
+  plan_phase(s->plan, std::vector<uint64_t>(rnd, rnd + n), 4, read_switches(), Ph);
+  LSG_RC(upload_plan(s));
+  s->cur = 0;
+  if (Ph.buckets_direct) {
+    LSG_RC(run_msm_buckets(s, 1, Ph.buckets, P_<uint32_t>(s->d_bkt)));
+  } else {
+    KL(s, "k_sig_prep", lsgk::sig_prep(S_(s), (int)n, P_<uint32_t>(s->d_sigaff), P_<uint8_t>(s->d_siginf),
+                                       P_<int32_t>(s->d_seterr), P_<uint8_t>(s->d_pinf), nullptr, nullptr,
+                                       P_<uint32_t>(s->d_rs)));
+    LSG_RC(run_seg(s, 1, "msm_buckets", Ph.buckets, P_<uint32_t>(s->d_rs), P_<uint32_t>(s->d_bkt)));
+  }
+  LSG_RC(run_seg(s, 1, "msm_bits", Ph.bits, P_<uint32_t>(s->d_bkt), P_<uint32_t>(s->d_bits)));
+  LSG_RC(ensure(s, s->d_aux, 96));
+  KL(s, "k_check_msm_horner", lsgk::check_msm_horner(S_(s), P_<uint32_t>(s->d_bits), P_<uint8_t>(s->d_aux)));
+  LSG_HIP(s, hipMemcpyAsync(out96, s->d_aux.p, 96, hipMemcpyDeviceToHost, s->st[0]));
+  LSG_HIP(s, hipStreamSynchronize(s->st[0]));
+  keep_times(s);
+  return LSG_OK;
+}
+
 int lsg_probe_fp_mul_rate(lsg_ctx* c, double* fp_mul_per_s, double* mad_per_s) {
   if (!c || !fp_mul_per_s || !mad_per_s) return LSG_ERR_INVALID_ARG;
   LSG_ENTER(c);
diff --git a/lodestar_amd/csrc/lsg_k_reduce.hip b/lodestar_amd/csrc/lsg_k_reduce.hip
--- a/lodestar_amd/csrc/lsg_k_reduce.hip
+++ b/lodestar_amd/csrc/lsg_k_reduce.hip
@@ -1,4 +1,5 @@
 #include "lsg_kcommon.hpp"
+#include "lsg_msm.h"
 namespace {
 #include "lsg_inv.hpp"
 }
@@ -57,6 +58,71 @@
     else
       lane_store(tmp, (size_t)(-out - 1), acc);
   }
+}
+
+__global__ void LSG_KERNEL_ATTR k_msm_buckets(int n_rows, int s_log2, const int32_t* __restrict__ rows,
+                                              const int32_t* __restrict__ idx, const uint32_t* __restrict__ sig_aff,
+                                              const uint8_t* __restrict__ inf, const int32_t* __restrict__ err,
+                                              const uint8_t* __restrict__ pinf, uint32_t* __restrict__ dst,
+                                              uint32_t* __restrict__ tmp) {
+  lsg_lane_setup();
+#if LSG_RED_PRIO
+  __builtin_amdgcn_s_setprio(LSG_RED_PRIO);
+#endif
+  const size_t item = gtid() / LSG_GROUP;
+  const size_t c = item >> s_log2;
+  const int S = 1 << s_log2, j = (int)(item & (size_t)(S - 1));
+  const bool active = c < (size_t)n_rows;
+  int start = 0, cnt = 0, out = 0;
+  if (active) {
+    const lsg_msm_slice_t sl = lsg_msm_slice(rows[3 * c], rows[3 * c + 1], s_log2, j);
+    start = sl.start;
+    cnt = sl.cnt;
+    out = rows[3 * c + 2];
+  }
+  int steps = cnt;
+#pragma unroll
+  for (int o = 32; o >= 1; o >>= 1) steps = max(steps, __shfl_xor(steps, o, 64));
+  g2p_t acc = proj_inf<fp2_t>();
+  auto set_at = [&](int k, bool& use) {
+    const size_t i = cnt > 0 ? (size_t)idx[start + min(k, cnt - 1)] : 0;
+    use = k < cnt && sig_usable(i, inf, err, pinf);
+    return i;
+  };
+  bool use = false;
+  size_t i = set_at(0, use);
+#pragma unroll 1
+  for (int k = 0; k < steps; k++) {
+    const g2a_t cur = lane_load<g2a_t>(sig_aff, i);
+    const bool cur_use = use;
+    if (k + 1 < steps) i = set_at(k + 1, use);
+    const g2p_t sum = g2_add_mixed(acc, cur);
+    acc.X = fselect(cur_use, sum.X, acc.X);
+    acc.Y = fselect(cur_use, sum.Y, acc.Y);
+    acc.Z = fselect(cur_use, sum.Z, acc.Z);
+  }
+#pragma unroll 1
+  for (int o = S >> 1; o >= 1; o >>= 1) acc = g2_add(acc, shfl_xor_t(acc, LSG_GROUP * o));
+  if (active && j == 0) {
+    if (out >= 0)
+      lane_store(dst, (size_t)out, acc);
+    else
+      lane_store(tmp, (size_t)(-out - 1), acc);
+  }
+}
+
+__global__ void LSG_KERNEL_ATTR k_check_msm_horner(const uint32_t* __restrict__ bits, uint8_t* __restrict__ out96) {
+  LANE_ITEM(1);
+  (void)lead;
+  g2p_t acc = lane_load<g2p_t>(bits, 63);
+#pragma unroll 1
+  for (int k = 62; k >= 0; k--) acc = g2_add(g2_dbl(acc), lane_load<g2p_t>(bits, (size_t)k));
+  const bool is_inf = proj_is_inf(acc);
+  g2a_t a;
+  a.x = fp2_zero();
+  a.y = fp2_zero();
+  if (!is_inf) a = proj_to_aff(acc);
+  g2_compress(out96 + 96 * item, a, is_inf);
 }
 
 __global__ void LSG_KERNEL_ATTR k_binv_fold(int n, int zero_to_one, const uint32_t* __restrict__ in,
@@ -312,6 +378,15 @@
   if (op == 1) LSG_LAUNCH_ITEMS(k_seg_reduce<1>, items, st, n_chunks, ips_log2, chunks, idx, src, dst, tmp);
   LSG_LAUNCH_ITEMS(k_seg_reduce<2>, items, st, n_chunks, ips_log2, chunks, idx, src, dst, tmp);
 }
+hipError_t msm_buckets(hipStream_t st, int n_rows, int s_log2, const int32_t* rows, const int32_t* idx,
+                       const uint32_t* sig_aff, const uint8_t* inf, const int32_t* err, const uint8_t* pinf, uint32_t* dst,
+                       uint32_t* tmp) {
+  LSG_LAUNCH_ITEMS(k_msm_buckets, (size_t)n_rows << s_log2, st, n_rows, s_log2, rows, idx, sig_aff, inf, err, pinf, dst,
+                   tmp);
+}
+hipError_t check_msm_horner(hipStream_t st, const uint32_t* bits, uint8_t* out96) {
+  LSG_LAUNCH_ITEMS(k_check_msm_horner, 1, st, bits, out96);
+}
 hipError_t binv_fold(hipStream_t st, int n, int zero_to_one, const uint32_t* in, uint32_t* pre, uint32_t* tot) {
   LSG_LAUNCH_ITEMS(k_binv_fold, (n + LSG_BINV_T - 1) / LSG_BINV_T, st, n, zero_to_one, in, pre, tot);
 }
diff --git a/lodestar_amd/csrc/lsg_k_sig.hip b/lodestar_amd/csrc/lsg_k_sig.hip
--- a/lodestar_amd/csrc/lsg_k_sig.hip
+++ b/lodestar_amd/csrc/lsg_k_sig.hip
@@ -33,9 +33,6 @@
   if (lead && !ok) err[item] = LSG_BLST_POINT_NOT_IN_GROUP;
 }
 
-LSG_DEVI bool sig_usable(size_t i, const uint8_t* inf, const int32_t* err, const uint8_t* pinf) {
-  return err[i] == 0 && !inf[i] && !(pinf && pinf[i]);
-}
 __global__ void LSG_KERNEL_ATTR k_sig_proj(int n, const uint32_t* __restrict__ sig_aff, const uint8_t* __restrict__ inf,
                                            const int32_t* __restrict__ err, const uint8_t* __restrict__ pinf,
                                            uint32_t* __restrict__ out) {
diff --git a/lodestar_amd/csrc/lsg_kcommon.hpp b/lodestar_amd/csrc/lsg_kcommon.hpp
--- a/lodestar_amd/csrc/lsg_kcommon.hpp
+++ b/lodestar_amd/csrc/lsg_kcommon.hpp
@@ -61,6 +61,10 @@
   return r;
 }
 
+static __device__ __forceinline__ bool sig_usable(size_t i, const uint8_t* inf, const int32_t* err, const uint8_t* pinf) {
+  return err[i] == 0 && !inf[i] && !(pinf && pinf[i]);
+}
+
 static __device__ __forceinline__ size_t gtid() { return (size_t)blockIdx.x * blockDim.x + threadIdx.x; }
 #define LANE_ITEM(n)                        \
   lsg_lane_setup();                         \
diff --git a/lodestar_amd/csrc/lsg_launch.h b/lodestar_amd/csrc/lsg_launch.h
--- a/lodestar_amd/csrc/lsg_launch.h
+++ b/lodestar_amd/csrc/lsg_launch.h
@@ -93,6 +93,10 @@
 
 hipError_t seg_reduce(hipStream_t st, int op, int n_chunks, int ips_log2, const int32_t* chunks, const int32_t* idx,
                       const uint32_t* src, uint32_t* dst, uint32_t* tmp);
+hipError_t msm_buckets(hipStream_t st, int n_rows, int s_log2, const int32_t* rows, const int32_t* idx,
+                       const uint32_t* sig_aff, const uint8_t* inf, const int32_t* err, const uint8_t* pinf, uint32_t* dst,
+                       uint32_t* tmp);
+hipError_t check_msm_horner(hipStream_t st, const uint32_t* bits, uint8_t* out96);
 hipError_t binv_fold(hipStream_t st, int n, int zero_to_one, const uint32_t* in, uint32_t* pre, uint32_t* tot);
 hipError_t binv_root(hipStream_t st, const uint32_t* top, uint32_t* inv);
 hipError_t binv_block(hipStream_t st, int n, int T, int zero_to_one, const uint32_t* in, uint32_t* pre, uint32_t* out);
diff --git a/lodestar_amd/csrc/lsg_msm.h b/lodestar_amd/csrc/lsg_msm.h
--- /dev/null
+++ b/lodestar_amd/csrc/lsg_msm.h
@@ -0,0 +1,20 @@
+#pragma once
+#include <stdint.h>
+
+#if defined(__HIPCC__)
+#define LSG_MSM_HD __host__ __device__ inline
+#else
+#define LSG_MSM_HD inline
+#endif
+
+struct lsg_msm_slice_t {
+  int32_t start, cnt;
+};
+
+LSG_MSM_HD lsg_msm_slice_t lsg_msm_slice(int32_t off, int32_t len, int s_log2, int j) {
+  const int32_t q = len >> s_log2, r = len & ((1 << s_log2) - 1);
+  lsg_msm_slice_t s;
+  s.start = off + j * q + (j < r ? j : r);
+  s.cnt = q + (j < r ? 1 : 0);
+  return s;
+}
diff --git a/lodestar_amd/csrc/lsg_plan.hpp b/lodestar_amd/csrc/lsg_plan.hpp
--- a/lodestar_amd/csrc/lsg_plan.hpp
+++ b/lodestar_amd/csrc/lsg_plan.hpp
@@ -69,6 +69,10 @@
   size_t b0_run = 4;
   int seg_fold_wide = SEG_FOLD_WIDE;
   size_t slp_items = 2048;
+  bool msm_direct = true;
+  int msm_slices_log2 = -1;
+  int msm_fold = 32;
+  size_t msm_wide_pairs = SEG_WIDE_PAIRS;
 };
 
 inline int ips_for(double avg, int32_t max_len, int fold) {
@@ -77,9 +81,15 @@
   return l;
 }
 
+struct SegPend {
+  int32_t seg, off, len;
+};
+inline void plan_seg_passes(std::vector<int32_t>& A, SegPlan& P, std::vector<SegPend> cur, double avg, int src,
+                            int tmp_out, int32_t dst_base, int fold_wide, size_t wide_pairs);
+
 inline SegPlan plan_seg(std::vector<int32_t>& A, int op, const std::vector<int32_t>& seg_off,
                         const std::vector<int32_t>& seg_len, bool has_idx, size_t idx_off, int32_t dst_base,
-                        int fold_wide) {
+                        int fold_wide, size_t wide_pairs = SEG_WIDE_PAIRS) {
   SegPlan P;
   P.op = op;
   P.has_idx = has_idx;
@@ -88,20 +98,23 @@
   if (ns == 0) return P;
   size_t total = 0;
   for (int32_t l : seg_len) total += (size_t)l;
-  struct Pend {
-    int32_t seg, off, len;
-  };
-  std::vector<Pend> cur(ns);
+  std::vector<SegPend> cur(ns);
   for (size_t s = 0; s < ns; s++) cur[s] = {(int32_t)s, seg_off[s], seg_len[s]};
-  double avg = (double)total / (double)ns;
-  int src = 0, tmp_out = 1;
+  plan_seg_passes(A, P, cur, (double)total / (double)ns, 0, 1, dst_base, fold_wide, wide_pairs);
+  return P;
+}
+
+inline void plan_seg_passes(std::vector<int32_t>& A, SegPlan& P, std::vector<SegPend> cur, double avg, int src,
+                            int tmp_out, int32_t dst_base, int fold_wide, size_t wide_pairs) {
+  typedef SegPend Pend;
+  const int op = P.op;
   while (!cur.empty()) {
     SegPass pass;
     int32_t max_len = 0;
     for (const Pend& p : cur) max_len = std::max(max_len, p.len);
     int fold = op == 2 ? SEG_FOLD_FP12 : SEG_FOLD;
     pass.ips_log2 = ips_for(avg, max_len, fold);
-    if (op != 2 && (cur.size() << 5) >= SEG_WIDE_PAIRS) {
+    if (op != 2 && (cur.size() << 5) >= wide_pairs) {
       int l = 0;
       while (l < pass.ips_log2 && (int32_t)(fold_wide << l) < max_len) l++;
       pass.ips_log2 = l;
@@ -140,6 +153,64 @@
     src = tmp_out;
     tmp_out = tmp_out == 1 ? 2 : 1;
   }
+}
+
+constexpr int MSM_FOLD = 32;
+constexpr size_t MSM_MIN_WAVES = 384;
+constexpr int MSM_MIN_SLICE = 8;
+
+inline int msm_slices_log2(size_t n_max, int c, size_t n_buckets, int fold) {
+  const size_t L = std::max<size_t>(1, 2 * ((n_max + ((size_t)1 << c) - 1) >> c));
+  int l = 0;
+  while (l < 5 && (((L + ((size_t)1 << l) - 1) >> l) > (size_t)fold ||
+                   ((n_buckets << l) < MSM_MIN_WAVES * 32 && (L >> (l + 1)) >= (size_t)MSM_MIN_SLICE)))
+    l++;
+  return l;
+}
+
+inline SegPlan plan_msm_buckets(std::vector<int32_t>& A, const std::vector<int32_t>& seg_off,
+                                const std::vector<int32_t>& seg_len, size_t idx_off, int s_log2, int fold, int fold_wide) {
+  SegPlan P;
+  P.op = 1;
+  P.has_idx = true;
+  P.idx_off = idx_off;
+  const size_t nb = seg_len.size();
+  if (nb == 0) return P;
+  SegPass pass;
+  pass.ips_log2 = s_log2;
+  pass.src = 0;
+  pass.tmp_out = 1;
+  pass.chunk_off = A.size();
+  const int32_t cap = (int32_t)(fold << s_log2);
+  std::vector<SegPend> nxt;
+  int32_t t = 0;
+  size_t nxt_total = 0;
+  for (size_t b = 0; b < nb; b++) {
+    const int32_t off = seg_off[b], len = seg_len[b];
+    if (len <= cap) {
+      A.push_back(off);
+      A.push_back(len);
+      A.push_back((int32_t)b);
+      pass.n_chunks++;
+      continue;
+    }
+    const int32_t k = (len + cap - 1) / cap, q = len / k, r = len % k;
+    int32_t o = off;
+    for (int32_t i = 0; i < k; i++) {
+      A.push_back(o);
+      A.push_back(q + (i < r ? 1 : 0));
+      A.push_back(-(t + i + 1));
+      o += q + (i < r ? 1 : 0);
+      pass.n_chunks++;
+    }
+    nxt.push_back({(int32_t)b, t, k});
+    t += k;
+    nxt_total += (size_t)k;
+  }
+  P.tmp_items = (size_t)t;
+  P.passes.push_back(pass);
+  if (!nxt.empty())
+    plan_seg_passes(A, P, nxt, (double)nxt_total / (double)nxt.size(), 1, 2, 0, fold_wide, SEG_WIDE_PAIRS);
   return P;
 }
 
@@ -152,6 +223,7 @@
   std::vector<Grp> groups;
   size_t n_msm = 0;
   SegPlan buckets, bits, sums, prod;
+  bool buckets_direct = false;
   size_t n_items = 0;
   size_t item_off = 0;
   size_t term_base = 0;
@@ -231,7 +303,17 @@
         }
       }
     }
-    Ph.buckets = plan_seg(A, 1, seg_off, seg_len, true, idx_off, 0, sw.seg_fold_wide);
+    Ph.buckets_direct = sw.msm_direct;
+    if (sw.msm_direct) {
+      size_t big = 0;
+      for (size_t g = 1; g < Ph.n_msm; g++)
+        if ((Ph.groups[g].len >> cw[g]) > (Ph.groups[big].len >> cw[big])) big = g;
+      const int s_log2 = sw.msm_slices_log2 >= 0 ? std::min(sw.msm_slices_log2, 5)
+                                                 : msm_slices_log2(Ph.groups[big].len, cw[big], cnt.size(), sw.msm_fold);
+      Ph.buckets = plan_msm_buckets(A, seg_off, seg_len, idx_off, s_log2, sw.msm_fold, sw.seg_fold_wide);
+    } else {
+      Ph.buckets = plan_seg(A, 1, seg_off, seg_len, true, idx_off, 0, sw.seg_fold_wide, sw.msm_wide_pairs);
+    }
     const size_t bidx = A.size();
     std::vector<int32_t> boff, blen;
     for (size_t g = 0; g < Ph.n_msm; g++) {
```

After: 3.648 million, median of 6. Within noise of the previous version (+0.7%).
